# rpp0/gr-lora

Hardware: AMD Instinct MI355X
Metric: IQ Msamples/s demodulated (higher is better)
Workload: dtype f32

## Files before the change

### gr_lora_amd/capi.py

```python
from __future__ import annotations

import ctypes as C
import os
from typing import List, Optional, Sequence, Tuple

import numpy as np

_HERE = os.path.dirname(os.path.abspath(__file__))
LIB_PATH = os.environ.get("LORA_HIP_LIB") or os.path.join(_HERE, "liblora_hip.so")

DEMOD_GRAD, DEMOD_FFT, DEMOD_FFT_COMPAT = 0, 1, 2
FLAG_TRACE = 1
FLAG_PIN_HOST = 2
FLAG_FAST_SYNC = 4
FLAG_NO_DECOUPLED = 8
IQ_CF32, IQ_SC16, IQ_SC8, IQ_CU8 = 0, 1, 2, 3

EXPORTS = [
    "lora_hip_abi_version", "lora_hip_strerror", "lora_hip_last_error", "lora_hip_create", "lora_hip_destroy",
    "lora_hip_get_geometry", "lora_hip_set_sf", "lora_hip_set_samp_rate", "lora_hip_work", "lora_hip_flush",
    "lora_hip_decode_device", "lora_hip_frames_available", "lora_hip_poll_frame", "lora_hip_drain_frames", "lora_hip_drain_slots", "lora_hip_demod_symbols_device", "lora_hip_demod_symbols_ex_device",
    "lora_hip_last_timing", "lora_hip_last_plan", "lora_hip_get_table", "lora_hip_last_payload_pass", "lora_hip_gap_starts_device", "lora_hip_decode_device_begin", "lora_hip_decode_device_end", "lora_hip_decode_device_prepass", "lora_hip_trace", "lora_hip_trace_clear", "lora_hip_check_frame", "lora_hip_estimate_cfo_device", "lora_hip_ref_ifreq_device",
    "lora_hip_set_stream_latency", "lora_hip_stream_info", "lora_hip_walker_kernel_name", "lora_hip_window_stats_device", "lora_hip_detect_preambles_device", "lora_hip_decode_at_headers_device",
    "lora_hip_mux_create", "lora_hip_mux_destroy", "lora_hip_mux_work", "lora_hip_mux_flush", "lora_hip_mux_set_latency", "lora_hip_mux_set_max_ahead", "lora_hip_mux_frames_available",
    "lora_hip_mux_poll_frame", "lora_hip_mux_passes", "lora_hip_mux_last_error",
    "lora_hip_iq_item_bytes", "lora_hip_iq_unpack_device", "lora_hip_work_raw",
]


EXPORTS_CHANNELIZER = [
    "lora_hip_channelizer_create", "lora_hip_channelizer_destroy", "lora_hip_channelizer_last_error", "lora_hip_channelizer_taps",
    "lora_hip_channelizer_output_items", "lora_hip_channelizer_run_device", "lora_hip_channelizer_work", "lora_hip_channelizer_apply_cfo",
    "lora_hip_channelizer_last_kernel_ms", "lora_hip_channelizer_run_device_raw", "lora_hip_channelizer_work_raw",
]


EXPORTS_FILTERBANK = [
    "lora_hip_filterbank_create", "lora_hip_filterbank_destroy", "lora_hip_filterbank_last_error", "lora_hip_filterbank_taps",
    "lora_hip_filterbank_output_items", "lora_hip_filterbank_run_device", "lora_hip_filterbank_run_device_rows", "lora_hip_filterbank_work",
    "lora_hip_filterbank_last_kernel_ms", "lora_hip_filterbank_run_device_raw", "lora_hip_filterbank_run_device_rows_raw", "lora_hip_filterbank_work_raw",
]


EXPORTS_GATEWAY = [
    "lora_hip_gateway_create", "lora_hip_gateway_destroy", "lora_hip_gateway_last_error", "lora_hip_gateway_work", "lora_hip_gateway_work_device",
    "lora_hip_gateway_flush", "lora_hip_gateway_set_latency", "lora_hip_gateway_frames_available", "lora_hip_gateway_poll_frame", "lora_hip_gateway_stats",
    "lora_hip_gateway_work_raw", "lora_hip_gateway_work_device_raw",
]

FILTERBANK_MAX_DST = 8
GATEWAY_MAX_DECODERS = 7
GATEWAY_STEP_OUTPUTS = 65536


class FilterBankConfig(C.Structure):
    _fields_ = [("struct_size", C.c_uint32), ("samp_rate", C.c_double), ("grid_offset_hz", C.c_double), ("n_grid", C.c_uint32),
                ("channels", C.POINTER(C.c_int32)), ("n_channels", C.c_uint32), ("bandwidth", C.c_uint32), ("decimation", C.c_uint32),
                ("device", C.c_int32), ("cutoff_hz", C.c_float), ("transition_hz", C.c_float), ("flags", C.c_uint32)]


class ChannelizerConfig(C.Structure):
    _fields_ = [("struct_size", C.c_uint32), ("samp_rate", C.c_float), ("center_freq", C.c_float), ("channel_list", C.POINTER(C.c_float)),
                ("n_channels", C.c_uint32), ("bandwidth", C.c_uint32), ("decimation", C.c_uint32), ("device", C.c_int32),
                ("cutoff_hz", C.c_float), ("transition_hz", C.c_float), ("flags", C.c_uint32)]


CHANNELIZER_FLAG_UINT32_OFFSET = 1


class Config(C.Structure):
    _fields_ = [("struct_size", C.c_uint32), ("samp_rate", C.c_float), ("bandwidth", C.c_uint32),
                ("sf", C.c_uint8), ("implicit", C.c_uint8), ("cr", C.c_uint8), ("crc", C.c_uint8),
                ("reduced_rate", C.c_uint8), ("disable_drift_correction", C.c_uint8), ("reserved0", C.c_uint8 * 2),
                ("device", C.c_int32), ("demod", C.c_int32), ("flags", C.c_uint32),
                ("segment_symbols", C.c_uint32), ("batch_items", C.c_uint32)]


class FrameInfo(C.Structure):
    _fields_ = [("stream", C.c_uint32), ("length", C.c_uint32), ("header_pos", C.c_int64), ("end_pos", C.c_int64)]


class Step(C.Structure):
    _fields_ = [("state", C.c_int32), ("consumed", C.c_int32), ("pos", C.c_int64), ("bin", C.c_int32),
                ("fine", C.c_int32), ("value", C.c_float), ("stream", C.c_uint32), ("cycles", C.c_uint32), ("reserved", C.c_uint32)]


class Timing(C.Structure):
    _fields_ = [("walker_ms", C.c_float), ("total_device_ms", C.c_float), ("walker_launches", C.c_uint32),
                ("jobs", C.c_uint32), ("probes", C.c_uint32), ("slow_path_relaunches", C.c_uint32),
                ("items", C.c_uint64)]


class FrameCheck(C.Structure):
    _fields_ = [("has_header", C.c_uint8), ("header_checksum_ok", C.c_uint8), ("has_crc", C.c_uint8), ("crc_ok", C.c_uint8),
                ("header_checksum_rx", C.c_uint8), ("header_checksum_calc", C.c_uint8), ("crc_rx", C.c_uint16), ("crc_calc", C.c_uint16),
                ("reserved", C.c_uint16)]


class StreamInfo(C.Structure):
    _fields_ = [("batch_items", C.c_uint64), ("buffered_items", C.c_uint64), ("passes", C.c_uint64), ("passes_by_latency", C.c_uint64),
                ("consumed_base", C.c_int64), ("max_latency_ms", C.c_float), ("pass_in_flight", C.c_uint32)]


class WindowStats(C.Structure):
    _fields_ = [("bin_down", C.c_int32), ("peak_down", C.c_float), ("total_down", C.c_float), ("bin_up", C.c_int32), ("peak_up", C.c_float), ("total_up", C.c_float)]


class Preamble(C.Structure):
    _fields_ = [("header_pos", C.c_int64), ("run_pos", C.c_int64), ("stream", C.c_uint32), ("run_len", C.c_uint32), ("bin", C.c_int32), ("sfd_index", C.c_int32),
                ("pmr", C.c_float), ("cfo_bins", C.c_float), ("cfo_hz", C.c_float), ("delta", C.c_int32)]


class GatewayConfig(C.Structure):
    _fields_ = [("struct_size", C.c_uint32), ("filterbank", FilterBankConfig), ("decoders", C.POINTER(Config)), ("n_decoders", C.c_uint32),
                ("flags", C.c_uint32)]


class GatewayFrameInfo(C.Structure):
    _fields_ = [("row", C.c_uint32), ("grid_index", C.c_int32), ("sf", C.c_uint32), ("decoder", C.c_uint32), ("length", C.c_uint32),
                ("reserved", C.c_uint32), ("header_pos", C.c_int64), ("end_pos", C.c_int64)]


class GatewayStats(C.Structure):
    _fields_ = [("struct_size", C.c_uint32), ("n_decoders", C.c_uint32), ("passes", C.c_uint64 * GATEWAY_MAX_DECODERS),
                ("passes_by_latency", C.c_uint64 * GATEWAY_MAX_DECODERS), ("filterbank_calls", C.c_uint64), ("filterbank_ms", C.c_double),
                ("items_in", C.c_uint64), ("step_outputs", C.c_uint64)]


class LoraHipError(RuntimeError):
    def __init__(self, status: int, msg: str):
        super().__init__("lora_hip status %d: %s" % (status, msg))
        self.status = status


_lib = None


def load():
    global _lib
    if _lib is not None:
        return _lib
    try:
        import torch
    except ImportError:
        pass
    if not os.path.exists(LIB_PATH):
        raise ImportError("liblora_hip.so not built: run `python -c 'import __graft_entry__ as g; g.build()'` "
                          "(hipcc --offload-arch=gfx950).  There is no CPU fallback.")
    L = C.CDLL(LIB_PATH)
    vp = C.c_void_p
    L.lora_hip_abi_version.restype = C.c_uint32
    L.lora_hip_strerror.restype = C.c_char_p
    L.lora_hip_strerror.argtypes = [C.c_int]
    L.lora_hip_last_error.restype = C.c_char_p
    L.lora_hip_last_error.argtypes = [vp]
    L.lora_hip_create.argtypes = [C.POINTER(Config), C.POINTER(vp)]
    L.lora_hip_destroy.argtypes = [vp]
    L.lora_hip_destroy.restype = None
    L.lora_hip_get_geometry.argtypes = [vp, C.POINTER(C.c_uint32), C.POINTER(C.c_uint32), C.POINTER(C.c_uint32)]
    L.lora_hip_set_sf.argtypes = [vp, C.c_uint8]
    L.lora_hip_set_samp_rate.argtypes = [vp, C.c_float]
    L.lora_hip_work.argtypes = [vp, vp, C.c_size_t, C.POINTER(C.c_size_t)]
    L.lora_hip_flush.argtypes = [vp]
    L.lora_hip_decode_device.argtypes = [vp, vp, C.c_size_t, vp, vp, C.c_uint32, vp]
    L.lora_hip_frames_available.restype = C.c_size_t
    L.lora_hip_frames_available.argtypes = [vp]
    L.lora_hip_poll_frame.argtypes = [vp, vp, C.c_size_t, C.POINTER(C.c_size_t), C.POINTER(FrameInfo)]
    L.lora_hip_drain_frames.argtypes = [vp, vp, C.c_size_t, C.POINTER(FrameInfo), C.c_size_t, C.POINTER(C.c_size_t)]
    L.lora_hip_drain_slots.argtypes = [vp, vp, C.c_size_t, C.c_size_t, C.POINTER(C.c_size_t)]
    L.lora_hip_demod_symbols_device.argtypes = [vp, vp, C.c_size_t, vp, C.c_size_t, C.c_int, vp, vp]
    L.lora_hip_demod_symbols_ex_device.argtypes = [vp, vp, C.c_size_t, vp, C.c_size_t, C.c_int, vp, vp, vp]
    L.lora_hip_last_timing.argtypes = [vp, C.POINTER(Timing)]
    L.lora_hip_last_plan.argtypes = [vp, C.POINTER(C.c_uint32), C.POINTER(C.c_uint32)]
    L.lora_hip_last_payload_pass.argtypes = [vp, C.POINTER(C.c_uint32), C.POINTER(C.c_uint32), C.POINTER(C.c_uint32), C.POINTER(C.c_uint32), C.POINTER(C.c_uint32), C.POINTER(C.c_float)]
    L.lora_hip_decode_device_begin.argtypes = [vp, vp, C.c_size_t, vp, vp, C.c_uint32, vp, C.c_uint32]
    L.lora_hip_decode_device_end.argtypes = [vp]
    L.lora_hip_decode_device_prepass.argtypes = [vp, vp, C.c_size_t, vp, vp, C.c_uint32, vp, C.c_uint32]
    L.lora_hip_gap_starts_device.argtypes = [vp, vp, C.c_size_t, vp, vp, C.c_uint32, vp, C.c_size_t, vp, vp]
    L.lora_hip_trace.restype = C.c_size_t
    L.lora_hip_trace.argtypes = [vp, C.POINTER(C.POINTER(Step))]
    L.lora_hip_trace_clear.argtypes = [vp]
    L.lora_hip_trace_clear.restype = None
    L.lora_hip_estimate_cfo_device.argtypes = [vp, vp, C.c_size_t, C.POINTER(C.c_int64), C.c_size_t, C.c_int, C.POINTER(C.c_float), vp]
    L.lora_hip_estimate_cfo_device.restype = C.c_int
    L.lora_hip_ref_ifreq_device.argtypes = [vp, vp, C.c_size_t, C.POINTER(C.c_float), C.POINTER(C.c_float), vp]
    L.lora_hip_ref_ifreq_device.restype = C.c_int
    if hasattr(L, "lora_hip_get_table") or not os.environ.get("LORA_HIP_LIB"):
        L.lora_hip_get_table.argtypes = [vp, C.c_int, C.POINTER(C.c_float), C.c_size_t, C.POINTER(C.c_size_t)]
        L.lora_hip_get_table.restype = C.c_int
    L.lora_hip_window_stats_device.argtypes = [vp, vp, C.c_size_t, vp, C.c_size_t, C.POINTER(WindowStats), vp]
    L.lora_hip_detect_preambles_device.argtypes = [vp, vp, C.c_size_t, vp, vp, C.c_uint32, C.c_float, C.POINTER(Preamble), C.c_size_t, C.POINTER(C.c_size_t), vp]
    L.lora_hip_decode_at_headers_device.argtypes = [vp, vp, C.c_size_t, vp, vp, C.c_uint32, C.POINTER(Preamble), C.c_size_t, vp]
    L.lora_hip_walker_kernel_name.argtypes = [vp]
    L.lora_hip_walker_kernel_name.restype = C.c_char_p
    L.lora_hip_mux_create.argtypes = [C.POINTER(Config), C.c_uint32, C.POINTER(vp)]
    L.lora_hip_mux_destroy.argtypes = [vp]
    L.lora_hip_mux_destroy.restype = None
    L.lora_hip_mux_work.argtypes = [vp, C.c_uint32, vp, C.c_size_t]
    L.lora_hip_mux_flush.argtypes = [vp]
    L.lora_hip_mux_set_latency.argtypes = [vp, C.c_float]
    L.lora_hip_mux_set_max_ahead.argtypes = [vp, C.c_size_t]
    L.lora_hip_mux_frames_available.argtypes = [vp]
    L.lora_hip_mux_frames_available.restype = C.c_size_t
    L.lora_hip_mux_poll_frame.argtypes = [vp, vp, C.c_size_t, C.POINTER(C.c_size_t), C.POINTER(FrameInfo)]
    L.lora_hip_mux_passes.argtypes = [vp, C.POINTER(C.c_uint64), C.POINTER(C.c_uint64)]
    L.lora_hip_mux_last_error.argtypes = [vp]
    L.lora_hip_mux_last_error.restype = C.c_char_p
    L.lora_hip_set_stream_latency.argtypes = [vp, C.c_float]
    L.lora_hip_stream_info.argtypes = [vp, C.POINTER(StreamInfo)]
    L.lora_hip_check_frame.argtypes = [C.c_char_p, C.c_size_t, C.POINTER(FrameCheck)]
    L.lora_hip_check_frame.restype = C.c_int
    L.lora_hip_channelizer_create.argtypes = [C.POINTER(ChannelizerConfig), C.POINTER(vp)]
    L.lora_hip_channelizer_destroy.argtypes = [vp]
    L.lora_hip_channelizer_destroy.restype = None
    L.lora_hip_channelizer_last_error.argtypes = [vp]
    L.lora_hip_channelizer_last_error.restype = C.c_char_p
    L.lora_hip_channelizer_taps.argtypes = [vp, vp, C.c_size_t, C.POINTER(C.c_size_t)]
    L.lora_hip_channelizer_output_items.argtypes = [vp, C.c_size_t]
    L.lora_hip_channelizer_output_items.restype = C.c_size_t
    L.lora_hip_channelizer_run_device.argtypes = [vp, vp, C.c_size_t, vp, C.c_size_t, C.POINTER(C.c_size_t), vp]
    L.lora_hip_channelizer_work.argtypes = [vp, vp, C.c_size_t, vp, C.c_size_t, C.POINTER(C.c_size_t)]
    L.lora_hip_channelizer_apply_cfo.argtypes = [vp, C.c_float]
    L.lora_hip_channelizer_last_kernel_ms.argtypes = [vp]
    L.lora_hip_channelizer_last_kernel_ms.restype = C.c_float
    L.lora_hip_filterbank_create.argtypes = [C.POINTER(FilterBankConfig), C.POINTER(vp)]
    L.lora_hip_filterbank_destroy.argtypes = [vp]
    L.lora_hip_filterbank_destroy.restype = None
    L.lora_hip_filterbank_last_error.argtypes = [vp]
    L.lora_hip_filterbank_last_error.restype = C.c_char_p
    L.lora_hip_filterbank_taps.argtypes = [vp, vp, C.c_size_t, C.POINTER(C.c_size_t)]
    L.lora_hip_filterbank_output_items.argtypes = [vp, C.c_size_t]
    L.lora_hip_filterbank_output_items.restype = C.c_size_t
    L.lora_hip_filterbank_run_device.argtypes = [vp, vp, C.c_size_t, vp, C.c_size_t, C.POINTER(C.c_size_t), vp]
    L.lora_hip_filterbank_work.argtypes = [vp, vp, C.c_size_t, vp, C.c_size_t, C.POINTER(C.c_size_t)]
    L.lora_hip_filterbank_last_kernel_ms.argtypes = [vp]
    L.lora_hip_filterbank_last_kernel_ms.restype = C.c_float
    L.lora_hip_filterbank_run_device_rows.argtypes = [vp, vp, C.c_size_t, C.POINTER(vp), C.c_uint32, C.c_size_t, C.POINTER(C.c_size_t), vp]
    L.lora_hip_gateway_create.argtypes = [C.POINTER(GatewayConfig), C.POINTER(vp)]
    L.lora_hip_gateway_destroy.argtypes = [vp]
    L.lora_hip_gateway_destroy.restype = None
    L.lora_hip_gateway_last_error.argtypes = [vp]
    L.lora_hip_gateway_last_error.restype = C.c_char_p
    L.lora_hip_gateway_work.argtypes = [vp, vp, C.c_size_t]
    L.lora_hip_gateway_work_device.argtypes = [vp, vp, C.c_size_t, vp]
    L.lora_hip_gateway_flush.argtypes = [vp]
    L.lora_hip_gateway_set_latency.argtypes = [vp, C.c_float]
    L.lora_hip_gateway_frames_available.argtypes = [vp]
    L.lora_hip_gateway_frames_available.restype = C.c_size_t
    L.lora_hip_gateway_poll_frame.argtypes = [vp, vp, C.c_size_t, C.POINTER(C.c_size_t), C.POINTER(GatewayFrameInfo)]
    L.lora_hip_gateway_stats.argtypes = [vp, C.POINTER(GatewayStats)]
    if hasattr(L, "lora_hip_work_raw") or not os.environ.get("LORA_HIP_LIB"):
        L.lora_hip_iq_item_bytes.argtypes = [C.c_int]
        L.lora_hip_iq_item_bytes.restype = C.c_size_t
        L.lora_hip_iq_unpack_device.argtypes = [C.c_int, vp, C.c_size_t, C.c_int, C.c_float, vp, vp]
        L.lora_hip_work_raw.argtypes = [vp, vp, C.c_size_t, C.c_int, C.c_float, C.POINTER(C.c_size_t)]
        L.lora_hip_channelizer_run_device_raw.argtypes = [vp, vp, C.c_size_t, C.c_int, C.c_float, vp, C.c_size_t, C.POINTER(C.c_size_t), vp]
        L.lora_hip_channelizer_work_raw.argtypes = [vp, vp, C.c_size_t, C.c_int, C.c_float, vp, C.c_size_t, C.POINTER(C.c_size_t)]
        L.lora_hip_filterbank_run_device_raw.argtypes = [vp, vp, C.c_size_t, C.c_int, C.c_float, vp, C.c_size_t, C.POINTER(C.c_size_t), vp]
        L.lora_hip_filterbank_run_device_rows_raw.argtypes = [vp, vp, C.c_size_t, C.c_int, C.c_float, C.POINTER(vp), C.c_uint32, C.c_size_t, C.POINTER(C.c_size_t), vp]
        L.lora_hip_filterbank_work_raw.argtypes = [vp, vp, C.c_size_t, C.c_int, C.c_float, vp, C.c_size_t, C.POINTER(C.c_size_t)]
        L.lora_hip_gateway_work_raw.argtypes = [vp, vp, C.c_size_t, C.c_int, C.c_float]
        L.lora_hip_gateway_work_device_raw.argtypes = [vp, vp, C.c_size_t, C.c_int, C.c_float, vp]
    _lib = L
    return L


def _raw_items(raw, fmt=None):
    from . import iqformat
    return iqformat.as_components(raw, fmt)


def unpack_device(d_raw: int, n_items: int, fmt: int, d_out: int, scale: float = 0.0, device: int = 0, stream: int = 0):
    L = load()
    st = L.lora_hip_iq_unpack_device(int(device), d_raw, int(n_items), int(fmt), float(scale), d_out, stream)
    if st != 0:
        raise LoraHipError(st, "lora_hip_iq_unpack_device: %s" % L.lora_hip_strerror(st).decode())


def check_frame(blob: bytes) -> FrameCheck:
    out = FrameCheck()
    st = load().lora_hip_check_frame(bytes(blob), len(blob), C.byref(out))
    if st != 0:
        raise LoraHipError(st, "lora_hip_check_frame: blob too short")
    return out


class Handle:

    def __init__(self, samp_rate=1e6, bandwidth=125000, sf=7, implicit=False, cr=4, crc=True, reduced_rate=False,
                 disable_drift_correction=False, device=0, demod=DEMOD_FFT_COMPAT, flags=0, segment_symbols=0,
                 batch_items=0):
        self.L = load()
        cfg = Config(struct_size=C.sizeof(Config), samp_rate=float(samp_rate), bandwidth=int(bandwidth), sf=int(sf),
                     implicit=int(bool(implicit)), cr=int(cr), crc=int(bool(crc)), reduced_rate=int(bool(reduced_rate)),
                     disable_drift_correction=int(bool(disable_drift_correction)), device=int(device), demod=int(demod),
                     flags=int(flags), segment_symbols=int(segment_symbols), batch_items=int(batch_items))
        h = C.c_void_p()
        st = self.L.lora_hip_create(C.byref(cfg), C.byref(h))
        if st != 0:
            raise LoraHipError(st, "%s (%s)" % (self.L.lora_hip_strerror(st).decode(), self.L.lora_hip_last_error(None).decode()))
        self.h = h
        a, b, d = C.c_uint32(), C.c_uint32(), C.c_uint32()
        self.L.lora_hip_get_geometry(self.h, C.byref(a), C.byref(b), C.byref(d))
        self.sps, self.nbins, self.decim = a.value, b.value, d.value
        self.device, self.batch_items = int(device), int(batch_items)

    def close(self):
        if getattr(self, "h", None):
            self.L.lora_hip_destroy(self.h)
            self.h = None

    __del__ = close

    def _check(self, st: int):
        if st != 0:
            raise LoraHipError(st, "%s (%s)" % (self.L.lora_hip_strerror(st).decode(), self.L.lora_hip_last_error(self.h).decode()))

    def work(self, iq: np.ndarray) -> int:
        a = np.ascontiguousarray(iq, dtype=np.complex64)
        n = C.c_size_t(0)
        self._check(self.L.lora_hip_work(self.h, a.ctypes.data, a.size, C.byref(n)))
        return n.value

    def work_raw(self, raw, fmt=None, scale: float = 0.0) -> int:
        a, f, n_items = _raw_items(raw, fmt)
        n = C.c_size_t(0)
# ... 31 lines not shown

    def decode_device_end(self):
        self._check(self.L.lora_hip_decode_device_end(self.h))

    def gap_starts_device(self, dev_ptr: int, total_items: int, offs: Sequence[int], lens: Sequence[int], stream: int = 0):
        o = np.ascontiguousarray(offs, dtype=np.uint64)
        l = np.ascontiguousarray(lens, dtype=np.uint64)
        cap = int(sum(int(x) for x in l) // 64 + 16)
        pos = np.zeros(cap, dtype=np.int64)
        cnt = np.zeros(o.size, dtype=np.uint32)
        self._check(self.L.lora_hip_gap_starts_device(self.h, dev_ptr, total_items, o.ctypes.data, l.ctypes.data, o.size, pos.ctypes.data, cap,
                                                      cnt.ctypes.data, stream))
        out, k = [], 0
        for c in cnt:
            out.append(pos[k:k + int(c)].copy()); k += int(c)
        return out

    def demod_symbols_device(self, dev_ptr: int, total_items: int, offsets: Sequence[int], demod: int, stream: int = 0) -> np.ndarray:
        off = np.ascontiguousarray(offsets, dtype=np.int64)
        out = np.zeros(off.size, dtype=np.uint32)
        self._check(self.L.lora_hip_demod_symbols_device(self.h, dev_ptr, total_items, off.ctypes.data, off.size, demod, out.ctypes.data, stream))
        return out

    def demod_symbols_ex_device(self, dev_ptr: int, total_items: int, offsets: Sequence[int], demod: int, stream: int = 0):
        off = np.ascontiguousarray(offsets, dtype=np.int64)
        out = np.zeros(off.size, dtype=np.uint32)
        fine = np.zeros(off.size, dtype=np.int32)
        self._check(self.L.lora_hip_demod_symbols_ex_device(self.h, dev_ptr, total_items, off.ctypes.data, off.size, demod, out.ctypes.data,
                                                            fine.ctypes.data, stream))
        return out, fine

    def estimate_cfo_device(self, dev_ptr: int, total_items: int, offsets: Sequence[int], mode: int = 1, stream: int = 0) -> np.ndarray:
        off = np.ascontiguousarray(offsets, dtype=np.int64)
        out = np.zeros(off.size, dtype=np.float32)
        self._check(self.L.lora_hip_estimate_cfo_device(self.h, C.c_void_p(dev_ptr), total_items, off.ctypes.data_as(C.POINTER(C.c_int64)), off.size, mode,
                                                        out.ctypes.data_as(C.POINTER(C.c_float)), C.c_void_p(stream)))
        return out

    def ref_ifreq_device(self, dev_ptr: int, n_items: int, stream: int = 0):
        arg = np.zeros(n_items, dtype=np.float32)
        f = np.zeros(n_items - 1, dtype=np.float32)
        self._check(self.L.lora_hip_ref_ifreq_device(self.h, C.c_void_p(dev_ptr), n_items, arg.ctypes.data_as(C.POINTER(C.c_float)),
                                                     f.ctypes.data_as(C.POINTER(C.c_float)), C.c_void_p(stream)))
        return arg, f

    def window_stats_device(self, dev_ptr: int, total_items: int, offsets: Sequence[int], stream: int = 0):
        off = np.ascontiguousarray(offsets, dtype=np.int64)
        out = (WindowStats * max(off.size, 1))()
        self._check(self.L.lora_hip_window_stats_device(self.h, dev_ptr, total_items, off.ctypes.data, off.size, out, stream))
        return [(o.bin_down, o.peak_down, o.total_down, o.bin_up, o.peak_up, o.total_up) for o in out[: off.size]]

    def detect_preambles_device(self, dev_ptr: int, total_items: int, offs: Sequence[int], lens: Sequence[int], threshold: float = 0.0, stream: int = 0, cap: int = 4096):
        o = np.ascontiguousarray(offs, dtype=np.uint64)
        l = np.ascontiguousarray(lens, dtype=np.uint64)
        out = (Preamble * cap)()
        n = C.c_size_t(0)
        self._check(self.L.lora_hip_detect_preambles_device(self.h, dev_ptr, total_items, o.ctypes.data, l.ctypes.data, o.size, float(threshold), out, cap, C.byref(n), stream))
        return [dict(header_pos=p.header_pos, run_pos=p.run_pos, stream=p.stream, run_len=p.run_len, bin=p.bin, sfd_index=p.sfd_index, pmr=p.pmr,
                     cfo_bins=p.cfo_bins, cfo_hz=p.cfo_hz, delta=p.delta) for p in out[: n.value]]

    def decode_at_headers_device(self, dev_ptr: int, total_items: int, offs: Sequence[int], lens: Sequence[int], preambles, stream: int = 0):
        o = np.ascontiguousarray(offs, dtype=np.uint64)
        l = np.ascontiguousarray(lens, dtype=np.uint64)
        arr = (Preamble * max(len(preambles), 1))()
        for i, p in enumerate(preambles):
            st, hp = (p["stream"], p["header_pos"]) if isinstance(p, dict) else p
            arr[i].stream, arr[i].header_pos = int(st), int(hp)
        self._check(self.L.lora_hip_decode_at_headers_device(self.h, dev_ptr, total_items, o.ctypes.data, l.ctypes.data, o.size, arr, len(preambles), stream))

    def frames_available(self) -> int:
        return self.L.lora_hip_frames_available(self.h)

    def poll_frame(self) -> Optional[Tuple[bytes, FrameInfo]]:
        buf = (C.c_uint8 * 320)()
        n = C.c_size_t(0)
        info = FrameInfo()
        self._check(self.L.lora_hip_poll_frame(self.h, buf, 320, C.byref(n), C.byref(info)))
        if n.value == 0:
            return None
        return bytes(buf[: n.value]), info

    def drain(self) -> List[Tuple[bytes, FrameInfo]]:
        out = []
        while True:
            n_avail = self.frames_available()
            if n_avail == 0:
                return out
            k = min(n_avail, 4096)
            buf = (C.c_uint8 * (k * 280))()
            infos = (FrameInfo * k)()
            n = C.c_size_t(0)
            self._check(self.L.lora_hip_drain_frames(self.h, buf, k * 280, infos, k, C.byref(n)))
            raw = bytes(buf)
            off = 0
            for i in range(n.value):
                ln = infos[i].length
                inf = FrameInfo(infos[i].stream, ln, infos[i].header_pos, infos[i].end_pos)
                out.append((raw[off:off + ln], inf))
                off += ln
            if n.value == 0:
                return out

    INFO_DTYPE = np.dtype([("stream", "<u4"), ("length", "<u4"), ("header_pos", "<i8"), ("end_pos", "<i8")])

    def drain_raw(self):
        bufs, infos = [], []
        while True:
            n_avail = self.frames_available()
            if n_avail == 0:
                break
            k = min(n_avail, 8192)
            buf = np.empty(k * 280, dtype=np.uint8)
            inf = np.empty(k, dtype=self.INFO_DTYPE)
            n = C.c_size_t(0)
            self._check(self.L.lora_hip_drain_frames(self.h, buf.ctypes.data, buf.size, C.cast(inf.ctypes.data, C.POINTER(FrameInfo)), k, C.byref(n)))
            if n.value == 0:
                break
            inf = inf[: n.value]
            bufs.append(buf[: int(inf["length"].sum())])
            infos.append(inf)
        if not bufs:
            return np.empty(0, dtype=np.uint8), np.empty(0, dtype=self.INFO_DTYPE)
        return np.concatenate(bufs), np.concatenate(infos)

    def drain_slots(self, slot_bytes: int) -> np.ndarray:
        n_avail = self.frames_available()
        out = np.empty((max(n_avail, 1), slot_bytes), dtype=np.uint8)
        n = C.c_size_t(0)
        self._check(self.L.lora_hip_drain_slots(self.h, out.ctypes.data, slot_bytes, n_avail, C.byref(n)))
        return out[: n.value]

    def timing(self) -> Timing:
        t = Timing()
        self._check(self.L.lora_hip_last_timing(self.h, C.byref(t)))
        return t

    def plan(self):
        b, n = C.c_uint32(0), C.c_uint32(0)
        self._check(self.L.lora_hip_last_plan(self.h, C.byref(b), C.byref(n)))
        return bool(b.value), int(n.value)

    def table(self, which: int) -> np.ndarray:
        n = C.c_size_t()
        self._check(self.L.lora_hip_get_table(self.h, which, None, 0, C.byref(n)))
        out = np.empty(n.value, np.float32)
        self._check(self.L.lora_hip_get_table(self.h, which, out.ctypes.data_as(C.POINTER(C.c_float)), n.value, C.byref(n)))
        return out

    def payload_pass(self):
        a, mv, b, r, c, m = C.c_uint32(0), C.c_uint32(0), C.c_uint32(0), C.c_uint32(0), C.c_uint32(0), C.c_float(0)
        self._check(self.L.lora_hip_last_payload_pass(self.h, C.byref(a), C.byref(mv), C.byref(b), C.byref(r), C.byref(c), C.byref(m)))
        return dict(packets=int(a.value), moved=int(mv.value), rerun=int(b.value), rounds=int(r.value), symbols=int(c.value), ms=float(m.value))

    def trace(self):
        p = C.POINTER(Step)()
        n = self.L.lora_hip_trace(self.h, C.byref(p))
        return [(p[i].state, p[i].pos, p[i].consumed, p[i].bin, p[i].fine, p[i].value, p[i].stream, p[i].cycles) for i in range(n)]

    def trace_clear(self):
        self.L.lora_hip_trace_clear(self.h)


class Mux:

    def __init__(self, n_channels, samp_rate=1e6, bandwidth=125000, sf=7, implicit=False, cr=4, crc=True, reduced_rate=False,
                 disable_drift_correction=False, device=0, demod=DEMOD_FFT_COMPAT, flags=0, segment_symbols=0, batch_items=0):
        self.L = load()
        cfg = Config(struct_size=C.sizeof(Config), samp_rate=float(samp_rate), bandwidth=int(bandwidth), sf=int(sf), implicit=int(bool(implicit)), cr=int(cr),
                     crc=int(bool(crc)), reduced_rate=int(bool(reduced_rate)), disable_drift_correction=int(bool(disable_drift_correction)), device=int(device),
                     demod=int(demod), flags=int(flags), segment_symbols=int(segment_symbols), batch_items=int(batch_items))
        self.h = C.c_void_p()
        st = self.L.lora_hip_mux_create(C.byref(cfg), int(n_channels), C.byref(self.h))
        if st != 0:
            raise LoraHipError(st, "%s (%s)" % (self.L.lora_hip_strerror(st).decode(), self.L.lora_hip_last_error(None).decode()))
        self.n_channels = int(n_channels)

    def _check(self, st):
        if st != 0:
            raise LoraHipError(st, "%s (%s)" % (self.L.lora_hip_strerror(st).decode(), (self.L.lora_hip_mux_last_error(self.h) or b"").decode()))

    def work(self, channel: int, iq: np.ndarray):
        a = np.ascontiguousarray(iq, dtype=np.complex64)
        self._check(self.L.lora_hip_mux_work(self.h, int(channel), a.ctypes.data, a.size))

    def flush(self):
        self._check(self.L.lora_hip_mux_flush(self.h))

    def set_latency(self, ms: float):
        self._check(self.L.lora_hip_mux_set_latency(self.h, float(ms)))

    def set_max_ahead(self, items: int):
        self._check(self.L.lora_hip_mux_set_max_ahead(self.h, int(items)))

    def passes(self):
        a, b = C.c_uint64(0), C.c_uint64(0)
        self._check(self.L.lora_hip_mux_passes(self.h, C.byref(a), C.byref(b)))
        return int(a.value), int(b.value)

    def drain(self) -> List[Tuple[bytes, FrameInfo]]:
        out = []
        buf = (C.c_uint8 * 320)()
        while self.L.lora_hip_mux_frames_available(self.h):
            n = C.c_size_t(0)
            info = FrameInfo()
            self._check(self.L.lora_hip_mux_poll_frame(self.h, buf, 320, C.byref(n), C.byref(info)))
            out.append((bytes(buf[: n.value]), info))
        return out

    def close(self):
        if getattr(self, "h", None):
            self.L.lora_hip_mux_destroy(self.h)
            self.h = None

    __del__ = close


class Channelizer:

    def __init__(self, samp_rate, center_freq, channel_list, bandwidth, decimation=1, device=0, cutoff_hz=0.0, transition_hz=0.0, flags=0):
        self.L = load()
        self.n_channels = len(channel_list)
        self._chan = (C.c_float * self.n_channels)(*[float(c) for c in channel_list])
        cfg = ChannelizerConfig(struct_size=C.sizeof(ChannelizerConfig), samp_rate=float(samp_rate), center_freq=float(center_freq),
                                channel_list=self._chan, n_channels=self.n_channels, bandwidth=int(bandwidth), decimation=int(decimation), device=int(device),
                                cutoff_hz=float(cutoff_hz), transition_hz=float(transition_hz), flags=int(flags))
        self.h = C.c_void_p()
        st = self.L.lora_hip_channelizer_create(C.byref(cfg), C.byref(self.h))
        if st != 0:
            raise LoraHipError(st, self.L.lora_hip_strerror(st).decode())

    def _check(self, st):
        if st != 0:
            raise LoraHipError(st, (self.L.lora_hip_channelizer_last_error(self.h) or b"").decode() or self.L.lora_hip_strerror(st).decode())

    def taps(self) -> np.ndarray:
        n = C.c_size_t(0)
        self._check(self.L.lora_hip_channelizer_taps(self.h, None, 0, C.byref(n)))
        t = np.zeros(n.value, dtype=np.float32)
        self._check(self.L.lora_hip_channelizer_taps(self.h, t.ctypes.data, t.size, C.byref(n)))
        return t

    def output_items(self, n_in: int) -> int:
        return int(self.L.lora_hip_channelizer_output_items(self.h, n_in))

    def work(self, x) -> np.ndarray:
        a = np.ascontiguousarray(x, dtype=np.complex64)
        no = self.output_items(a.size)
        out = np.zeros((self.n_channels, max(no, 1)), dtype=np.complex64)
        n = C.c_size_t(0)
        self._check(self.L.lora_hip_channelizer_work(self.h, a.ctypes.data, a.size, out.ctypes.data, out.shape[1], C.byref(n)))
        return out[:, : n.value]

    def run_device(self, d_in: int, n_in: int, d_out: int, out_stride: int, stream: int = 0) -> int:
        n = C.c_size_t(0)
        self._check(self.L.lora_hip_channelizer_run_device(self.h, d_in, n_in, d_out, out_stride, C.byref(n), stream))
        return int(n.value)

    def work_raw(self, raw, fmt=None, scale: float = 0.0) -> np.ndarray:
        a, f, n_items = _raw_items(raw, fmt)
        no = self.output_items(n_items)
        out = np.zeros((self.n_channels, max(no, 1)), dtype=np.complex64)
        n = C.c_size_t(0)
        self._check(self.L.lora_hip_channelizer_work_raw(self.h, a.ctypes.data, n_items, f, float(scale), out.ctypes.data, out.shape[1], C.byref(n)))
        return out[:, : n.value]

    def run_device_raw(self, d_in: int, n_in: int, fmt: int, d_out: int, out_stride: int, scale: float = 0.0, stream: int = 0) -> int:
        n = C.c_size_t(0)
        self._check(self.L.lora_hip_channelizer_run_device_raw(self.h, d_in, n_in, int(fmt), float(scale), d_out, out_stride, C.byref(n), stream))
        return int(n.value)

    def apply_cfo(self, cfo: float):
        self._check(self.L.lora_hip_channelizer_apply_cfo(self.h, float(cfo)))

    def kernel_ms(self) -> float:
        return float(self.L.lora_hip_channelizer_last_kernel_ms(self.h))

    def close(self):
        if self.h:
            self.L.lora_hip_channelizer_destroy(self.h)
            self.h = C.c_void_p()

    def __del__(self):
        try:
            self.close()
        except Exception:
            pass


class FilterBank:

    def __init__(self, samp_rate, grid_offset, n_grid, channels, bandwidth, decimation=1, device=0, cutoff_hz=0.0, transition_hz=0.0, flags=0):
        self.L = load()
        self.channels = [int(k) for k in channels]
        self.n_channels = len(self.channels)
        self._chan = (C.c_int32 * max(self.n_channels, 1))(*self.channels)
        cfg = FilterBankConfig(struct_size=C.sizeof(FilterBankConfig), samp_rate=float(samp_rate), grid_offset_hz=float(grid_offset), n_grid=int(n_grid),
                               channels=self._chan, n_channels=self.n_channels, bandwidth=int(bandwidth), decimation=int(decimation), device=int(device),
                               cutoff_hz=float(cutoff_hz), transition_hz=float(transition_hz), flags=int(flags))
        self.h = C.c_void_p()
        st = self.L.lora_hip_filterbank_create(C.byref(cfg), C.byref(self.h))
        if st != 0:
            raise LoraHipError(st, self.L.lora_hip_strerror(st).decode())

    def _check(self, st):
        if st != 0:
            raise LoraHipError(st, (self.L.lora_hip_filterbank_last_error(self.h) or b"").decode() or self.L.lora_hip_strerror(st).decode())
# ... 139 lines not shown
```

### gr_lora_amd/csrc/lora_device.h

```cpp
#pragma once
#include <stdint.h>

#if !defined(__HIPCC__) && !defined(HIP_INCLUDE_HIP_HIP_RUNTIME_H)
struct float2 { float x, y; };
#endif

namespace lora_hip {

constexpr int kWG = 256;
constexpr int kMaxBinsPerThread = 16;
constexpr int kMaxFrame = 3 + 255 + 2;
constexpr int kMaxCodewords = 640;

enum DecState : int32_t { kDetect = 0, kSync, kFindSfd, kPause, kDecodeHeader, kDecodePayload, kStop };

enum AttemptStatus : uint32_t {
    kAttemptNone = 0,
    kAttemptFrame = 1,
    kAttemptLostSync = 2,
    kAttemptOutOfData = 3,
    kAttemptAtHeader = 4,
    kAttemptAtSfd = 5,
    kAttemptHeaderOnly = 6
};
struct SkippedPayload {
    uint8_t  phdr[3];
    uint8_t  n_left;
    uint8_t  left[8];
    int32_t  payload_symbols;
};
constexpr float kSfdIllVar = 1.0f / 4096.0f;
constexpr int kMaxSfdRec = 12;

struct DevParams {
    uint32_t sf, nbins, nbins_hdr, sps, decim, log_nbins, delay_after_sync;
    uint32_t implicit, reduced_rate, enable_fine_sync, demod_mode;
    uint32_t ctor_cr, ctor_crc;
    uint32_t use_fast;
    uint32_t fft_groups;
    uint32_t fft_stride;
    uint32_t lds_work_bytes;
    uint32_t ifreq_in_lds_1;
    uint32_t ifreq_in_lds_2;
    float    down_ifreq_avg;
    float    down_ifreq_sd;
    float    down_ifreq_dsum;
    double   sync_a, sync_b;
    uint32_t sync_closed_form;
    uint32_t strict_sync;
    uint32_t samples_per_second;
    uint32_t ffs_on;
    float    ffs_alpha, ffs_jump, ffs_tol;
    const float2 *down;
    const float  *up_ifreq;
    const float  *down_ifreq;
    const float  *up_ifreq_v;
    const float2 *twN;
    const float2 *tws;
    const float  *wave_tabs;
    const float2 *w3_tw;
    const float2 *w3_ctab;
    const float  *team_tabs;
};

struct Job {
    uint64_t stream_off;
    uint64_t stream_len;
    int64_t  start;
    int64_t  scan_limit;
    uint32_t stream_id;
    uint32_t cr_prev;
    uint32_t max_attempts;
    uint32_t stop_at_header;
    int64_t  probe_limit;
    uint32_t start_at_header;
    uint32_t tail_stop_sfd;
};

struct AttemptRec {
    int64_t  start_pos;
    int64_t  trig_pos;
    int64_t  hdr_pos;
    int64_t  end_pos;
    uint32_t status;
    uint32_t npush;
    float    push_tail[4];
    uint32_t cr_prev;
    uint32_t hdr_ambig;
    uint32_t frame_len;
    uint32_t n_symbols;
    int64_t  sfd_pos[kMaxSfdRec];
    uint32_t n_sfd;
    uint8_t  sfd_fails[kMaxSfdRec];
    uint8_t  frame[kMaxFrame + 4];
};

struct JobResult {
    int64_t  final_pos;
    uint32_t n_attempts;
    uint32_t final_cr;
    uint32_t npush;
    float    push_tail[4];
    uint32_t stop_reason;
    uint32_t n_steps;
    uint32_t pad;
    uint32_t cyc[6];
    uint32_t rounds[6];
    int64_t  tail_final_pos;
    uint32_t tail_valid, tail_first_rec, tail_n_attempts, tail_final_cr, tail_npush, tail_stop_reason, tail_pad, tail_rsv;
    float    tail_push_tail[4];
    uint32_t ctl[4];
    uint32_t dbg[6];
};

struct StepRec {
    int32_t  state, consumed;
    int64_t  pos;
    int32_t  bin, fine;
    float    value;
    uint32_t stream;
    uint32_t cycles;
    uint32_t pad;
};

struct LaunchCfg {
    const float2 *iq;
    const Job *jobs;
    JobResult *results;
    AttemptRec *recs;
    uint32_t recs_per_job;
    float *scratch;
    StepRec *trace;
    uint32_t trace_cap;
    uint32_t n_jobs;
    uint32_t *balance;
    uint32_t skip_payload;
};
constexpr uint32_t kBalanceCus = 2048;
constexpr uint32_t kBalanceWords = 3u * kBalanceCus;

struct EnvStream {
    uint64_t off;
    uint32_t first_block;
    uint32_t n_blocks;
};
int launch_envelope(const float2 *iq, const EnvStream *streams , uint32_t n_streams, uint32_t sps,
                    float *d_E, unsigned long long *d_bitmap , void *stream);

int launch_walker(const DevParams &p, const LaunchCfg &c, void *stream);
const char *walker_kernel_name(const DevParams &p);
struct DemodAlt { int32_t *shift; uint32_t *bins; int32_t *fine; int64_t max_start; };
int launch_demod_symbols(const DevParams &p, const float2 *iq, const int64_t *d_offsets, uint32_t n,
                         int demod, uint32_t *d_bins, int32_t *d_fine, float *scratch, void *stream, const DemodAlt *alt = nullptr);
int launch_detect_windows(const DevParams &p, const float2 *iq, const int64_t *d_offsets, uint32_t n, void *d_out , void *stream);
constexpr int kPayloadHyp = 4;
struct PayloadDesc {
    uint32_t n_walk;
    uint32_t n_hyp;
    int32_t  hyp_shift[kPayloadHyp];
    int32_t  hyp_base[kPayloadHyp];
    uint32_t hyp_from[kPayloadHyp];
    uint32_t hyp_to[kPayloadHyp];
    int64_t  room;
    SkippedPayload sk;
};
enum PayloadWalk : uint32_t { kWalkComplete = 0, kWalkOutOfData = 1, kWalkNeedShift = 2 };
struct PayloadOut {
    uint32_t result;
    uint32_t at;
    int32_t  shift;
    uint32_t frame_len;
    uint8_t  frame[kMaxFrame + 4];
};
int launch_payload_chain(const DevParams &p, const uint32_t *d_bins, const int32_t *d_fine, const DemodAlt &alt, const PayloadDesc *descs, PayloadOut *outs, uint32_t n_packets, void *stream);
bool walker_has_skip_variant(const DevParams &p);
int launch_ref_ifreq(const float2 *x, uint32_t n, float *d_arg, float *d_ifreq, void *stream);
int launch_cfo(const DevParams &p, const float2 *iq, const int64_t *d_offsets, uint32_t n, int mode, float *d_out, void *stream);
bool walker3_covers(uint32_t sf);
uint32_t w3_tw_entries(uint32_t sf);
void build_w3_tables(uint32_t sf, float2 *tw, float2 *ctab );
uint32_t wave_tables_floats(uint32_t sf);
void build_wave_tables(uint32_t sf, const float2 *down, float *out);
uint32_t wave_tables_floats_d(uint32_t sf, uint32_t decim);
void build_wave_tables_d(uint32_t sf, uint32_t decim, const float2 *down, float *out);
uint32_t team_tables_entries(uint32_t sf);
void build_team_tables(uint32_t sf, const float2 *down, double dt, double bandwidth, float2 *out);
uint32_t walker_lds_bytes(const DevParams &p);
uint32_t walker_resident_slots(const DevParams &p);
uint32_t walker_resident_slots_full(const DevParams &p);
const char *walker_kernel_name_for(const DevParams &p, uint32_t n_jobs, bool skip = false);

}
```

### gr_lora_amd/csrc/lora_kernels.hip

```cpp

#include <hip/hip_runtime.h>
#include <math.h>
#include <stdio.h>
#include <atomic>
#include <cstdlib>
#include <stdint.h>
#include <type_traits>

#include "lora_device.h"
#include "whitening_data.inc"

namespace lora_hip {

__constant__ unsigned char c_whiten_cr56[LORA_WHITEN_CR56_LEN];
__constant__ unsigned char c_whiten_cr78[LORA_WHITEN_CR78_LEN];
__constant__ unsigned char c_h84_decode[256];
static std::atomic<bool> g_consts_ready[16];

static unsigned char h_hamming_encode(unsigned v)
{
    const unsigned b0 = v & 1u, b1 = (v >> 1) & 1u, b2 = (v >> 2) & 1u, b3 = (v >> 3) & 1u;
    const unsigned p1 = b1 ^ b2 ^ b3, p2 = b0 ^ b1 ^ b2, p3 = b0 ^ b1 ^ b3, p4 = b0 ^ b2 ^ b3;
    return (unsigned char)(p1 | (b0 << 1) | (b1 << 2) | (b2 << 3) | (p2 << 4) | (b3 << 5) | (p3 << 6) | (p4 << 7));
}
// ... 295 lines not shown
    return r;
}
constexpr int ilog2(int v) { return v <= 1 ? 0 : 1 + ilog2(v >> 1); }

#define LORA_DPP(old, v, ctrl, bank) __builtin_amdgcn_update_dpp((old), (v), (ctrl), 0xf, (bank), false)

template <int MASK>
__device__ __forceinline__ float lane_xor(float f)
{
    const int v = __builtin_bit_cast(int, f);
    int r;
    if constexpr (MASK == 1) r = LORA_DPP(0, v, 0xB1, 0xf);
    else if constexpr (MASK == 2) r = LORA_DPP(0, v, 0x4E, 0xf);
    else if constexpr (MASK == 4) {
        r = LORA_DPP(0, v, 0x104, 0x5);
        r = LORA_DPP(r, v, 0x114, 0xA);
    } else if constexpr (MASK == 8) r = LORA_DPP(0, v, 0x128, 0xf);
    else if constexpr (MASK == 16) {
        const auto p = __builtin_amdgcn_permlane16_swap(v, v, false, false);
        r = (threadIdx.x & 16) ? p[0] : p[1];
    } else {
        const auto p = __builtin_amdgcn_permlane32_swap(v, v, false, false);
        r = (threadIdx.x & 32) ? p[0] : p[1];
    }
    return __builtin_bit_cast(float, r);
}

template <int MASK>
__device__ __forceinline__ float2 lane_xor2(float2 v) { return make_float2(lane_xor<MASK>(v.x), lane_xor<MASK>(v.y)); }

__device__ __forceinline__ float wave_sum_rows(float v)
{
    v += lane_xor<1>(v); v += lane_xor<2>(v); v += lane_xor<4>(v); v += lane_xor<8>(v);
    const float r0 = __builtin_bit_cast(float, __builtin_amdgcn_readlane(__builtin_bit_cast(int, v), 0));
    const float r1 = __builtin_bit_cast(float, __builtin_amdgcn_readlane(__builtin_bit_cast(int, v), 16));
    const float r2 = __builtin_bit_cast(float, __builtin_amdgcn_readlane(__builtin_bit_cast(int, v), 32));
    const float r3 = __builtin_bit_cast(float, __builtin_amdgcn_readlane(__builtin_bit_cast(int, v), 48));
    return (r0 + r1) + (r2 + r3);
}

__device__ __forceinline__ uint32_t uni32(uint32_t v) { return (uint32_t)__builtin_amdgcn_readfirstlane((int)v); }
__device__ __forceinline__ uint64_t uni64(uint64_t v) { return ((uint64_t)uni32((uint32_t)(v >> 32)) << 32) | uni32((uint32_t)v); }
__device__ __forceinline__ Job uniform_job(const Job &j)
{
    Job u;
    u.stream_off = uni64(j.stream_off); u.stream_len = uni64(j.stream_len);
    u.start = (int64_t)uni64((uint64_t)j.start); u.scan_limit = (int64_t)uni64((uint64_t)j.scan_limit);
    u.stream_id = uni32(j.stream_id); u.cr_prev = uni32(j.cr_prev); u.max_attempts = uni32(j.max_attempts); u.stop_at_header = uni32(j.stop_at_header);
    u.probe_limit = (int64_t)uni64((uint64_t)j.probe_limit);
    u.start_at_header = uni32(j.start_at_header); u.tail_stop_sfd = uni32(j.tail_stop_sfd);
    return u;
}

__device__ __forceinline__ uint32_t rotl_bits(uint32_t bits, uint32_t count, uint32_t size)
{
    const uint32_t mask = (1u << size) - 1u;
    count %= size;
    bits &= mask;
    return ((bits << count) & mask) | (bits >> (size - count));
}

__device__ __forceinline__ uint8_t deshuffle_byte(uint8_t v)
{
    return (uint8_t)(((v >> 5) & 1u) | (((v >> 0) & 1u) << 1) | (((v >> 1) & 1u) << 2) | (((v >> 2) & 1u) << 3) |
                     (((v >> 4) & 1u) << 4) | (((v >> 3) & 1u) << 5) | (((v >> 6) & 1u) << 6) | (((v >> 7) & 1u) << 7));
}

__device__ __forceinline__ uint8_t data_bits(uint8_t cw)
{
    return (uint8_t)(((cw >> 1) & 1u) | (((cw >> 2) & 1u) << 1) | (((cw >> 3) & 1u) << 2) | (((cw >> 5) & 1u) << 3));
}

__device__ void deinterleave_block(Shared &sh, uint32_t n_words, uint32_t ppm, uint32_t &n_cw)
{
    if (n_words <= 8u) {
        uint32_t r[8];
#pragma unroll
        for (uint32_t i = 0; i < 8u; i++) r[i] = (i < n_words) ? rotl_bits(sh.words[i], i, ppm) : 0u;
        for (uint32_t x = 0; x < ppm; x++) {
            uint32_t c = 0;
#pragma unroll
            for (uint32_t i = 0; i < 8u; i++) c |= ((r[i] >> x) & 1u) << i;
            if (n_cw < kMaxCodewords) sh.cw[n_cw++] = (uint8_t)c;
        }
        return;
    }
    for (uint32_t x = 0; x < ppm; x++) {
        uint8_t c = 0;
        for (uint32_t i = 0; i < n_words; i++) c |= (uint8_t)(((rotl_bits(sh.words[i], i, ppm) >> x) & 1u) << i);
        if (n_cw < kMaxCodewords) sh.cw[n_cw++] = c;
    }
}
__device__ __forceinline__ void deinterleave_block_wave(Shared &sh, uint64_t words_pk, uint32_t n_words, uint32_t ppm, uint32_t &n_cw)
{
    const uint32_t lane = threadIdx.x & 63u, x = lane >> 3, i = lane & 7u;
    const uint32_t w = (uint32_t)(words_pk >> (8u * i)) & 0xffu;
    int sh_amt = (int)x - (int)(i % ppm);
    if (sh_amt < 0) sh_amt += (int)ppm;
    const bool bit = x < ppm && i < n_words && ((w >> sh_amt) & 1u);
    const unsigned long long m = __ballot(bit);
    if (i == 0u && x < ppm && n_cw + x < (uint32_t)kMaxCodewords) sh.cw[n_cw + x] = (uint8_t)((m >> (8u * x)) & 0xffu);
    n_cw = (n_cw + ppm <= (uint32_t)kMaxCodewords) ? n_cw + ppm : (uint32_t)kMaxCodewords;
}

__device__ __forceinline__ void deinterleave_block_wave16(Shared &sh, const uint32_t (&wpk)[4], uint32_t n_words, uint32_t ppm, uint32_t &n_cw)
{
    const uint32_t lane = threadIdx.x & 63u, x = lane >> 3, i = lane & 7u;
    const uint32_t pair = i < 2u ? wpk[0] : i < 4u ? wpk[1] : i < 6u ? wpk[2] : wpk[3];
    const uint32_t w = (pair >> (16u * (i & 1u))) & 0xffffu;
    const int rot = (int)(i % ppm);
    int sh_amt = (int)x - rot;
    if (sh_amt < 0) sh_amt += (int)ppm;
    const bool bit = x < ppm && i < n_words && ((w >> sh_amt) & 1u);
    const unsigned long long m = __ballot(bit);
    if (i == 0u && x < ppm && n_cw + x < (uint32_t)kMaxCodewords) sh.cw[n_cw + x] = (uint8_t)((m >> (8u * x)) & 0xffu);
    int sh8 = 8 - rot;
    if (sh8 < 0) sh8 += (int)ppm;
    const unsigned long long m8 = __ballot(lane < 8u && ppm > 8u && i < n_words && ((w >> sh8) & 1u));
    if (lane == 0u && ppm > 8u && n_cw + 8u < (uint32_t)kMaxCodewords) sh.cw[n_cw + 8u] = (uint8_t)(m8 & 0xffu);
    n_cw = (n_cw + ppm <= (uint32_t)kMaxCodewords) ? n_cw + ppm : (uint32_t)kMaxCodewords;
}

__device__ void decode_header_bytes(const Shared &sh, uint32_t n_cw, int cr_class, uint8_t out[3])
{
    uint8_t w[6];
    for (int i = 0; i < 5; i++) w[i] = ((uint32_t)i < n_cw) ? deshuffle_byte(sh.cw[i]) : 0;
    w[5] = 0;
    for (int k = 0; k < 3; k++) {
        if (cr_class == 2) out[k] = (uint8_t)((c_h84_decode[w[2 * k]] << 4) | c_h84_decode[w[2 * k + 1]]);
        else if (cr_class == 1) out[k] = (uint8_t)((data_bits(w[2 * k]) << 4) | data_bits(w[2 * k + 1]));
        else out[k] = 0;
    }
}

__device__ void decode_payload_bytes(Shared &sh, uint32_t n_cw, uint32_t cr, uint32_t n_bytes)
{
    __syncthreads();
    for (uint32_t i = threadIdx.x; i < n_cw; i += blockDim.x) {
        uint8_t w = deshuffle_byte(sh.cw[i]);
        if (cr <= 2u) w ^= (i < LORA_WHITEN_CR56_LEN) ? c_whiten_cr56[i] : 0;
        else w ^= (i < LORA_WHITEN_CR78_LEN) ? c_whiten_cr78[i] : 0;
        sh.cw[i] = w;
    }
    __syncthreads();
    for (uint32_t k = threadIdx.x; k < n_bytes; k += blockDim.x) {
        const uint8_t c0 = (2u * k < n_cw) ? sh.cw[2u * k] : 0, c1 = (2u * k + 1u < n_cw) ? sh.cw[2u * k + 1u] : 0;
        uint8_t lo, hi;
        if (cr >= 3u) { lo = c_h84_decode[c0]; hi = c_h84_decode[c1]; }
        else if (cr >= 1u) { lo = data_bits(c0); hi = data_bits(c1); }
        else { lo = 0; hi = 0; }
        sh.dec[k] = (uint8_t)((hi << 4) | lo);
    }
    __syncthreads();
}

template <int FLDS>
__device__ __forceinline__ void walker_body(const DevParams &P, const LaunchCfg &C)
{
    extern __shared__ __attribute__((aligned(16))) unsigned char smem[];
    float2 *work = reinterpret_cast<float2 *>(smem);
    float *fl = reinterpret_cast<float *>(smem);
    Shared &sh = *reinterpret_cast<Shared *>(smem + P.lds_work_bytes);
    float *red = sh.red;
    __shared__ strict::Cands g_sc;
    __shared__ __attribute__((aligned(16))) float g_strict_buf[strict::kK * 256];

    const uint32_t jid = blockIdx.x;
    if (jid >= C.n_jobs) return;
    const Job job = C.jobs[jid];
    const float2 *__restrict__ X = C.iq + job.stream_off;
    const int64_t n_items = (int64_t)job.stream_len;
    const uint32_t sps = P.sps;
    float *gscratch = C.scratch ? C.scratch + (size_t)jid * 2u * sps : nullptr;
    float *f1, *f2;
    if constexpr (FLDS >= 1) f1 = fl; else f1 = gscratch;
    if constexpr (FLDS >= 2) f2 = fl; else f2 = gscratch;
    AttemptRec *recs = C.recs + (size_t)jid * C.recs_per_job;
    StepRec *trace = C.trace ? C.trace + (size_t)jid * C.trace_cap : nullptr;
    const bool t0 = threadIdx.x == 0;
    const float *vtab = P.up_ifreq_v, *utab = P.up_ifreq;

    int32_t state = kDetect;
    int64_t pos = job.start;
    uint32_t corr_fails = 0, cr = job.cr_prev, has_crc = P.ctor_crc;
    int32_t payload_symbols = 0;
    uint32_t payload_length = 0, n_words = 0, n_cw = 0, n_sym = 0;
    float energy_threshold = 0.0f;
    uint8_t phdr0 = 0, phdr1 = (uint8_t)((P.ctor_cr << 5) | (P.ctor_crc << 4)), phdr2 = 0;
    uint32_t n_att = 0, npush = 0, n_steps = 0, stop_reason = 0;
    float push_tail[4] = {0.f, 0.f, 0.f, 0.f};
    int64_t att_start = pos, att_trig = -1, att_hdr = -1;
    uint32_t att_cr_prev = cr, att_ambig = 0;
    bool in_attempt = false, frame_ok = false;
    if (job.start_at_header) { state = kDecodeHeader; in_attempt = true; att_trig = pos; att_hdr = pos; }

    auto end_step = [&](int32_t st_in, int32_t consumed, int32_t step_bin, int32_t fine, float step_val, long long t_start) -> bool {
        if (trace && t0 && n_steps < C.trace_cap) {
            StepRec &s = trace[n_steps];
            s.state = st_in; s.consumed = consumed; s.pos = pos; s.bin = step_bin; s.fine = fine; s.value = step_val;
            s.stream = job.stream_id; s.cycles = (uint32_t)(clock64() - t_start); s.pad = 0;
        }
        n_steps++;
        pos += consumed;
        if (in_attempt && state == kDetect) {
            if (t0) {
                AttemptRec &r = recs[n_att];
                r.status = frame_ok ? kAttemptFrame : kAttemptLostSync;
                if (!frame_ok) r.frame_len = 0;
                r.start_pos = att_start; r.trig_pos = att_trig; r.hdr_pos = att_hdr; r.end_pos = pos;
                r.npush = npush;
                for (int i = 0; i < 4; i++) r.push_tail[i] = push_tail[i];
                r.cr_prev = att_cr_prev; r.hdr_ambig = att_ambig; r.n_symbols = n_sym; r.n_sfd = 0;
            }
            n_att++;
            in_attempt = false;
            frame_ok = false;
            npush = 0;
            att_start = pos;
        } else if (in_attempt && job.stop_at_header && state == kDecodeHeader) {
            stop_reason = 3;
            return true;
        }
        return false;
    };

    auto post_symbol = [&](bool do_demod, uint32_t bin_idx, bool is_first) {
        bool block_done = false;
        if (do_demod) {
            const bool reduced = is_first || P.reduced_rate;
            if (reduced) bin_idx = (uint32_t)(lroundf((float)bin_idx / 4.0f) % (long)P.nbins_hdr);
            const uint32_t word = bin_idx ^ (bin_idx >> 1u);
            const uint32_t need = 4u + (is_first ? 4u : cr);
            if (t0 && n_words < 16u) sh.words[n_words] = word;
            n_words++;
            n_sym++;
            if (n_words == need) {
                const uint32_t ppm = reduced ? P.sf - 2u : P.sf;
                if (t0) { uint32_t tmp = n_cw; deinterleave_block(sh, need, ppm, tmp); }
                n_cw = (n_cw + ppm <= (uint32_t)kMaxCodewords) ? n_cw + ppm : (uint32_t)kMaxCodewords;
                n_words = 0;
                block_done = true;
            }
        }
        if (is_first) {
            if (block_done) {
                if (P.implicit) {
                    payload_symbols = 1;
                } else {
                    __syncthreads();
                    if (t0) {
                        uint8_t hA[3], hB[3], h0[3] = {0, 0, 0};
                        decode_header_bytes(sh, n_cw, 2, hA);
                        decode_header_bytes(sh, n_cw, 1, hB);
                        const uint8_t *use = (cr >= 3u) ? hA : (cr >= 1u ? hB : h0);
                        sh.hdr[0] = use[0]; sh.hdr[1] = use[1]; sh.hdr[2] = use[2];
                        sh.hdr[3] = (uint8_t)((hA[0] != hB[0]) || (hA[1] != hB[1]) || (hA[2] != hB[2]));
                        const uint32_t rem = n_cw > 5u ? n_cw - 5u : 0u;
                        for (uint32_t i = 0; i < rem; i++) sh.cw[i] = sh.cw[i + 5u];
                    }
                    __syncthreads();
                    n_cw = n_cw > 5u ? n_cw - 5u : 0u;
                    phdr0 = sh.hdr[0]; phdr1 = sh.hdr[1]; phdr2 = sh.hdr[2];
                    att_ambig = sh.hdr[3];
                    if ((phdr1 >> 5) > 4) phdr1 = (uint8_t)((phdr1 & 0x1f) | (4u << 5));
                    cr = phdr1 >> 5;
                    has_crc = (phdr1 >> 4) & 1u;
                    payload_length = (uint32_t)phdr0 + 2u * has_crc;
                    const uint32_t redundancy = P.reduced_rate ? 2u : 0u;
                    const int symbols_per_block = (int)cr + 4;
                    const float bits_needed = (float)payload_length * 8.0f;
                    const float symbols_needed = bits_needed * ((float)symbols_per_block / 4.0f) / (float)(P.sf - redundancy);
                    const int blocks_needed = (int)ceilf(symbols_needed / (float)symbols_per_block);
                    payload_symbols = blocks_needed * symbols_per_block;
                }
                state = kDecodePayload;
            }
        } else {
            if (block_done && !P.implicit) payload_symbols -= (int32_t)(4u + cr);
            if (payload_symbols <= 0) {
                uint32_t n_bytes;
                if (cr >= 3u) n_bytes = (uint32_t)ceilf((float)n_cw * 4.0f / (4.0f + (float)cr));
                else n_bytes = (n_cw + 1u) / 2u;
                if (n_bytes > (uint32_t)(kMaxCodewords / 2 + 8)) n_bytes = kMaxCodewords / 2 + 8;
                decode_payload_bytes(sh, n_cw, cr, n_bytes);
                const uint32_t plen = payload_length > 257u ? 257u : payload_length;
                AttemptRec &r = recs[n_att];
                for (uint32_t i = threadIdx.x; i < plen; i += kWG) r.frame[3u + i] = (i < n_bytes) ? sh.dec[i] : 0;
                if (t0) {
                    r.frame[0] = phdr0; r.frame[1] = phdr1; r.frame[2] = phdr2;
                    r.frame_len = 3u + plen;
                }
                frame_ok = true;
                state = kDetect;
                n_words = 0; n_cw = 0;
            }
        }
    };

    while (true) {
        if (state == kDetect && !in_attempt) {
            if (pos >= job.scan_limit) { stop_reason = 0; break; }
            if (n_att >= C.recs_per_job) { stop_reason = 2; break; }
            if (job.max_attempts && n_att >= job.max_attempts) { stop_reason = 3; break; }
        }
        if (pos + 2 * (int64_t)sps > n_items) { stop_reason = 1; break; }
        const float2 *__restrict__ x = X + pos;
// ... 737 lines not shown
```

### gr_lora_amd/csrc/lora_runtime.cpp

```cpp

#include <hip/hip_runtime.h>

#include <algorithm>
#include <cmath>
#include <cstddef>
#include <cstdarg>
#include <cstdio>
#include <cstdlib>
#include <cstring>
#include <chrono>
#include <deque>
#include <new>
#include <string>
#include <vector>

#include "../../include/lora_hip.h"
#include "lora_device.h"
#include "lora_stitch.hpp"
#include "lora_mux_dev.h"
#include "lora_iq.h"

using namespace lora_hip;

namespace {

constexpr int kLoratapLen = 15;
constexpr uint32_t kWorkBudget = 64u * 1024u + 64u;

struct FrameQueue {
    struct Ref { size_t off; lora_hip_frame_info_t info; };
    std::vector<uint8_t> bytes;
    std::vector<Ref> refs;
    size_t head = 0;
    size_t size() const { return refs.size() - head; }
    bool empty() const { return head == refs.size(); }
    uint8_t *push(uint32_t len, const lora_hip_frame_info_t &info)
    {
        const size_t off = bytes.size();
        bytes.resize(off + len, 0);
        refs.push_back(Ref{off, info});
        return bytes.data() + off;
    }
    const Ref &front() const { return refs[head]; }
    const uint8_t *front_bytes() const { return bytes.data() + refs[head].off; }
    void pop()
    {
        if (++head == refs.size()) { refs.clear(); bytes.clear(); head = 0; }
    }
};

template <typename T>
struct PinnedBuf {
    T *p = nullptr;
    size_t cap = 0;
    hipError_t reserve(size_t n)
    {
        if (n <= cap) return hipSuccess;
        if (p) (void)hipHostFree(p);
        p = nullptr; cap = 0;
        const size_t want = n + n / 4 + 16;
        hipError_t e = hipHostMalloc((void **)&p, want * sizeof(T), hipHostMallocDefault);
        if (e == hipSuccess) cap = want;
        return e;
    }
    void release() { if (p) (void)hipHostFree(p); p = nullptr; cap = 0; }
};

uint8_t snr_byte(float snr)
{
    const double v = (double)(10.0f * log10f(snr)) + 0.5;
    if (!(v > -2147483649.0 && v < 2147483648.0)) return 0;
    return (uint8_t)(int32_t)v;
}

template <typename T>
struct DevBuf {
    T *p = nullptr;
    size_t cap = 0;
    hipError_t reserve(size_t n)
    {
        if (n <= cap) return hipSuccess;
        if (p) (void)hipFree(p);
        p = nullptr; cap = 0;
        const size_t want = n + n / 4 + 16;
        hipError_t e = hipMalloc((void **)&p, want * sizeof(T));
        if (e == hipSuccess) cap = want;
        return e;
    }
    void release() { if (p) (void)hipFree(p); p = nullptr; cap = 0; }
};

struct ChunkPipe {
    struct Chan {
        size_t fill = 0, tail_len = 0;
        uint32_t cr = 0;
        PwrState pwr;
        int64_t host_base = 0;
    };
    std::vector<Chan> ch;
    DevBuf<float2> dbuf[2];
    int cur = 0;
    size_t batch = 0, tailcap = 0, region = 0;
    hipStream_t copy_st = nullptr, comp_st = nullptr;
    hipEvent_t up_ev = nullptr, tail_ev = nullptr;
    bool inflight = false;
    float max_latency_ms = 50.0f;
    std::chrono::steady_clock::time_point t_first;
    bool have_first = false;
    uint64_t passes = 0, passes_by_latency = 0;
    float2 *row(size_t c) const { return dbuf[cur].p + c * region + tailcap + ch[c].fill; }
};

}

struct lora_hip_decoder {
    lora_hip_config_t cfg{};
    DevParams P{};
    int device = 0;
    float2 *d_down = nullptr, *d_twN = nullptr, *d_tws = nullptr;
    float *d_wave_tabs = nullptr;
    float2 *d_w3_tw = nullptr, *d_w3_ctab = nullptr;
    float2 *d_team_tabs = nullptr;
    float *d_up_ifreq = nullptr, *d_down_ifreq = nullptr, *d_up_ifreq_v = nullptr;
    std::vector<float2> h_up;
    size_t n_up_ifreq_v = 0;
    DevBuf<Job> d_jobs;
    DevBuf<JobResult> d_results;
    DevBuf<AttemptRec> d_recs;
    DevBuf<float> d_scratch;
    DevBuf<StepRec> d_trace;
    DevBuf<float2> d_staging;
    DevBuf<int64_t> d_offsets;
    DevBuf<uint32_t> d_bins;
    RunOut run_out[2];
    std::vector<JobResult> h_results;
    std::vector<AttemptRec> h_recs;
    std::vector<StepRec> h_trace;
    hipEvent_t ev0 = nullptr, ev1 = nullptr, ev_done = nullptr;
    hipEvent_t ev_pre0 = nullptr, ev_pre1 = nullptr, ev_dep = nullptr;
    hipStream_t pre_stream = nullptr;
    struct Pending { uint32_t nj = 0, recs_per_job = 0, eager = 0, trace_cap = 0; bool direct = true, open = false; hipStream_t st = nullptr;
                     std::chrono::steady_clock::time_point hp0, hp1; } pending;
    PassCtx pass;
    std::vector<StreamDesc> pass_streams;
    const float2 *pass_iq = nullptr;
    hipStream_t pass_st = nullptr;
    bool pass_open = false, iq_ready = false;
    bool pre_issued = false;
    const float2 *pre_iq = nullptr;
    uint64_t pre_sig = 0;
    uint32_t pre_ns = 0;
    std::chrono::steady_clock::time_point pre_hq0;
    FrameQueue frames;
    PinnedBuf<Job> p_jobs;
    PinnedBuf<JobResult> p_res;
    PinnedBuf<AttemptRec> p_recs;
    DevBuf<uint32_t> d_balance;
    DevBuf<float> d_env_E;
    DevBuf<unsigned long long> d_env_buf;
    PinnedBuf<EnvStream> p_env_streams;
    PinnedBuf<unsigned long long> p_env_buf;
    float envelope_ms = 0.0f;
    std::vector<lora_hip_step_t> trace;
    lora_hip_timing_t timing{};
    std::string err;
    ChunkPipe pipe;
    struct HostFeed {
        PinnedBuf<float2> stage[2];
        hipEvent_t stage_ev[2] = {nullptr, nullptr};
        bool stage_busy[2] = {false, false};
        int stage_i = 0;
        DevBuf<uint32_t> d_raw;
        std::vector<std::pair<uintptr_t, uintptr_t>> pinned;
        std::vector<std::pair<uintptr_t, uintptr_t>> refused;
    } feed;
    const char *last_kernel = nullptr;
    uint32_t last_kernel_jobs = 0;
    uint32_t resident_slots = 0;
    uint32_t resident_slots_alt = ~0u;
    uint32_t eager_recs = 4;
    uint32_t last_plan_burst = 0, last_plan_segments = 0;
    int decoupled_policy = -1;
    bool launch_skip = false;
    uint32_t dec_backoff = 0;
    uint32_t last_payload_packets = 0, last_payload_rerun = 0, last_payload_symbols = 0, last_payload_moved = 0, last_payload_rounds = 0;
    float last_payload_ms = 0.0f;
    PinnedBuf<int64_t> p_pay_off;
    PinnedBuf<PayloadDesc> p_pay_desc;
    PinnedBuf<PayloadOut> p_pay_out;
    DevBuf<int32_t> d_fine, d_alt_shift, d_alt_fine;
    DevBuf<uint32_t> d_alt_bins;
    hipStream_t pay_stream = nullptr;
    hipEvent_t ev_pay0 = nullptr, ev_pay1 = nullptr, ev_pay_done = nullptr;
    struct PayState { std::vector<uint32_t> active; size_t used = 0, cap_sym = 0, n_sym = 0; int round = 0; float ms = 0.0f; bool open = false; } pay;
};

namespace {

thread_local std::string g_create_err;

lora_hip_status fail(lora_hip_decoder *h, lora_hip_status s, const char *fmt, ...)
{
    char buf[512];
    va_list ap;
    va_start(ap, fmt);
    vsnprintf(buf, sizeof buf, fmt, ap);
    va_end(ap);
    if (h) h->err = buf;
    g_create_err = buf;
    return s;
}

#define HIP_TRY(h, expr)                                                                                   \
    do {                                                                                                   \
        hipError_t e__ = (expr);                                                                           \
        if (e__ != hipSuccess) return fail(h, LORA_HIP_ERR_HIP, "%s: %s", #expr, hipGetErrorString(e__)); \
    } while (0)

void host_ifreq(const float2 *x, float *out, uint32_t window)
{
    for (uint32_t i = 1; i < window; i++) {
        const float p1 = std::atan2(x[i - 1].y, x[i - 1].x);
        float p2 = std::atan2(x[i].y, x[i].x);
        while ((double)(p2 - p1) > M_PI) p2 = (float)((double)p2 - 2.0 * M_PI);
        while ((double)(p2 - p1) < -M_PI) p2 = (float)((double)p2 + 2.0 * M_PI);
        out[i - 1] = p2 - p1;
    }
    out[window - 1] = out[window - 2];
}

template <typename T>
lora_hip_status upload(lora_hip_decoder *h, T **dst, const std::vector<T> &src)
{
    HIP_TRY(h, hipMalloc((void **)dst, src.size() * sizeof(T)));
    HIP_TRY(h, hipMemcpy(*dst, src.data(), src.size() * sizeof(T), hipMemcpyHostToDevice));
    return LORA_HIP_OK;
}

lora_hip_status build_tables(lora_hip_decoder *h)
{
    const lora_hip_config_t &c = h->cfg;
    DevParams &P = h->P;
    const uint32_t samples_per_second = (uint32_t)c.samp_rate;
    const double dt = (double)(1.0f / (float)samples_per_second);
    const double symbols_per_second = (double)c.bandwidth / (double)(1u << c.sf);
    const uint32_t sps = (uint32_t)((double)samples_per_second / symbols_per_second);
    const uint32_t N = 1u << c.sf;
    if (sps < N || (sps & (sps - 1u)) != 0u)
        return fail(h, LORA_HIP_ERR_BAD_CONFIG, "samples per symbol (%u) must be a power-of-two multiple of 2^sf (%u)", sps, N);
    const uint32_t D = sps / N;
    if (D > 16u) return fail(h, LORA_HIP_ERR_BAD_CONFIG, "decimation %u > 16 is not supported", D);
    P.sf = c.sf; P.nbins = N; P.nbins_hdr = 1u << (c.sf - 2); P.sps = sps; P.decim = D; P.samples_per_second = samples_per_second;
    P.log_nbins = c.sf; P.delay_after_sync = sps / 4u;
    P.implicit = c.implicit ? 1u : 0u; P.reduced_rate = c.reduced_rate ? 1u : 0u;
    P.enable_fine_sync = c.disable_drift_correction ? 0u : 1u;
    P.demod_mode = (uint32_t)c.demod;
    P.ctor_cr = c.cr & 7u; P.ctor_crc = c.crc ? 1u : 0u;
    P.use_fast = getenv("LORA_HIP_NO_FAST") ? 0u : 1u;
    uint32_t G = 1;
    while ((size_t)(D / G) * (N + 1u) * sizeof(float2) > kWorkBudget && G < D) G <<= 1;
    P.fft_groups = G;
    P.fft_stride = (D / G > 1u) ? N + 1u : N;
    uint32_t work = (uint32_t)((size_t)(D / G) * P.fft_stride * sizeof(float2));
    if (work < 2u * sps * sizeof(float) && 2u * sps * sizeof(float) <= kWorkBudget) work = 2u * sps * (uint32_t)sizeof(float);
    if (work < sps * sizeof(float) && sps * sizeof(float) <= kWorkBudget) work = sps * (uint32_t)sizeof(float);
    work = (work + 15u) & ~15u;
    P.lds_work_bytes = work;
    P.ifreq_in_lds_1 = (sps * sizeof(float) <= work) ? 1u : 0u;
    P.ifreq_in_lds_2 = (2u * sps * sizeof(float) <= work) ? 1u : 0u;

    std::vector<float2> down(sps), up(sps), twN(N / 2u > 0 ? N / 2u : 1u), tws(sps);
    const double T = -0.5 * c.bandwidth * symbols_per_second, f0 = c.bandwidth / 2.0, pre_dir = 2.0 * M_PI;
    for (uint32_t i = 0; i < sps; i++) {
        const double t = dt * i;
        const float pd = (float)(pre_dir * t * (f0 + T * t));
        const float pu = (float)(pre_dir * t * (f0 + T * t) * -1.0f);
        const float cd = std::cos(pd), sd = std::sin(pd), cu = std::cos(pu), su = std::sin(pu);
        down[i] = make_float2(cd - sd, sd + cd);
        up[i] = make_float2(cu - su, su + cu);
    }
    std::vector<float> down_ifreq(sps), up_ifreq(sps), up3(3u * (size_t)sps + 4u * D + 8u);
    host_ifreq(down.data(), down_ifreq.data(), sps);
    host_ifreq(up.data(), up_ifreq.data(), sps);
    {
        std::vector<float2> tmp(3u * (size_t)sps);
        for (int r = 0; r < 3; r++) std::copy(up.begin(), up.end(), tmp.begin() + (size_t)r * sps);
        host_ifreq(tmp.data(), up3.data(), 3u * sps);
        for (size_t i = 3u * (size_t)sps; i < up3.size(); i++) up3[i] = up3[3u * (size_t)sps - 1u];
    }
    {
        P.ffs_on = 0u; P.ffs_alpha = 0.0f; P.ffs_jump = 0.0f; P.ffs_tol = 0.0f;
        if (D == 8u && c.sf >= 7u && c.sf <= 12u && !getenv("LORA_HIP_NO_FFS")) {
            const size_t S = sps, lo = S + 7u, hi = 3u * S - 8u;
            auto dV = [&](size_t m) { return (double)up3[m + 1u] - (double)up3[m]; };
            double sum = 0.0;
            bool ok = std::fabs(dV(2u * S - 1u)) > 0.5;
            for (size_t m = lo; m < hi; m++) if (m != 2u * S - 1u) { sum += dV(m); ok = ok && std::fabs(dV(m)) < 0.01; }
            const double alpha = sum / (double)(hi - lo - 1u);
            std::vector<double> cs(hi - lo + 1u, 0.0);
            for (size_t m = lo; m < hi; m++) { const double e = (m == 2u * S - 1u) ? 0.0 : dV(m) - alpha; cs[m - lo + 1u] = cs[m - lo] + e * e; }
            double worst = 0.0;
            for (size_t o = lo; o + S <= hi; o++) worst = std::max(worst, cs[o + S - lo] - cs[o - lo]);
            const double enorm = std::sqrt(worst), fmax = c.sf >= 11u ? std::atan(0.5) : c.sf >= 9u ? M_PI / 2.0 : M_PI;
            const double fnorm = c.sf >= 9u ? std::sqrt((double)S * fmax * fmax + 8.0 * M_PI * M_PI) : fmax * std::sqrt((double)S);
            double tol = 1.05 * fnorm * enorm + 1.0e-4;
            if (c.sf >= 9u && tol > 0.15) tol = 12.0 * fmax * enorm + 1.0e-4;
            if (ok && tol < 0.2) { P.ffs_on = 1u; P.ffs_alpha = (float)alpha; P.ffs_jump = (float)(dV(2u * S - 1u) - alpha); P.ffs_tol = (float)tol; }
            if (getenv("LORA_HIP_DEBUG")) fprintf(stderr, "[lora_hip] closed-form fine_sync: SF%u alpha %.6g jump %.6g |e| %.4g tol %.4g -> %s\n", (unsigned)c.sf, alpha, dV(2u * S - 1u) - alpha, enorm, tol, P.ffs_on ? "on" : "off");
        }
    }
    {
        const uint32_t n = sps - 1u;
        float s = 0.0f;
        for (uint32_t i = 0; i < n; i++) s += down_ifreq[i];
        const float avg = s / (float)n;
        float var = 0.0f;
        for (uint32_t i = 0; i < n; i++) { const float t = down_ifreq[i] - avg; var += t * t; }
        var /= (float)n;
        P.down_ifreq_avg = avg;
        P.down_ifreq_sd = std::sqrt(var);
        float ds = 0.0f;
        for (uint32_t i = 0; i < n; i++) ds += down_ifreq[i] - avg;
        P.down_ifreq_dsum = ds;
        double sk = 0, su = 0, skk = 0, sku = 0;
        for (uint32_t k = 0; k < n; k++) { sk += k; su += up_ifreq[k]; skk += (double)k * k; sku += (double)k * up_ifreq[k]; }
        P.sync_b = (n * sku - sk * su) / (n * skk - sk * sk);
        P.sync_a = (su - P.sync_b * sk) / n;
        P.sync_closed_form = sps >= 4096u ? 1u : 0u;
        P.strict_sync = (c.flags & LORA_HIP_FLAG_FAST_SYNC) ? 0u : 1u;
        if (const char *e = getenv("LORA_HIP_STRICT_SYNC")) P.strict_sync = (e[0] != '0') ? 1u : 0u;
        h->decoupled_policy = (c.flags & LORA_HIP_FLAG_NO_DECOUPLED) ? 0 : -1;
        if (const char *e = getenv("LORA_HIP_DECOUPLED")) h->decoupled_policy = e[0] == '0' ? 0 : e[0] == '1' ? 1 : -1;
    }
    for (uint32_t t = 0; t < N / 2u; t++) {
        const double a = -2.0 * M_PI * (double)t / (double)N;
        twN[t] = make_float2((float)std::cos(a), (float)std::sin(a));
    }
    for (uint32_t m = 0; m < sps; m++) {
        const double a = -2.0 * M_PI * (double)m / (double)sps;
        tws[m] = make_float2((float)std::cos(a), (float)std::sin(a));
    }
    lora_hip_status s;
    if ((s = upload(h, &h->d_down, down)) != LORA_HIP_OK) return s;
    if ((s = upload(h, &h->d_twN, twN)) != LORA_HIP_OK) return s;
    if ((s = upload(h, &h->d_tws, tws)) != LORA_HIP_OK) return s;
    if ((s = upload(h, &h->d_up_ifreq, up_ifreq)) != LORA_HIP_OK) return s;
    if ((s = upload(h, &h->d_down_ifreq, down_ifreq)) != LORA_HIP_OK) return s;
    if ((s = upload(h, &h->d_up_ifreq_v, up3)) != LORA_HIP_OK) return s;
    h->h_up = up; h->n_up_ifreq_v = up3.size();
    P.down = h->d_down; P.twN = h->d_twN; P.tws = h->d_tws;
    P.wave_tabs = nullptr;
    if (D == 8u && wave_tables_floats(c.sf) != 0u) {
        std::vector<float> wt(wave_tables_floats(c.sf));
        build_wave_tables(c.sf, down.data(), wt.data());
        if ((s = upload(h, &h->d_wave_tabs, wt)) != LORA_HIP_OK) return s;
        P.wave_tabs = h->d_wave_tabs;
    }
    if (wave_tables_floats_d(c.sf, D) != 0u) {
        std::vector<float> wt(wave_tables_floats_d(c.sf, D));
        build_wave_tables_d(c.sf, D, down.data(), wt.data());
        if ((s = upload(h, &h->d_wave_tabs, wt)) != LORA_HIP_OK) return s;
        P.wave_tabs = h->d_wave_tabs;
    }
    P.w3_tw = nullptr; P.w3_ctab = nullptr;
    if (D == 8u && walker3_covers(c.sf)) {
        std::vector<float2> tw(w3_tw_entries(c.sf)), ct(sps);
        build_w3_tables(c.sf, tw.data(), ct.data());
        if ((s = upload(h, &h->d_w3_tw, tw)) != LORA_HIP_OK) return s;
        if ((s = upload(h, &h->d_w3_ctab, ct)) != LORA_HIP_OK) return s;
        P.w3_tw = h->d_w3_tw; P.w3_ctab = h->d_w3_ctab;
    }
    P.team_tabs = nullptr;
    if (D == 8u && team_tables_entries(c.sf) != 0u) {
        std::vector<float2> tt(team_tables_entries(c.sf));
        build_team_tables(c.sf, down.data(), dt, (double)c.bandwidth, tt.data());
        if ((s = upload(h, &h->d_team_tabs, tt)) != LORA_HIP_OK) return s;
        P.team_tabs = reinterpret_cast<const float *>(h->d_team_tabs);
    }
    P.up_ifreq = h->d_up_ifreq; P.down_ifreq = h->d_down_ifreq; P.up_ifreq_v = h->d_up_ifreq_v;
    return LORA_HIP_OK;
}

void publish(lora_hip_decoder *h, const AttemptRec &r, StreamDesc &sd)
{
    lora_hip_frame_info_t info;
    info.stream = sd.id;
    info.length = (uint32_t)kLoratapLen + r.frame_len;
    info.header_pos = sd.abs_base + r.hdr_pos;
    info.end_pos = sd.abs_base + r.end_pos;
    uint8_t *blob = h->frames.push(info.length, info);
    blob[13] = snr_byte(sd.pwr.snr);
    std::memcpy(blob + kLoratapLen, r.frame, r.frame_len);
}

lora_hip_status run_jobs_begin(lora_hip_decoder *h, const float2 *d_iq, const std::vector<Job> &jobs, uint32_t recs_per_job,
                               uint32_t trace_cap, hipStream_t st, RunOut &out)
{
    const uint32_t nj = (uint32_t)jobs.size();
    const auto hp0 = std::chrono::steady_clock::now();
    if (h->pending.open) return fail(h, LORA_HIP_ERR_INTERNAL, "a launch is already in flight on this handle");
    h->pending = lora_hip_decoder::Pending{};
    h->pending.nj = nj; h->pending.recs_per_job = recs_per_job; h->pending.trace_cap = trace_cap; h->pending.st = st; h->pending.hp0 = hp0;
    out.rpj = recs_per_job; out.cap = recs_per_job;
    out.res.resize(nj);
    out.recs.clear();
    if (nj == 0) return LORA_HIP_OK;
    static const bool staged_bufs = getenv("LORA_HIP_STAGED") != nullptr;
    if (staged_bufs) {
        HIP_TRY(h, h->d_jobs.reserve(nj));
        HIP_TRY(h, h->d_results.reserve(nj));
        HIP_TRY(h, h->d_recs.reserve((size_t)nj * recs_per_job));
    }
    const bool need_scratch = !h->P.ifreq_in_lds_2;
    if (need_scratch) HIP_TRY(h, h->d_scratch.reserve((size_t)nj * 2u * h->P.sps));
    if (trace_cap) HIP_TRY(h, h->d_trace.reserve((size_t)nj * trace_cap));
    static const bool direct = getenv("LORA_HIP_STAGED") == nullptr;
    const uint32_t eager = direct ? recs_per_job : std::min(std::max(h->eager_recs, 2u), recs_per_job);
    HIP_TRY(h, h->p_jobs.reserve(nj));
    HIP_TRY(h, h->p_res.reserve(nj));
    HIP_TRY(h, h->p_recs.reserve((size_t)nj * eager));
    std::memcpy(h->p_jobs.p, jobs.data(), nj * sizeof(Job));
    if (!direct) HIP_TRY(h, hipMemcpyAsync(h->d_jobs.p, h->p_jobs.p, nj * sizeof(Job), hipMemcpyHostToDevice, st));
    LaunchCfg c{};
    c.iq = d_iq; c.recs_per_job = recs_per_job;
    c.jobs = direct ? h->p_jobs.p : h->d_jobs.p; c.results = direct ? h->p_res.p : h->d_results.p; c.recs = direct ? h->p_recs.p : h->d_recs.p;
    c.scratch = need_scratch ? h->d_scratch.p : nullptr;
    c.trace = trace_cap ? h->d_trace.p : nullptr; c.trace_cap = trace_cap; c.n_jobs = nj;
    static const bool no_balance = getenv("LORA_HIP_NO_BALANCE") != nullptr;
    if (!h->d_balance.p && !no_balance) {
        HIP_TRY(h, h->d_balance.reserve(kBalanceWords));
        HIP_TRY(h, hipMemsetAsync(h->d_balance.p, 0, kBalanceWords * sizeof(uint32_t), st));
    }
    c.balance = no_balance ? nullptr : h->d_balance.p;
    c.skip_payload = h->launch_skip ? 1u : 0u;
    HIP_TRY(h, hipEventRecord(h->ev0, st));
    if (nj >= h->last_kernel_jobs) { h->last_kernel = walker_kernel_name_for(h->P, nj, h->launch_skip); h->last_kernel_jobs = nj; }
    if (launch_walker(h->P, c, st) != 0) return fail(h, LORA_HIP_ERR_HIP, "walker launch failed: %s", hipGetErrorString(hipGetLastError()));
    HIP_TRY(h, hipEventRecord(h->ev1, st));
    if (!direct) {
        HIP_TRY(h, hipMemcpyAsync(h->p_res.p, h->d_results.p, nj * sizeof(JobResult), hipMemcpyDeviceToHost, st));
        HIP_TRY(h, hipMemcpy2DAsync(h->p_recs.p, eager * sizeof(AttemptRec), h->d_recs.p, recs_per_job * sizeof(AttemptRec), eager * sizeof(AttemptRec), nj,
                                    hipMemcpyDeviceToHost, st));
    }
    HIP_TRY(h, hipEventRecord(h->ev_done, st));
    h->pending.eager = eager; h->pending.direct = direct; h->pending.open = true;
    h->pending.hp1 = std::chrono::steady_clock::now();
    return LORA_HIP_OK;
}

lora_hip_status run_jobs_end(lora_hip_decoder *h, RunOut &out)
{
    if (!h->pending.open) return LORA_HIP_OK;
    h->pending.open = false;
    const uint32_t nj = h->pending.nj, recs_per_job = h->pending.recs_per_job, eager = h->pending.eager, trace_cap = h->pending.trace_cap;
    const hipStream_t st = h->pending.st;
    const auto hp0 = h->pending.hp0, hp1 = h->pending.hp1;
    const Job *jobs = h->p_jobs.p;
    HIP_TRY(h, hipEventSynchronize(h->ev_done));
    const auto hp2 = std::chrono::steady_clock::now();
    std::memcpy(out.res.data(), h->p_res.p, nj * sizeof(JobResult));
    static const bool dbg_stats = getenv("LORA_HIP_DEBUG") != nullptr;
    if (dbg_stats && h->P.use_fast) {
        double cyc[6] = {0}, rnd[6] = {0};
        for (uint32_t j = 0; j < nj; j++) for (int i = 0; i < 6; i++) { cyc[i] += 64.0 * out.res[j].cyc[i]; rnd[i] += out.res[j].rounds[i]; }
        fprintf(stderr, "[lora_hip] per-job avg kcycles (rounds): DETECT %.0f (%.1f) SYNC %.0f (%.1f) SFD %.0f (%.1f) PAUSE %.0f (%.1f) HDR %.0f (%.1f) PAYLOAD %.0f (%.1f)\n",
                cyc[0] / nj / 1e3, rnd[0] / nj, cyc[1] / nj / 1e3, rnd[1] / nj, cyc[2] / nj / 1e3, rnd[2] / nj, cyc[3] / nj / 1e3, rnd[3] / nj, cyc[4] / nj / 1e3, rnd[4] / nj, cyc[5] / nj / 1e3, rnd[5] / nj);
        {
            double na = 0, nt = 0, ntv = 0; uint32_t sr[4] = {0, 0, 0, 0}, tsr[4] = {0, 0, 0, 0}, tpad = 0;
            for (uint32_t j = 0; j < nj; j++) {
                const JobResult &r = out.res[j];
                na += r.n_attempts; sr[r.stop_reason & 3u]++;
                if (r.tail_valid) { ntv++; nt += r.tail_n_attempts; tsr[r.tail_stop_reason & 3u]++; tpad += r.tail_pad; }
            }
            fprintf(stderr, "[lora_hip] attempts/job %.2f, stop reasons %u/%u/%u/%u; tails %.0f (attempts/tail %.2f, stop reasons %u/%u/%u/%u, pending %u)\n", na / nj, sr[0], sr[1],
                    sr[2], sr[3], ntv, ntv ? nt / ntv : 0.0, tsr[0], tsr[1], tsr[2], tsr[3], tpad);
        }
        double ctl[4] = {0};
        for (uint32_t j = 0; j < nj; j++) for (int i = 0; i < 4; i++) ctl[i] += 64.0 * out.res[j].ctl[i];
        fprintf(stderr, "[lora_hip] control per job, kcycles: copy-in %.0f loop %.0f plan %.0f copy-out %.0f (walker3: demodulation %.0f, replay %.0f of the decode rounds; with LORA_W3_REPLAY_STATS=2 copy-in and symbol loop in the 3rd / 4th figure)\n", ctl[0] / nj / 1e3, ctl[1] / nj / 1e3, ctl[2] / nj / 1e3, ctl[3] / nj / 1e3, ctl[0] / nj / 1e3, ctl[1] / nj / 1e3);
        std::vector<double> tot(nj);
        for (uint32_t j = 0; j < nj; j++) { double t = 0; for (int i = 0; i < 6; i++) t += 64.0 * out.res[j].cyc[i]; tot[j] = t; }
        std::sort(tot.begin(), tot.end());
        double mean = 0; for (double t : tot) mean += t; mean /= nj;
        fprintf(stderr, "[lora_hip] job kcycles over %u jobs: min %.0f p50 %.0f p90 %.0f max %.0f mean %.0f\n", nj, tot[0] / 1e3, tot[nj / 2] / 1e3,
                tot[(size_t)(nj * 0.9)] / 1e3, tot[nj - 1] / 1e3, mean / 1e3);
    }
    if (const char *tl = getenv("LORA_HIP_JOB_TIMELINE")) {
        if (FILE *f = fopen(tl, "a")) {
            fprintf(f, "# launch of %u jobs: job hw_id xcc_id t_start t_end(100MHz) cyc[6] x64 start scan_limit n_att\n", nj);
            for (uint32_t j = 0; j < nj; j++) {
                const JobResult &r = out.res[j];
                fprintf(f, "%u %u %u %u %u %u %u %u %u %u %u %lld %lld %u %u %u %u %u\n", j, r.dbg[0], r.dbg[1], r.dbg[2], r.dbg[3], r.cyc[0], r.cyc[1], r.cyc[2], r.cyc[3], r.cyc[4], r.cyc[5],
                        (long long)jobs[j].start, (long long)jobs[j].scan_limit, r.n_attempts, r.dbg[5] - r.dbg[4], r.rounds[5], r.rounds[0], r.rounds[2]);
            }
            fclose(f);
        }
    }
    uint32_t max_att = 0;
    for (uint32_t j = 0; j < nj; j++) max_att = std::max(max_att, out.res[j].n_attempts + (out.res[j].tail_valid ? out.res[j].tail_n_attempts : 0u));
    if (max_att > recs_per_job) max_att = recs_per_job;
    const uint32_t stride = std::max(max_att, 1u);
    out.rpj = stride;
    out.recs.resize_uninit((size_t)nj * stride);
    for (uint32_t j = 0; j < nj; j++) {
        const uint32_t used = std::min(std::min(eager, max_att), out.res[j].n_attempts + (out.res[j].tail_valid ? out.res[j].tail_n_attempts : 0u));
        for (uint32_t a = 0; a < used; a++) {
            const AttemptRec *src = h->p_recs.p + (size_t)j * eager + a;
            const size_t n = offsetof(AttemptRec, frame) + std::min<size_t>(src->frame_len, sizeof src->frame);
            std::memcpy(&out.recs[(size_t)j * stride + a], src, n);
        }
    }
    if (dbg_stats && h->P.use_fast) {
        double sync_rounds = 0; uint32_t frames = 0, tails = 0, early = 0;
        for (uint32_t j = 0; j < nj; j++) {
            const JobResult &r = out.res[j];
            sync_rounds += r.rounds[1];
            const uint32_t used = std::min(std::min(eager, max_att), r.n_attempts + (r.tail_valid ? r.tail_n_attempts : 0u));
            for (uint32_t a = 0; a < used; a++) {
                const AttemptRec &t = out.recs[(size_t)j * stride + a];
                frames += (a < r.n_attempts && t.status == kAttemptFrame) ? 1u : 0u;
                if (r.tail_valid && a + 1u == r.n_attempts + r.tail_n_attempts && r.tail_pad) { tails++; early += t.status == kAttemptAtSfd ? 1u : 0u; }
            }
        }
        fprintf(stderr, "[lora_hip] acquisitions: %.0f SYNC rounds for %u frames of this launch (%.2f per frame); %u tail probes reached a packet, %u of them stopped behind their first FIND_SFD step\n",
                sync_rounds, frames, frames ? sync_rounds / frames : 0.0, tails, early);
    }
    h->eager_recs = std::min(std::max(max_att, 2u), 8u);
    bool more = false;
    if (max_att > eager) {
        HIP_TRY(h, hipMemcpy2DAsync(out.recs.data() + eager, stride * sizeof(AttemptRec), h->d_recs.p + eager,
                                    recs_per_job * sizeof(AttemptRec), (max_att - eager) * sizeof(AttemptRec), nj, hipMemcpyDeviceToHost, st));
        more = true;
    }
    if (trace_cap) {
        h->h_trace.resize((size_t)nj * trace_cap);
        HIP_TRY(h, hipMemcpyAsync(h->h_trace.data(), h->d_trace.p, (size_t)nj * trace_cap * sizeof(StepRec), hipMemcpyDeviceToHost, st));
        more = true;
    }
    if (more) HIP_TRY(h, hipStreamSynchronize(st));
    float ms = 0.0f;
    HIP_TRY(h, hipEventElapsedTime(&ms, h->ev0, h->ev1));
    if (dbg_stats) {
        const auto hp3 = std::chrono::steady_clock::now();
        auto us = [](auto a, auto b) { return std::chrono::duration<double, std::micro>(b - a).count(); };
        fprintf(stderr, "[lora_hip] run_jobs host: enqueue %.0f us, wait %.0f us (kernel %.0f us), unpack %.0f us; results %zu B + records %zu B\n", us(hp0, hp1), us(hp1, hp2),
                ms * 1e3, us(hp2, hp3), nj * sizeof(JobResult), (size_t)nj * eager * sizeof(AttemptRec));
    }
    h->timing.walker_ms += ms;
    h->timing.total_device_ms += ms;
    h->timing.walker_launches++;
    return LORA_HIP_OK;
}

lora_hip_status run_jobs(lora_hip_decoder *h, const float2 *d_iq, const std::vector<Job> &jobs, uint32_t recs_per_job, uint32_t trace_cap,
                         hipStream_t st, RunOut &out)
{
    const lora_hip_status s = run_jobs_begin(h, d_iq, jobs, recs_per_job, trace_cap, st, out);
    return s == LORA_HIP_OK ? run_jobs_end(h, out) : s;
}

void append_trace(lora_hip_decoder *h, const RunOut &out, uint32_t job_index, uint32_t trace_cap, int64_t abs_base)
{
    const JobResult &jr = out.res[job_index];
    for (uint32_t i = 0; i < jr.n_steps; i++) {
        const StepRec &s = h->h_trace[(size_t)job_index * trace_cap + i];
        lora_hip_step_t o;
        o.state = s.state; o.consumed = s.consumed; o.pos = abs_base + s.pos; o.bin = s.bin; o.fine = s.fine;
        o.value = s.value; o.stream = s.stream; o.cycles = s.cycles; o.reserved = 0;
        h->trace.push_back(o);
    }
}

uint64_t streams_signature(const std::vector<StreamDesc> &streams)
{
    uint64_t x = 1469598103934665603ull;
    for (const StreamDesc &sd : streams)
        for (uint64_t v : {sd.off, sd.len}) { x ^= v; x *= 1099511628211ull; }
    return x ^ streams.size();
}

lora_hip_status quiet_edges_enqueue(lora_hip_decoder *h, const float2 *d_iq, const std::vector<StreamDesc> &streams, hipStream_t st)
{
    const uint32_t sps = h->P.sps, ns = (uint32_t)streams.size();
    h->pre_issued = false;
    h->pre_hq0 = std::chrono::steady_clock::now();
    HIP_TRY(h, h->p_env_streams.reserve(ns));
    uint64_t nb = 0;
    for (uint32_t i = 0; i < ns; i++) {
        const uint64_t n = streams[i].len / sps;
        nb = (nb + 63u) & ~63ull;
        if (n == 0 || nb + n > 0xffffffffull) return LORA_HIP_ERR_ARG;
        h->p_env_streams.p[i] = EnvStream{streams[i].off, (uint32_t)nb, (uint32_t)n};
        nb += n;
    }
    const size_t words = (size_t)((nb + 63u) / 64u);
    HIP_TRY(h, h->d_env_E.reserve(nb));
    HIP_TRY(h, h->d_env_buf.reserve(words));
    HIP_TRY(h, h->p_env_buf.reserve(words));
    const hipStream_t ps = h->pre_stream;
    if (!h->iq_ready) {
        HIP_TRY(h, hipEventRecord(h->ev_dep, st));
        HIP_TRY(h, hipStreamWaitEvent(ps, h->ev_dep, 0));
    }
    static const bool dbg = getenv("LORA_HIP_DEBUG") != nullptr;
    if (dbg) HIP_TRY(h, hipEventRecord(h->ev_pre0, ps));
    static const bool direct = getenv("LORA_HIP_STAGED") == nullptr;
    if (launch_envelope(d_iq, h->p_env_streams.p, ns, sps, h->d_env_E.p, direct ? h->p_env_buf.p : h->d_env_buf.p, ps) != 0)
        return fail(h, LORA_HIP_ERR_HIP, "envelope launch failed: %s", hipGetErrorString(hipGetLastError()));
    if (dbg) HIP_TRY(h, hipEventRecord(h->ev_pre1, ps));
    if (!direct) HIP_TRY(h, hipMemcpyAsync(h->p_env_buf.p, h->d_env_buf.p, words * 8u, hipMemcpyDeviceToHost, ps));
    h->pre_issued = true; h->pre_iq = d_iq; h->pre_sig = streams_signature(streams); h->pre_ns = ns;
    return LORA_HIP_OK;
}

lora_hip_status quiet_edges_collect(lora_hip_decoder *h, std::vector<std::vector<int64_t>> &edges)
{
    if (!h->pre_issued) return LORA_HIP_ERR_ARG;
    h->pre_issued = false;
    const uint32_t sps = h->P.sps, ns = h->pre_ns;
    static const bool dbg = getenv("LORA_HIP_DEBUG") != nullptr;
    const auto hq0 = h->pre_hq0, hq1 = std::chrono::steady_clock::now();
    HIP_TRY(h, hipStreamSynchronize(h->pre_stream));
    const auto hq2 = std::chrono::steady_clock::now();
    if (dbg) { float ms = 0; if (hipEventElapsedTime(&ms, h->ev_pre0, h->ev_pre1) == hipSuccess) h->envelope_ms = ms; }
    edges.resize(ns);
    uint32_t n_found = 0;
    const unsigned long long *bm = h->p_env_buf.p;
    for (uint32_t i = 0; i < ns; i++) {
        std::vector<int64_t> &e = edges[i];
        e.clear();
        const uint64_t b0 = h->p_env_streams.p[i].first_block, b1 = b0 + h->p_env_streams.p[i].n_blocks;
        for (uint64_t w = b0 / 64u; w * 64u < b1; w++) {
            unsigned long long bits = bm[w];
            while (bits) {
// ... 64 lines not shown
        if (launch_demod_symbols(h->P, d_iq, h->d_offsets.p, (uint32_t)n_sym, (int)h->P.demod_mode, h->d_bins.p + ps.used, h->d_fine.p + ps.used, nullptr, st, has_alt ? &ar : nullptr) != 0)
            return fail(h, LORA_HIP_ERR_HIP, "payload pass: symbol launch failed: %s", hipGetErrorString(hipGetLastError()));
    }
    if (launch_payload_chain(h->P, h->d_bins.p, h->d_fine.p, alt, launch, h->p_pay_out.p, (uint32_t)ps.active.size(), st) != 0)
        return fail(h, LORA_HIP_ERR_HIP, "payload pass: chain launch failed: %s", hipGetErrorString(hipGetLastError()));
    HIP_TRY(h, hipEventRecord(h->ev_pay1, st));
    HIP_TRY(h, hipEventRecord(h->ev_pay_done, st));
    ps.n_sym = n_sym;
    return LORA_HIP_OK;
}

lora_hip_status payload_pass_begin(lora_hip_decoder *h, const float2 *d_iq, std::vector<PayloadReq> &reqs)
{
    lora_hip_decoder::PayState &ps = h->pay;
    ps = lora_hip_decoder::PayState{};
    const size_t np = reqs.size();
    if (np == 0) return LORA_HIP_OK;
    size_t total = 0;
    for (const PayloadReq &q : reqs) total += q.n_walk;
    ps.cap_sym = total * (size_t)kPayloadHyp;
    HIP_TRY(h, h->p_pay_off.reserve(total));
    HIP_TRY(h, h->p_pay_desc.reserve(2 * np));
    HIP_TRY(h, h->p_pay_out.reserve(np));
    HIP_TRY(h, h->d_offsets.reserve(total));
    HIP_TRY(h, h->d_bins.reserve(ps.cap_sym));
    HIP_TRY(h, h->d_fine.reserve(ps.cap_sym));
    HIP_TRY(h, h->d_alt_shift.reserve(ps.cap_sym));
    HIP_TRY(h, h->d_alt_bins.reserve(ps.cap_sym));
    HIP_TRY(h, h->d_alt_fine.reserve(ps.cap_sym));
    const int64_t sps = (int64_t)h->P.sps;
    ps.active.resize(np);
    for (size_t i = 0; i < np; i++) {
        PayloadReq &q = reqs[i];
        q.status = kPayloadUnresolved; q.end_shift = 0; q.frame_len = 0;
        PayloadDesc &d = h->p_pay_desc.p[i];
        d = PayloadDesc{};
        d.n_walk = q.n_walk; d.sk = q.sk;
        d.room = (int64_t)q.stream_len - 2 * sps - q.start;
        ps.active[i] = (uint32_t)i;
    }
    ps.open = true;
    return payload_launch_round(h, d_iq, reqs);
}

void payload_pass_abort(lora_hip_decoder *h)
{
    if (h->pay_stream) (void)hipStreamSynchronize(h->pay_stream);
    h->pay = lora_hip_decoder::PayState{};
}

lora_hip_status payload_pass_end(lora_hip_decoder *h, const float2 *d_iq, std::vector<PayloadReq> &reqs)
{
    lora_hip_decoder::PayState &ps = h->pay;
    if (!ps.open) return LORA_HIP_OK;
    ps.open = false;
    for (;;) {
        HIP_TRY(h, hipEventSynchronize(h->ev_pay_done));
        ps.used += ps.n_sym;
        h->last_payload_symbols += (uint32_t)ps.n_sym;
        h->last_payload_rounds++;
        float ms = 0.0f;
        HIP_TRY(h, hipEventElapsedTime(&ms, h->ev_pay0, h->ev_pay1));
        ps.ms += ms;
        for (size_t a = ps.active.size(); a-- > 0;) if (ps.active[a] != a) h->p_pay_out.p[ps.active[a]] = h->p_pay_out.p[a];
        std::vector<uint32_t> next;
        for (uint32_t i : ps.active) {
            PayloadReq &q = reqs[i];
            const PayloadOut &o = h->p_pay_out.p[i];
            if (o.result == kWalkComplete && o.frame_len >= 3u && o.frame_len <= (uint32_t)sizeof q.frame) {
                q.status = kPayloadDecoded; q.end_shift = o.shift; q.frame_len = o.frame_len;
                std::memcpy(q.frame, o.frame, o.frame_len);
            } else if (o.result == kWalkOutOfData) {
                q.status = kPayloadOutOfData;
            } else if (o.result == kWalkNeedShift && h->p_pay_desc.p[i].n_hyp < (uint32_t)kPayloadHyp) {
                next.push_back(i);
            }
        }
        ps.active.swap(next);
        ps.round++;
        if (ps.active.empty() || ps.round >= kPayloadHyp) break;
        const lora_hip_status s = payload_launch_round(h, d_iq, reqs);
        if (s != LORA_HIP_OK) return s;
    }
    h->last_payload_ms += ps.ms;
    h->timing.walker_ms += ps.ms;
    h->timing.total_device_ms += ps.ms;
    h->timing.walker_launches += 2;
    return LORA_HIP_OK;
}

struct DeviceEnv {
    lora_hip_decoder *h;
    const float2 *d_iq;
    hipStream_t st;
    uint32_t sps() const { return h->P.sps; }
    uint32_t ctor_cr() const { return h->P.ctor_cr; }
    uint32_t segment_symbols() const { return h->cfg.segment_symbols; }
    uint32_t resident_slots() const
    {
        if (h->resident_slots == 0) h->resident_slots = std::max<uint32_t>(walker_resident_slots(h->P), 64u);
        return h->resident_slots;
    }
    uint32_t resident_slots_alt() const
    {
        if (h->resident_slots_alt == ~0u) h->resident_slots_alt = walker_resident_slots_full(h->P);
        return h->resident_slots_alt;
    }
    bool tracing() const { return (h->cfg.flags & LORA_HIP_FLAG_TRACE) != 0; }
    bool implicit() const { return h->P.implicit != 0; }
    bool early_probe() const
    {
        static const bool off = getenv("LORA_HIP_NO_EARLY_PROBE") != nullptr;
        return !off && h->P.use_fast && h->P.decim == 8u && walker3_covers(h->P.sf);
    }
    bool decoupled(size_t n_jobs)
    {
        h->last_payload_packets = 0; h->last_payload_rerun = 0; h->last_payload_symbols = 0; h->last_payload_ms = 0.0f; h->last_payload_moved = 0; h->last_payload_rounds = 0;
        if (h->decoupled_policy == 0 || !walker_has_skip_variant(h->P) || tracing()) return false;
        if (h->decoupled_policy == 1) return true;
        if (h->dec_backoff) return false;
        const uint32_t full = resident_slots_alt() ? resident_slots_alt() : resident_slots();
        constexpr uint32_t fill = 100u;
        return 100u * (uint32_t)n_jobs <= fill * full;
    }
    void set_skip_payload(bool on) { h->launch_skip = on; }
    void abort_payload() { ::payload_pass_abort(h); }
    int run_payload_begin(std::vector<PayloadReq> &reqs) { return ::payload_pass_begin(h, d_iq, reqs) == LORA_HIP_OK ? 0 : -1; }
    int run_payload_end(std::vector<PayloadReq> &reqs) { return ::payload_pass_end(h, d_iq, reqs) == LORA_HIP_OK ? 0 : -1; }
    void count_payload(uint32_t packets, uint32_t moved, uint32_t rerun)
    {
        h->last_payload_packets += packets; h->last_payload_rerun += rerun; h->last_payload_moved += moved;
        if (rerun) h->timing.slow_path_relaunches++;
        if (h->decoupled_policy < 0 && packets >= 4u && 4u * (rerun + moved) > packets) h->dec_backoff = 32;
        static const bool dbg = getenv("LORA_HIP_DEBUG") != nullptr;
        if (dbg) fprintf(stderr, "[lora_hip] payload pass: %u packets, %u symbol reads in %u round(s), %.3f ms; %u packet(s) ended off the zero-drift grid (their jobs split there), %u handed to the complete kernels\n",
                         packets, h->last_payload_symbols, h->last_payload_rounds, h->last_payload_ms, moved, rerun);
    }
    RunOut &run_out(int which) { return h->run_out[which & 1]; }
    bool quiet_edges(const std::vector<StreamDesc> &streams, std::vector<std::vector<int64_t>> &edges)
    {
        return ::quiet_edges(h, d_iq, streams, st, edges) == LORA_HIP_OK;
    }
    int run_jobs(const std::vector<Job> &jobs, uint32_t rpj, uint32_t trace_cap, RunOut &out)
    {
        return ::run_jobs(h, d_iq, jobs, rpj, trace_cap, st, out) == LORA_HIP_OK ? 0 : -1;
    }
    int run_jobs_begin(const std::vector<Job> &jobs, uint32_t rpj, uint32_t trace_cap, RunOut &out)
    {
        return ::run_jobs_begin(h, d_iq, jobs, rpj, trace_cap, st, out) == LORA_HIP_OK ? 0 : -1;
    }
    int run_jobs_end(RunOut &out) { return ::run_jobs_end(h, out) == LORA_HIP_OK ? 0 : -1; }
    void publish(const AttemptRec &r, StreamDesc &sd) { ::publish(h, r, sd); }
    void append_trace(const RunOut &out, uint32_t job, uint32_t cap, int64_t base) { ::append_trace(h, out, job, cap, base); }
    void count_jobs(uint32_t n) { h->timing.jobs += n; h->last_kernel_jobs = 0; if (h->dec_backoff) h->dec_backoff--; }
    void count_probes(uint32_t n) { h->timing.probes += n; }
    void count_slow_path() { h->timing.slow_path_relaunches++; }
    void count_repair()
    {
        static const bool dbg = getenv("LORA_HIP_DEBUG") != nullptr;
        if (dbg) fprintf(stderr, "[lora_hip] cut repaired from the true header (no serial walk)\n");
    }
    void note_plan(bool burst_aware, size_t n_segs)
    {
        h->last_plan_burst = burst_aware ? 1u : 0u; h->last_plan_segments = (uint32_t)n_segs;
        static const bool dbg = getenv("LORA_HIP_DEBUG") != nullptr;
        if (dbg) fprintf(stderr, "[lora_hip] segment plan: %s, %zu segments (envelope kernels %.3f ms)\n", burst_aware ? "burst-aware" : "fixed grid", n_segs, burst_aware ? h->envelope_ms : 0.0f);
    }
    double walker_ms() const { return h->timing.walker_ms; }
};

lora_hip_status scheduler_failed(lora_hip_decoder *h)
{
    h->pending.open = false;
    return h->err.empty() ? fail(h, LORA_HIP_ERR_INTERNAL, "scheduler failed") : LORA_HIP_ERR_HIP;
}

lora_hip_status pass_begin(lora_hip_decoder *h, const float2 *d_iq, hipStream_t st, bool iq_ready)
{
    h->pass_iq = d_iq; h->pass_st = st;
    h->iq_ready = iq_ready;
    h->err.clear();
    DeviceEnv env{h, d_iq, st};
    const int rc = lora_hip::decode_begin(env, h->pass_streams, h->pass);
    h->iq_ready = false;
    if (rc != 0) return scheduler_failed(h);
    h->pass_open = true;
    return LORA_HIP_OK;
}

lora_hip_status pass_end(lora_hip_decoder *h)
{
    h->pass_open = false;
    h->err.clear();
    DeviceEnv env{h, h->pass_iq, h->pass_st};
    return lora_hip::decode_end(env, h->pass_streams, h->pass) == 0 ? LORA_HIP_OK : scheduler_failed(h);
}


void pipe_init(lora_hip_decoder *h, uint32_t n_channels, size_t batch)
{
    ChunkPipe &p = h->pipe;
    p.ch.assign(n_channels, ChunkPipe::Chan{});
    for (ChunkPipe::Chan &c : p.ch) c.cr = h->P.ctor_cr;
    p.batch = batch;
    p.tailcap = std::max<size_t>(batch, 4u * (size_t)h->P.sps);
    p.region = p.tailcap + batch;
}

lora_hip_status pipe_open(lora_hip_decoder *h)
{
    ChunkPipe &p = h->pipe;
    if (p.copy_st) return LORA_HIP_OK;
    HIP_TRY(h, hipStreamCreateWithFlags(&p.copy_st, hipStreamNonBlocking));
    HIP_TRY(h, hipStreamCreateWithFlags(&p.comp_st, hipStreamNonBlocking));
    HIP_TRY(h, hipEventCreateWithFlags(&p.up_ev, hipEventDisableTiming));
    HIP_TRY(h, hipEventCreateWithFlags(&p.tail_ev, hipEventDisableTiming));
    for (int i = 0; i < 2; i++) HIP_TRY(h, p.dbuf[i].reserve(p.ch.size() * p.region));
    return LORA_HIP_OK;
}

bool pipe_launchable(const lora_hip_decoder *h)
{
    for (const ChunkPipe::Chan &c : h->pipe.ch)
        if (c.fill != 0 && c.tail_len + c.fill >= 2u * (size_t)h->P.sps) return true;
    return false;
}

bool pipe_latency_due(const lora_hip_decoder *h)
{
    const ChunkPipe &p = h->pipe;
    return p.max_latency_ms > 0.0f && p.have_first && pipe_launchable(h) &&
           std::chrono::duration<float, std::milli>(std::chrono::steady_clock::now() - p.t_first).count() >= p.max_latency_ms;
}

lora_hip_status pipe_collect(lora_hip_decoder *h)
{
    ChunkPipe &p = h->pipe;
    if (!p.inflight) return LORA_HIP_OK;
    p.inflight = false;
    const lora_hip_status s = pass_end(h);
    if (s != LORA_HIP_OK) return s;
    bool any_tail = false;
    for (const StreamDesc &sd : h->pass_streams) {
        ChunkPipe::Chan &c = p.ch[sd.id];
        c.cr = sd.cr_out; c.pwr = sd.pwr;
        const size_t keep_from = (size_t)std::min<int64_t>(std::max<int64_t>(sd.final_pos, 0), (int64_t)sd.len);
        const size_t tail = sd.len - keep_from;
        c.host_base += (int64_t)keep_from;
        if (tail > p.tailcap) {
            const size_t ncap = std::max(2u * p.tailcap, tail + (size_t)h->P.sps), nregion = ncap + p.batch;
            HIP_TRY(h, hipStreamSynchronize(p.copy_st));
            HIP_TRY(h, hipStreamSynchronize(p.comp_st));
            for (int i = 0; i < 2; i++) {
                DevBuf<float2> nb;
                HIP_TRY(h, nb.reserve(p.ch.size() * nregion));
                for (size_t q = 0; q < p.ch.size(); q++)
                    HIP_TRY(h, hipMemcpyAsync(nb.p + q * nregion + (ncap - p.tailcap), p.dbuf[i].p + q * p.region, p.region * sizeof(float2), hipMemcpyDeviceToDevice, p.comp_st));
                HIP_TRY(h, hipStreamSynchronize(p.comp_st));
                std::swap(p.dbuf[i], nb);
                nb.release();
            }
            for (StreamDesc &x : h->pass_streams) x.off = (x.off / p.region) * nregion + (x.off % p.region) + (ncap - p.tailcap);
            p.tailcap = ncap; p.region = nregion;
        }
        if (tail) {
            HIP_TRY(h, hipMemcpyAsync(p.dbuf[p.cur].p + (size_t)sd.id * p.region + p.tailcap - tail, p.dbuf[p.cur ^ 1].p + sd.off + keep_from, tail * sizeof(float2),
                                      hipMemcpyDeviceToDevice, p.comp_st));
            any_tail = true;
        }
        c.tail_len = tail;
    }
    if (any_tail) {
        HIP_TRY(h, hipEventRecord(p.tail_ev, p.comp_st));
        HIP_TRY(h, hipStreamWaitEvent(p.copy_st, p.tail_ev, 0));
    }
    return LORA_HIP_OK;
}

lora_hip_status pipe_collect_if_done(lora_hip_decoder *h)
{
    lora_hip_status s = LORA_HIP_OK;
    if (h->pipe.inflight && h->pending.open && hipEventQuery(h->ev_done) == hipSuccess) s = pipe_collect(h);
    (void)hipGetLastError();
    return s;
}

lora_hip_status pipe_rotate(lora_hip_decoder *h, bool by_latency)
{
    ChunkPipe &p = h->pipe;
    HIP_TRY(h, hipEventRecord(p.up_ev, p.copy_st));
    lora_hip_status s = pipe_collect(h);
    if (s != LORA_HIP_OK) return s;
    std::vector<StreamDesc> &sds = h->pass_streams;
    sds.clear();
    for (uint32_t c = 0; c < p.ch.size(); c++) {
        ChunkPipe::Chan &C = p.ch[c];
        const size_t len = C.tail_len + C.fill;
        if (len < 2u * (size_t)h->P.sps) continue;
        StreamDesc sd{};
        sd.off = (uint64_t)c * p.region + p.tailcap - C.tail_len; sd.len = len; sd.id = c;
        sd.cr_in = C.cr; sd.pwr = C.pwr; sd.abs_base = C.host_base;
        sds.push_back(sd);
    }
    if (sds.empty()) return LORA_HIP_OK;
    HIP_TRY(h, hipStreamWaitEvent(p.comp_st, p.up_ev, 0));
    h->timing = lora_hip_timing_t{};
    for (const StreamDesc &sd : sds) h->timing.items += sd.len;
// ... 770 lines not shown
    struct Cand { uint32_t stream; int64_t k, e, a0; int32_t bin; float pmr; size_t b_first, b_n; };
    std::vector<Cand> cands;
    std::vector<int64_t> boffs;
    for (uint32_t s = 0; s < n_streams; s++) {
        const lora_hip_window_stats_t *W = A.data() + first[s];
        const int64_t K = (int64_t)(first[s + 1] - first[s]), len = (int64_t)stream_len[s];
        int64_t k = 0;
        while (k < K) {
            if (!(pmr(W[k].peak_down, W[k].total_down) >= thr)) { k++; continue; }
            int64_t e = k + 1;
            while (e < K && pmr(W[e].peak_down, W[e].total_down) >= thr && circ(W[e].bin_down, W[e - 1].bin_down) <= 1) e++;
            if (e - k >= kMinRun) {
                int32_t best = W[k].bin_down; int64_t best_n = 0;
                for (int64_t i = k; i < e; i++) {
                    int64_t c = 0;
                    for (int64_t j = k; j < e; j++) c += W[j].bin_down == W[i].bin_down;
                    if (c > best_n || (c == best_n && W[i].bin_down < best)) { best_n = c; best = W[i].bin_down; }
                }
                float pm = 0.0f;
                for (int64_t i = k; i < e; i++) pm += pmr(W[i].peak_down, W[i].total_down);
                int64_t a0 = k * sps - (int64_t)best * D;
                if (a0 < 0) a0 += sps;
                Cand c{s, k, e, a0, best, pm / (float)(e - k), boffs.size(), 0};
                for (int64_t j = 0; j <= (e - k) + kSfdReach; j++) {
                    const int64_t p = a0 + j * sps;
                    if (p + sps > len) break;
                    boffs.push_back((int64_t)stream_off[s] + p);
                    c.b_n++;
                }
                cands.push_back(c);
            }
            k = e;
        }
    }
    std::vector<lora_hip_window_stats_t> B;
    rc = window_stats_abs(h, (const float2 *)d_iq, boffs, B, st);
    if (rc != LORA_HIP_OK) return rc;
    struct Hit { size_t cand; int64_t found; size_t c_first, c_n; int64_t j0, j1; };
    std::vector<Hit> hits;
    std::vector<int64_t> coffs;
    constexpr int64_t kRefineWindows = 6;
    int64_t skip_until = -1; uint32_t skip_stream = 0xffffffffu;
    for (size_t ci = 0; ci < cands.size(); ci++) {
        const Cand &c = cands[ci];
        if (c.stream == skip_stream && c.k < skip_until) continue;
        const lora_hip_window_stats_t *W = B.data() + c.b_first;
        int64_t found = -1;
        for (size_t j = 0; j + 1 < c.b_n; j++) {
            if (pmr(W[j].peak_up, W[j].total_up) >= thr && W[j].peak_up > W[j].peak_down && pmr(W[j + 1].peak_up, W[j + 1].total_up) >= thr &&
                W[j + 1].peak_up > W[j + 1].peak_down) { found = (int64_t)j; break; }
        }
        if (found < 0) continue;
        Hit hit{ci, found, coffs.size(), 0, std::max<int64_t>(0, found - 2 - kRefineWindows), found - 2};
        while (hit.j0 < hit.j1 && c.a0 + hit.j0 * sps - D / 2 < 0) hit.j0++;
        for (int64_t dl = -(D / 2); dl <= D / 2 && hit.j0 < hit.j1; dl++)
            for (int64_t j = hit.j0; j < hit.j1; j++) { coffs.push_back((int64_t)stream_off[c.stream] + c.a0 + j * sps + dl); hit.c_n++; }
        hits.push_back(hit);
        skip_stream = c.stream; skip_until = (c.a0 + (found + 2) * sps) / sps;
    }
    std::vector<lora_hip_window_stats_t> Cst;
    rc = window_stats_abs(h, (const float2 *)d_iq, coffs, Cst, st);
    if (rc != LORA_HIP_OK) return rc;
    size_t n_out = 0;
    bool overflow = false;
    for (const Hit &hit : hits) {
        const Cand &c = cands[hit.cand];
        const lora_hip_window_stats_t *W = B.data() + c.b_first;
        int64_t delta = 0;
        if (hit.c_n) {
            const int64_t nj = hit.j1 - hit.j0, nd = D + 1;
            std::vector<double> P((size_t)nd, 0.0);
            for (int64_t i = 0; i < nd; i++)
                for (int64_t j = 0; j < nj; j++) {
                    const lora_hip_window_stats_t &w = Cst[hit.c_first + (size_t)(i * nj + j)];
                    if (w.bin_down == 0) P[(size_t)i] += (double)w.peak_down;
                }
            double best = -1.0;
            for (int64_t i = 0; i < nd; i++) {
                const double v = P[(size_t)i] + (i >= 1 ? P[(size_t)i - 1] : 0.0) + (i + 1 < nd ? P[(size_t)i + 1] : 0.0);
                const int64_t d = i - D / 2;
                const bool closer = std::llabs(d) < std::llabs(delta) || (std::llabs(d) == std::llabs(delta) && d < delta);
                if (v > best || (v == best && closer)) { best = v; delta = d; }
            }
            if (!(best > 0.0)) delta = 0;
        }
        const int64_t found = hit.found;
        const int32_t bu = W[found].bin_up, sb = bu < N / 2 ? bu : bu - (int32_t)N;
        if (n_out < cap) {
            lora_hip_preamble_t &o = out[n_out];
            o.header_pos = c.a0 + delta + found * sps + 2 * sps + sps / 4; o.run_pos = c.k * sps; o.stream = c.stream; o.run_len = (uint32_t)(c.e - c.k);
            o.bin = c.bin; o.sfd_index = (int32_t)found; o.pmr = c.pmr; o.cfo_bins = -0.5f * (float)sb;
            o.cfo_hz = o.cfo_bins * (float)h->cfg.bandwidth / (float)N; o.delta = (int32_t)delta;
        } else overflow = true;
        n_out++;
    }
    *n_found = n_out;
    return overflow ? LORA_HIP_ERR_OVERFLOW : LORA_HIP_OK;
}

lora_hip_status lora_hip_decode_at_headers_device(lora_hip_decoder_t *h, const void *d_iq, size_t total_items, const uint64_t *stream_off,
                                                  const uint64_t *stream_len, uint32_t n_streams, const lora_hip_preamble_t *pre, size_t n, void *hip_stream)
{
    if (!h || !d_iq || !n_streams || !stream_off || !stream_len || (n && !pre)) return LORA_HIP_ERR_ARG;
    if (h->pass_open) return fail(h, LORA_HIP_ERR_ARG, "lora_hip_decode_at_headers_device: a pass is open on this handle");
    if (h->P.implicit) return fail(h, LORA_HIP_ERR_BAD_CONFIG, "decode at given headers needs an explicit header (the implicit mode's energy threshold comes from DETECT)");
    if (n == 0) return LORA_HIP_OK;
    HIP_TRY(h, hipSetDevice(h->device));
    std::vector<Job> jobs(n, Job{});
    for (size_t i = 0; i < n; i++) {
        const uint32_t s = pre[i].stream;
        if (s >= n_streams || stream_off[s] > total_items || stream_len[s] > total_items - stream_off[s]) return fail(h, LORA_HIP_ERR_ARG, "entry %zu: bad stream", i);
        if (pre[i].header_pos < 0 || (uint64_t)pre[i].header_pos + 2u * h->P.sps > stream_len[s]) return fail(h, LORA_HIP_ERR_ARG, "entry %zu: header position outside its stream", i);
        Job &j = jobs[i];
        j.stream_off = stream_off[s]; j.stream_len = stream_len[s]; j.stream_id = s;
        j.start = pre[i].header_pos; j.scan_limit = pre[i].header_pos;
        j.cr_prev = h->P.ctor_cr; j.max_attempts = 1; j.start_at_header = 1;
    }
    h->err.clear();
    h->timing = lora_hip_timing_t{};
    RunOut &out = h->run_out[0];
    const lora_hip_status rc = run_jobs(h, (const float2 *)d_iq, jobs, 2, 0, (hipStream_t)hip_stream, out);
    if (rc != LORA_HIP_OK) return rc;
    for (size_t i = 0; i < n; i++) {
        if (out.res[i].n_attempts == 0 || out.rpj == 0) continue;
        const AttemptRec &r = out.rec(i, 0);
        if (r.status != kAttemptFrame) continue;
        StreamDesc sd{};
        sd.id = jobs[i].stream_id; sd.abs_base = 0;
        publish(h, r, sd);
    }
    return LORA_HIP_OK;
}

lora_hip_status lora_hip_last_plan(const lora_hip_decoder_t *h, uint32_t *burst_aware, uint32_t *segments)
{
    if (!h) return LORA_HIP_ERR_ARG;
    if (burst_aware) *burst_aware = h->last_plan_burst;
    if (segments) *segments = h->last_plan_segments;
    return LORA_HIP_OK;
}

lora_hip_status lora_hip_last_payload_pass(const lora_hip_decoder_t *h, uint32_t *packets, uint32_t *moved, uint32_t *rerun, uint32_t *rounds, uint32_t *symbols, float *ms)
{
    if (!h) return LORA_HIP_ERR_ARG;
    if (packets) *packets = h->last_payload_packets;
    if (moved) *moved = h->last_payload_moved;
    if (rounds) *rounds = h->last_payload_rounds;
    if (rerun) *rerun = h->last_payload_rerun;
    if (symbols) *symbols = h->last_payload_symbols;
    if (ms) *ms = h->last_payload_ms;
    return LORA_HIP_OK;
}

const char *lora_hip_walker_kernel_name(const lora_hip_decoder_t *h) { return h ? (h->last_kernel ? h->last_kernel : walker_kernel_name(h->P)) : ""; }

lora_hip_status lora_hip_last_timing(const lora_hip_decoder_t *h, lora_hip_timing_t *t)
{
    if (!h || !t) return LORA_HIP_ERR_ARG;
    *t = h->timing;
    return LORA_HIP_OK;
}

size_t lora_hip_trace(const lora_hip_decoder_t *h, const lora_hip_step_t **steps)
{
    if (!h || !steps) return 0;
    *steps = h->trace.data();
    return h->trace.size();
}

void lora_hip_trace_clear(lora_hip_decoder_t *h)
{
    if (h) h->trace.clear();
}

}
```

### gr_lora_amd/csrc/lora_walker2.inc.hip

```cpp

constexpr int kW2DetectK = 4;
#ifndef LORA_W2_WAVES_SF7
#define LORA_W2_WAVES_SF7 8
#endif
#ifndef LORA_W2_WAVES_SF8
#define LORA_W2_WAVES_SF8 8
#endif
#ifndef LORA_W2_SFD_K
#define LORA_W2_SFD_K 2
#endif
#ifndef LORA_W2_EU_SF8
#define LORA_W2_EU_SF8 4
#endif
constexpr int kW2MaxWaves = LORA_W2_WAVES_SF7 > LORA_W2_WAVES_SF8 ? LORA_W2_WAVES_SF7 : LORA_W2_WAVES_SF8;

constexpr int kW2SfdK = LORA_W2_SFD_K;

enum W2Mode : int32_t { kPlanExit = 0, kPlanDetect, kPlanSync, kPlanSfd, kPlanPause, kPlanDecode, kPlanFinalize };

struct alignas(16) W2Plan {
    int64_t pos;
    int32_t mode;
    int32_t buf;
    int32_t resolve_prev;
    int32_t n_win;
    int32_t prev_n;
    int32_t zmode;
};

struct alignas(16) W2State {
    int64_t  pos, att_start, att_trig, att_hdr;
    int32_t  state, done, stop_reason, in_attempt;
    uint32_t corr_fails, cr, has_crc, payload_length;
    int32_t  payload_symbols;
    uint32_t n_words, n_cw, n_sym;
    uint32_t n_att, npush, n_steps, frame_ok;
    uint32_t att_cr_prev, att_ambig;
    float    energy_threshold;
    float    push_tail[4];
    uint8_t  phdr[4];
    uint32_t fin_pending, fin_n_bytes, fin_plen;
    int32_t  fin_st, fin_consumed, fin_bin, fin_fine;
};

struct alignas(16) W2Stats {
    long long prev_t;
    int32_t   prev_state;
    uint32_t  cyc[6], rounds[6], ctl[4];
};

struct alignas(16) W2Shared {
    float    red[kW2MaxWaves * 72 + 8];
    float    specf[kW2MaxWaves][4];
    float    detf[kW2MaxWaves * kW2DetectK][4];
    int32_t  detn[kW2MaxWaves];
    int32_t  speci[2][kW2MaxWaves][4];
    W2Plan   plan[2];
    Shared   sh;
    W2State  st;
    W2Stats  stats;
    int64_t  ph_start;
    uint32_t ph_go, ph_cr, ph_natt, ph_pad;
    uint32_t det_streak;
    uint32_t prio;
    uint32_t words_pk[2];
    strict::Cands sc;
    uint32_t words_pk16[4];
};

struct W2Tabs {
    const float  *v;
    const float  *dd;
    float        *scratch;
};

template <int WAVES>
__device__ __forceinline__ void w2_block_argmax_first(float &v, int &idx, float *red)
{
    const int lane = threadIdx.x & 63, wave = threadIdx.x >> 6;
#pragma unroll
    for (int o = 32; o > 0; o >>= 1) {
        const float ov = __shfl_xor(v, o, 64);
        const int oi = __shfl_xor(idx, o, 64);
        if (ov > v || (ov == v && oi < idx)) { v = ov; idx = oi; }
    }
    __syncthreads();
    if (lane == 0) { red[wave] = v; ((int *)red)[16 + wave] = idx; }
    __syncthreads();
    v = red[0]; idx = ((int *)red)[16];
#pragma unroll
    for (int w = 1; w < WAVES; w++) {
        const float ov = red[w];
        const int oi = ((int *)red)[16 + w];
        if (ov > v || (ov == v && oi < idx)) { v = ov; idx = oi; }
    }
}

__device__ __forceinline__ bool w2_pre_step(W2State &S, const Job &job, uint32_t rec_cap, uint32_t sps)
{
    if (S.state == kDetect && !S.in_attempt) {
        if (S.pos >= job.scan_limit) { S.stop_reason = 0; S.done = 1; return false; }
        if (S.n_att >= rec_cap) { S.stop_reason = 2; S.done = 1; return false; }
        if (job.max_attempts && S.n_att >= job.max_attempts) { S.stop_reason = 3; S.done = 1; return false; }
    }
    if (S.pos + 2 * (int64_t)sps > (int64_t)job.stream_len) { S.stop_reason = 1; S.done = 1; return false; }
    return true;
}

template <bool KEEP_SFD = false>
__device__ __forceinline__ void w2_end_step(W2State &S, const Job &job, const LaunchCfg &C, AttemptRec *recs, StepRec *trace, int32_t st_in,
                            int32_t consumed, int32_t step_bin, int32_t fine, float step_val, long long t_start, bool lead = true)
{
    if (trace && lead && S.n_steps < C.trace_cap) {
        StepRec &s = trace[S.n_steps];
        s.state = st_in; s.consumed = consumed; s.pos = S.pos; s.bin = step_bin; s.fine = fine; s.value = step_val;
        s.stream = job.stream_id; s.cycles = (uint32_t)(clock64() - t_start); s.pad = 0;
    }
    S.n_steps++;
    S.pos += consumed;
    if (S.in_attempt && S.state == kDetect) {
        if (lead) {
            AttemptRec &r = recs[S.n_att];
            r.status = S.frame_ok ? kAttemptFrame : kAttemptLostSync;
            if (!S.frame_ok) r.frame_len = 0;
            r.start_pos = S.att_start; r.trig_pos = S.att_trig; r.hdr_pos = S.att_hdr; r.end_pos = S.pos;
            r.npush = S.npush;
            for (int i = 0; i < 4; i++) r.push_tail[i] = S.push_tail[i];
            r.cr_prev = S.att_cr_prev; r.hdr_ambig = S.att_ambig; r.n_symbols = S.n_sym;
            if constexpr (!KEEP_SFD) r.n_sfd = 0;
        }
        S.n_att++;
        S.in_attempt = 0;
        S.frame_ok = 0;
        S.npush = 0;
        S.att_start = S.pos;
    } else if (S.in_attempt && job.stop_at_header && S.state == kDecodeHeader) {
        S.stop_reason = 3;
        S.done = 1;
    }
}

template <bool WAVE = false, bool W16 = false>
__device__ __forceinline__ bool w2_post_symbol(const DevParams &P, W2State &S, Shared &sh, uint32_t bin_idx, bool is_first, uint32_t *wpk = nullptr, bool do_demod = true)
{
    const bool reduced = is_first || P.reduced_rate;
    bool block_done = false;
    if (do_demod) {
    if (reduced) bin_idx = (uint32_t)lroundf((float)bin_idx / 4.0f) & (P.nbins_hdr - 1u);
    const uint32_t word = bin_idx ^ (bin_idx >> 1u);
    const uint32_t need = 4u + (is_first ? 4u : S.cr);
    if constexpr (WAVE && W16) {
        const uint32_t sh16 = 16u * (S.n_words & 1u), ins = (word & 0xffffu) << sh16, keep = ~(0xffffu << sh16), q = S.n_words >> 1;
        if (q == 0u) wpk[0] = (wpk[0] & keep) | ins;
        else if (q == 1u) wpk[1] = (wpk[1] & keep) | ins;
        else if (q == 2u) wpk[2] = (wpk[2] & keep) | ins;
        else if (q == 3u) wpk[3] = (wpk[3] & keep) | ins;
    } else
    if constexpr (WAVE) {
        const uint32_t sh8 = 8u * (S.n_words & 3u), ins = (word & 0xffu) << sh8, keep = ~(0xffu << sh8);
        if (S.n_words < 4u) wpk[0] = (wpk[0] & keep) | ins;
        else if (S.n_words < 8u) wpk[1] = (wpk[1] & keep) | ins;
    } else {
        if (S.n_words < 16u) sh.words[S.n_words] = word;
    }
    S.n_words++;
    S.n_sym++;
    if (S.n_words == need) {
        const uint32_t ppm = reduced ? P.sf - 2u : P.sf;
        uint32_t tmp = S.n_cw;
        if constexpr (WAVE && W16) { const uint32_t w4[4] = {wpk[0], wpk[1], wpk[2], wpk[3]}; deinterleave_block_wave16(sh, w4, need, ppm, tmp); }
        else if constexpr (WAVE) deinterleave_block_wave(sh, ((uint64_t)wpk[1] << 32) | wpk[0], need, ppm, tmp);
        else deinterleave_block(sh, need, ppm, tmp);
        S.n_cw = (S.n_cw + ppm <= (uint32_t)kMaxCodewords) ? S.n_cw + ppm : (uint32_t)kMaxCodewords;
        S.n_words = 0;
        block_done = true;
    }
    }
    if (is_first) {
        if (block_done && P.implicit) {
            S.payload_symbols = 1;
            S.state = kDecodePayload;
        } else
        if (block_done) {
            uint8_t hA[3], hB[3], h0[3] = {0, 0, 0};
            decode_header_bytes(sh, S.n_cw, 2, hA);
            decode_header_bytes(sh, S.n_cw, 1, hB);
            const uint8_t *use = (S.cr >= 3u) ? hA : (S.cr >= 1u ? hB : h0);
            S.att_ambig = (uint32_t)((hA[0] != hB[0]) || (hA[1] != hB[1]) || (hA[2] != hB[2]));
            S.phdr[0] = use[0]; S.phdr[1] = use[1]; S.phdr[2] = use[2];
            const uint32_t rem = S.n_cw > 5u ? S.n_cw - 5u : 0u;
            for (uint32_t i = 0; i < rem; i++) sh.cw[i] = sh.cw[i + 5u];
            S.n_cw = rem;
            if ((S.phdr[1] >> 5) > 4) S.phdr[1] = (uint8_t)((S.phdr[1] & 0x1f) | (4u << 5));
            S.cr = S.phdr[1] >> 5;
            S.has_crc = (S.phdr[1] >> 4) & 1u;
            S.payload_length = (uint32_t)S.phdr[0] + 2u * S.has_crc;
            const uint32_t redundancy = P.reduced_rate ? 2u : 0u;
            const int symbols_per_block = (int)S.cr + 4;
            const float bits_needed = (float)S.payload_length * 8.0f;
            const float symbols_needed = bits_needed * ((float)symbols_per_block / 4.0f) / (float)(P.sf - redundancy);
            const int blocks_needed = (int)ceilf(symbols_needed / (float)symbols_per_block);
            S.payload_symbols = blocks_needed * symbols_per_block;
            S.state = kDecodePayload;
        }
        return false;
    }
    if (block_done && !P.implicit) S.payload_symbols -= (int32_t)(4u + S.cr);
    if (S.payload_symbols <= 0) {
        uint32_t n_bytes;
        if (S.cr >= 3u) n_bytes = (uint32_t)ceilf((float)S.n_cw * 4.0f / (4.0f + (float)S.cr));
        else n_bytes = (S.n_cw + 1u) / 2u;
        if (n_bytes > (uint32_t)(kMaxCodewords / 2 + 8)) n_bytes = kMaxCodewords / 2 + 8;
        S.fin_n_bytes = n_bytes;
        S.fin_plen = S.payload_length > 257u ? 257u : S.payload_length;
        return true;
    }
    return false;
}

template <int SF>
// ... 107 lines not shown
    if (lane == 63) { g0 += (double)f[J - 1]; g1 += (double)(SPS - 1) * (double)f[J - 1]; }
    {
#pragma unroll
        for (int o = 32; o > 0; o >>= 1) { g0 += __shfl_xor(g0, o, 64); g1 += __shfl_xor(g1, o, 64); }
    }
    if (lane >= 1 && lane <= 32) scr[lane - 1] = f[0];
    if (lane >= 31) scr[32 + 1 + (63 - lane)] = f[J - 1];
    if (lane == 63) scr[32] = f[J - 1];
    __builtin_amdgcn_wave_barrier();
    asm volatile("s_waitcnt lgkmcnt(0)" ::: "memory");
    const int i = lane - 31;
    float ps = scr[lane];
#pragma unroll
    for (int o = 1; o < 32; o <<= 1) {
        const float up = __shfl_up(ps, o, 32);
        if ((lane & 31) >= o) ps += up;
    }
    const float hsum = __shfl(ps, lane < 31 ? 30 - lane : 0, 64);
    float c_i = -3.0e38f;
    bool in_range = lane <= 62;
    if constexpr (SEARCH < 32) in_range = in_range && i > -SEARCH && i < SEARCH;
    if (in_range) {
        const double a = sync_a, b = sync_b;
        const double wd = (double)Tv[2 * SPS - 1] - (a + b * (double)(SPS - 1));
        double edge;
        float wrap_f;
        if (i >= 0) {
            edge = i > 0 ? -(double)ps : 0.0;
            wrap_f = scr[32 + i];
        } else {
            edge = (double)hsum;
            wrap_f = scr[-i - 1];
        }
        c_i = (float)(a * g0 + b * ((double)i * g0 + g1) + b * (double)SPS * edge + wd * (double)wrap_f);
    }
    int li = lane;
#pragma unroll
    for (int o = 32; o > 0; o >>= 1) {
        const float ov = __shfl_xor(c_i, o, 64);
        const int oi = __shfl_xor(li, o, 64);
        if (ov > c_i || (ov == c_i && oi < li)) { c_i = ov; li = oi; }
    }
    const int32_t lag = (c_i > 0.0f) ? li - 31 : 0;
    return W2SfdOut{c, -lag, 0};
}

template <int SF, int WAVES>
__device__ __attribute__((noinline)) void w2_sync_closed_form(const float *f2, double *pre, double sync_a, double sync_b, float &bv, int &bi, float &b2, int &i2)
{
    constexpr uint32_t sps = 8u << SF, kW2 = 64u * WAVES;
    const int wave = threadIdx.x >> 6, lane = threadIdx.x & 63;
                constexpr uint32_t NCH = 2u * sps / 4u < 256u ? 2u * sps / 4u : 256u, CH = 2u * sps / NCH, n = sps - 1u;
                double sF = 0.0, sG = 0.0;
                if (threadIdx.x < NCH) {
    #pragma unroll
                    for (uint32_t q = 0; q < CH; q += 4u) {
                        const uint32_t t = threadIdx.x * CH + q;
                        const float4 fv = *reinterpret_cast<const float4 *>(f2 + t);
                        const double tc = (double)((int)t - (int)sps);
                        sF += ((double)fv.x + (double)fv.y) + ((double)fv.z + (double)fv.w);
                        sG += tc * (double)fv.x + (tc + 1.0) * (double)fv.y + (tc + 2.0) * (double)fv.z + (tc + 3.0) * (double)fv.w;
                    }
                }
                double iF = sF, iG = sG;
    #pragma unroll
                for (int o = 1; o < 64; o <<= 1) {
                    const double uF = __shfl_up(iF, o, 64), uG = __shfl_up(iG, o, 64);
                    if (lane >= o) { iF += uF; iG += uG; }
                }
                if (threadIdx.x < NCH && lane == 63) { pre[2u * NCH + wave] = iF; pre[2u * NCH + 4u + wave] = iG; }
                __syncthreads();
                if (threadIdx.x < NCH) {
                    double oF = iF - sF, oG = iG - sG;
                    for (int w = 0; w < wave; w++) { oF += pre[2u * NCH + w]; oG += pre[2u * NCH + 4u + w]; }
                    pre[threadIdx.x] = oF; pre[NCH + threadIdx.x] = oG;
                }
                __syncthreads();
                constexpr uint32_t R = (sps + kW2 - 1u) / kW2;
                const uint32_t i0 = threadIdx.x * R;
                bv = 0.0f;
                bi = 0x7fffffff;
                b2 = 0.0f;
                i2 = 0x7fffffff;
                if (sps % kW2 != 0u && i0 >= sps) return;
                auto prefix_at = [&](uint32_t j, double &F, double &G) {
                    const uint32_t c = j / CH;
                    F = pre[c]; G = pre[NCH + c];
                    for (uint32_t t = c * CH; t < j; t++) { const double fv = (double)f2[t]; F += fv; G += (double)((int)t - (int)sps) * fv; }
                };
                double F0, G0, F1, G1;
                prefix_at(i0, F0, G0);
                prefix_at(i0 + n, F1, G1);
                double s0 = F1 - F0, s1 = (G1 - G0) + (double)((int)sps - (int)i0) * s0;
    #pragma unroll
                for (uint32_t r = 0; r < R; r++) {
                    const uint32_t i = i0 + r;
                    if (sps % kW2 != 0u && i >= sps) break;
                    const float c = (float)(sync_a * s0 + sync_b * s1);
                    if (c > bv) { b2 = bv; i2 = bi; bv = c; bi = (int)i; }
                    else if (c > b2) { b2 = c; i2 = (int)i; }
                    const double fin = (double)f2[i + n], fout = (double)f2[i];
                    s0 += fin - fout;
                    s1 += (double)n * fin - s0;
                }
}

template <int SF, int WAVES>
__device__ __attribute__((noinline)) void w2_sync_exact_ifreq(const float2 *__restrict__ x, float *f2)
{
    constexpr int SPS = 8 << SF, kW2 = 64 * WAVES, NI = 2 * SPS / kW2;
    static_assert(NI * kW2 == 2 * SPS, "whole samples per thread");
    typedef __attribute__((address_space(3))) float lds_f;
    lds_f *fl = (lds_f *)f2;
    float2 xv[NI];
    float am[NI], an[NI];
#pragma unroll
    for (int k = 0; k < NI; k++) xv[k] = x[threadIdx.x + (uint32_t)k * kW2];
#pragma unroll
    for (int k = 0; k < NI; k++) { am[k] = strict::fd_atan2f(xv[k].y, xv[k].x); fl[threadIdx.x + (uint32_t)k * kW2] = am[k]; }
    __syncthreads();
#pragma unroll
    for (int k = 0; k < NI; k++) { const uint32_t i = threadIdx.x + (uint32_t)k * kW2; an[k] = fl[i + 1u < 2u * SPS ? i + 1u : i]; }
    __syncthreads();
#pragma unroll
    for (int k = 0; k < NI; k++) fl[threadIdx.x + (uint32_t)k * kW2] = strict::ref_ifreq(am[k], an[k]);
}

#ifndef LORA_W2_ZM_ATTR
#define LORA_W2_ZM_ATTR __forceinline__
#endif
template <int SF, int SEARCH = 32>
__device__ LORA_W2_ZM_ATTR W2SfdOut w2_sfd_window_zm(const float2 *p, const float *Tv, const float *Tdd, float *scr, float down_ifreq_sd, float down_ifreq_dsum, double sync_a, double sync_b)
{
    return w2_sfd_window<SF, true, SEARCH>(p, Tv, Tdd, scr, down_ifreq_sd, down_ifreq_dsum, sync_a, sync_b);
}
template <int SF> constexpr bool kW2Alias = SF == 8;
struct W2DemodZ { uint32_t s; int32_t fine; float en; };
template <int SF, bool GRAD, int LD = 3>
__device__ LORA_W2_ZM_ATTR W2DemodZ w2_demod_zm(uint32_t enable_fine_sync, uint32_t demod_mode, bool want_energy, WaveTabs T, const float2 *x)
{
    DevParams Q{};
    Q.enable_fine_sync = enable_fine_sync; Q.demod_mode = demod_mode;
    W2DemodZ r{0u, 0, 0.0f};
    if constexpr (LD != 3 || SF < 7) {
        if constexpr (GRAD) wave_demod_symbol_grad_d<SF, LD, true>(Q, T.v, x, want_energy, r.s, r.fine, r.en);
        else wave_demod_symbol_d<SF, LD, true>(Q, T, x, r.s, r.fine, want_energy ? &r.en : nullptr);
    } else
    if constexpr (GRAD) wave_demod_symbol_grad<SF, true>(Q, T.v, x, want_energy, r.s, r.fine, r.en);
    else wave_demod_symbol<SF, 0, true>(Q, T, x, r.s, r.fine, want_energy ? &r.en : nullptr);
    return r;
}
template <int SF, int LD> constexpr uint32_t w2_table_entries() { if constexpr (LD == 3 && SF >= 7) return WaveGeom<SF>::n_ent; else return WaveGeomD<SF, LD>::n_ent; }

template <int SF, int WAVES, bool GRAD, bool SKIP = false, int LD = 3>
__device__ __forceinline__ void walker2_body(const DevParams &P, const LaunchCfg &C)
{
    constexpr int N = 1 << SF, SPS = N << LD;
    constexpr int GSF = SF + LD - 3;
    constexpr uint32_t NENT = w2_table_entries<SF, LD>();
    constexpr int kW2 = 64 * WAVES, kW2Workers = WAVES - 1;
    constexpr int kW2Win = kW2Workers;
    static_assert(kW2Win <= kW2MaxWaves, "speci is sized for kW2MaxWaves windows");
    static_assert(WAVES <= kW2MaxWaves, "W2Shared is sized for kW2MaxWaves wavefronts");
    constexpr uint32_t sps = SPS;
    extern __shared__ __attribute__((aligned(16))) unsigned char smem[];
    W2Shared &W = *reinterpret_cast<W2Shared *>(smem);
    W2State &S = W.st;
    Shared &sh = W.sh;
    constexpr bool ALIAS = kW2Alias<SF> && !GRAD && LD == 3;
    constexpr uint32_t NV = (3u * SPS + 40u + 3u) & ~3u;
    float *lds0 = reinterpret_cast<float *>(smem + ((sizeof(W2Shared) + 15) & ~(size_t)15));
    float *vl = ALIAS ? lds0 : lds0 + 2 * SPS;
    float *ddl = vl + NV;
    v2f *tab2 = reinterpret_cast<v2f *>(ddl + SPS);
    float *f2 = ALIAS ? reinterpret_cast<float *>(tab2) : lds0;
    double *pre = ALIAS ? reinterpret_cast<double *>(f2 + 2 * SPS)
                        : reinterpret_cast<double *>(tab2 + (GRAD ? 0u : NENT));
    static_assert(!ALIAS || (2u * SPS * 4u + (2u * 256u + 8u) * 8u <= NENT * 8u), "SYNC's work areas fit the table block");

    const uint32_t jid = blockIdx.x;
    if (jid >= C.n_jobs) return;
    Job job = C.jobs[jid];
    if constexpr (SF == 7) job = uniform_job(job);
    uint32_t rec_cap = C.recs_per_job;
    const float2 *__restrict__ X = C.iq + job.stream_off;
    const int64_t n_items = (int64_t)job.stream_len;
    AttemptRec *recs = C.recs + (size_t)jid * C.recs_per_job;
    StepRec *trace = C.trace ? C.trace + (size_t)jid * C.trace_cap : nullptr;
    const int wave = threadIdx.x >> 6, lane = threadIdx.x & 63;
    const bool is_ctl = wave == kW2Workers;
    const bool t0 = threadIdx.x == kW2Workers * 64;
    if (is_ctl) __builtin_amdgcn_s_setprio(2);

    const uint32_t dbg_t0 = (uint32_t)__builtin_amdgcn_s_memrealtime(), dbg_c0 = (uint32_t)(clock64() >> 6);
    WaveTabs FT{};
    if constexpr (GRAD) {
        for (uint32_t i = threadIdx.x; i < 3u * sps + 40u; i += kW2) vl[i] = P.up_ifreq_v[i];
        FT.v = vl;
    } else {
        if constexpr (LD == 3 && SF >= 7) FT = wave_tabs_to_lds<SF>(P, tab2, vl, kW2);
        else FT = wave_tabs_to_lds_d<SF, LD>(P, tab2, vl, kW2);
    }
    for (uint32_t i = threadIdx.x; i < sps; i += kW2) ddl[i] = P.down_ifreq[i] - P.down_ifreq_avg;

    auto plan_from = [&](W2State &S, W2Plan &pl, bool zreq = false ) {
        pl.buf = 0; pl.resolve_prev = 0; pl.n_win = kW2Workers; pl.pos = S.pos; pl.prev_n = 0; pl.zmode = zreq ? 1 : 0;
        if (!S.done) (void)w2_pre_step(S, job, rec_cap, sps);
        if (S.done) { pl.mode = kPlanExit; return; }
        if (S.fin_pending) { pl.mode = kPlanFinalize; return; }
        if (S.state != kDetect) W.det_streak = 0u;
        switch (S.state) {
        case kDetect:
            pl.mode = kPlanDetect; pl.n_win = W.det_streak++ == 0u ? 1 : kW2DetectK;
            return;
        case kSync: pl.mode = kPlanSync; break;
        case kFindSfd: pl.mode = kPlanSfd; break;
        case kPause: pl.mode = kPlanPause; break;
        default:
            pl.mode = kPlanDecode; pl.n_win = kW2Win;
            if (S.state == kDecodePayload && !P.implicit) {
                const int32_t rem = S.payload_symbols - (int32_t)S.n_words;
                pl.n_win = rem < kW2Win ? (rem > 0 ? rem : 1) : kW2Win;
            }
            break;
        }
    };
    auto plan_from_state = [&](W2Plan &pl) { plan_from(S, pl); };

    W2Tabs T{vl, ddl, W.red};
    uint32_t *bal_mine = nullptr, *bal_other = nullptr;
    uint32_t bal_rem = 0xffffffffu, bal_seen = 0u, bal_slot = 0u;
    if (t0) W.prio = 0u;
    if (t0 && C.balance) {
        const uint32_t hw = __builtin_amdgcn_s_getreg((31 << 11) | 4), xcc = __builtin_amdgcn_s_getreg((31 << 11) | 20);
        const uint32_t cu = ((xcc & 7u) << 8) | ((hw >> 8) & 0xffu);
        bal_slot = atomicAdd(&C.balance[2u * kBalanceCus + cu], 1u) & 1u;
        bal_mine = C.balance + 2u * cu + bal_slot;
        bal_other = C.balance + 2u * cu + (bal_slot ^ 1u);
    }
    for (int phase = 0; phase < 2; phase++) {
    if (t0) {
        S = W2State{};
        S.state = kDetect; S.pos = job.start; S.cr = job.cr_prev; S.has_crc = P.ctor_crc;
        S.phdr[1] = (uint8_t)((P.ctor_cr << 5) | (P.ctor_crc << 4));
        S.att_start = job.start; S.att_trig = -1; S.att_hdr = -1; S.att_cr_prev = job.cr_prev;
        if (job.start_at_header && phase == 0) { S.state = kDecodeHeader; S.in_attempt = 1; S.att_trig = job.start; S.att_hdr = job.start; }
        if (phase == 0) W.stats = W2Stats{};
        W.stats.prev_state = -1;
        W.det_streak = 0u;
        plan_from_state(W.plan[0]);
    }

    for (uint32_t it = 0;; it++) {
        __syncthreads();
        const W2Plan &pl_in = W.plan[it & 1u];
        const uint64_t pl_pp = (uint64_t)pl_in.pos;
        const int64_t plan_pos = (int64_t)(((uint64_t)__builtin_amdgcn_readfirstlane((uint32_t)(pl_pp >> 32)) << 32) | __builtin_amdgcn_readfirstlane((uint32_t)pl_pp));
        const int32_t plan_mode = __builtin_amdgcn_readfirstlane(pl_in.mode), plan_buf = __builtin_amdgcn_readfirstlane(pl_in.buf);
        const int32_t plan_resolve_prev = __builtin_amdgcn_readfirstlane(pl_in.resolve_prev), plan_n_win = __builtin_amdgcn_readfirstlane(pl_in.n_win);
        const int32_t plan_prev_n = __builtin_amdgcn_readfirstlane(pl_in.prev_n), plan_z = __builtin_amdgcn_readfirstlane(pl_in.zmode);
        W2Plan &next = W.plan[(it + 1u) & 1u];
        if (plan_mode == kPlanExit) break;
        const int64_t pos = plan_pos;
        const long long t_start = clock64();
        if (t0) {
            W2Stats &Q = W.stats;
            const int sidx = plan_mode == kPlanDetect ? 0 : plan_mode == kPlanSync ? 1 : plan_mode == kPlanSfd ? 2 : plan_mode == kPlanPause ? 3 : 5;
            if (Q.prev_state >= 0) { Q.cyc[Q.prev_state] += (uint32_t)((t_start - Q.prev_t) >> 6); Q.rounds[Q.prev_state]++; }
            Q.prev_state = sidx; Q.prev_t = t_start;
        }
        if (t0 && bal_mine) {
            W.prio = (bal_rem > bal_seen || (bal_rem == bal_seen && bal_slot != 0u)) ? 1u : 0u;
            const int64_t target = phase == 0 ? job.scan_limit + (job.probe_limit > job.scan_limit ? 12 * (int64_t)sps : 0) : pos + 6 * (int64_t)sps;
            const int64_t left = (target - pos) / (int64_t)sps;
            bal_rem = left < 1 ? 1u : (left > 0x3fffffff ? 0x3fffffffu : (uint32_t)left);
            __hip_atomic_store(bal_mine, bal_rem, __ATOMIC_RELAXED, __HIP_MEMORY_SCOPE_AGENT);
            bal_seen = __hip_atomic_load(bal_other, __ATOMIC_RELAXED, __HIP_MEMORY_SCOPE_AGENT);
        }
        if (!is_ctl) {
            if (W.prio) __builtin_amdgcn_s_setprio(1); else __builtin_amdgcn_s_setprio(0);
        }
        const int64_t wpos = pos + (int64_t)wave * sps;

        if (plan_mode == kPlanDetect) {
            const int kd = plan_n_win;
            if (!is_ctl) {
                const int64_t dpos = pos + (int64_t)wave * kd * sps;
                int nvalid = 0;
                if (dpos + 2 * (int64_t)sps <= n_items) {
                    const int64_t fit = (n_items - dpos) / (int64_t)sps - 1;
                    nvalid = fit < kd ? (int)fit : kd;
                }
                float a[kW2DetectK][4];
                if (nvalid > 0) {
                    if (kd == 1) { const float4 r = w2_detect_window<GSF>(X + dpos); a[0][0] = r.x; a[0][1] = r.y; a[0][2] = r.z; a[0][3] = r.w; }
                    else w2_detect_windows<GSF, kW2DetectK>(X + dpos, nvalid, a);
                }
                if (lane == 0) {
                    W.detn[wave] = nvalid;
                    for (int i = 0; i < kW2DetectK; i++)
                        if (i < nvalid) { float *o = W.detf[wave * kW2DetectK + i]; o[0] = a[i][0]; o[1] = a[i][1]; o[2] = a[i][2]; o[3] = a[i][3]; }
                }
            }
            __syncthreads();
            if (is_ctl) {
                constexpr int NWmax = kW2Workers * kW2DetectK;
                static_assert(NWmax <= 64, "one lane per DETECT window");
                const int NW = kW2Workers * kd;
                const int q = lane;
                const int qw = q / kd, qi = q - qw * kd;
                const bool valid = q < NW && qi < W.detn[qw];
                float autocorr = 0.0f, pushed = 0.0f, e2 = 0.0f;
                if (valid) {
                    const float *o = W.detf[qw * kW2DetectK + qi];
                    const float d0 = o[0], d1 = o[1], e1 = o[2];
                    e2 = o[3];
                    pushed = e1 / (float)sps;
                    const float sq = sqrtf(e1 * e2);
                    autocorr = hypotf(d0 / sq, d1 / sq);
                }
                const unsigned long long vmask = __ballot(valid), tmask = __ballot(valid && autocorr >= 0.90f);
                W.red[q] = pushed; W.red[64 + q] = e2; W.red[128 + q] = autocorr;
                __builtin_amdgcn_wave_barrier();
                if (t0) {
                    W2State L = S;
                    int64_t n_lim = (job.scan_limit - L.pos + (int64_t)sps - 1) / (int64_t)sps;
                    if (n_lim < 1) n_lim = 1;
                    const int n_valid = (~vmask == 0ull) ? 64 : __builtin_ctzll(~vmask);
                    int n_max = n_valid < NW ? n_valid : NW;
                    if ((int64_t)n_max > n_lim) n_max = (int)n_lim;
                    const int qt = tmask ? __builtin_ctzll(tmask) : 64;
                    const bool trig = qt < n_max;
                    const int nd = trig ? qt + 1 : n_max;
                    if (nd > 0) {
                        if (trace) {
                            for (int i = 0; i < nd; i++) {
                                if (L.n_steps + (uint32_t)i < C.trace_cap) {
                                    StepRec &r = trace[L.n_steps + (uint32_t)i];
                                    r.state = kDetect; r.consumed = (trig && i == nd - 1) ? 0 : (int32_t)sps; r.pos = L.pos + (int64_t)i * sps; r.bin = -1; r.fine = 0;
                                    r.value = W.red[128 + i]; r.stream = job.stream_id; r.cycles = (uint32_t)(clock64() - t_start); r.pad = 0;
                                }
                            }
                        }
                        for (int i = (nd > 4 ? nd - 4 : 0); i < nd; i++) {
                            const float pv = W.red[i];
                            if (L.npush >= 4u) { L.push_tail[0] = L.push_tail[1]; L.push_tail[1] = L.push_tail[2]; L.push_tail[2] = L.push_tail[3]; L.push_tail[3] = pv; }
                            else {
                                const uint32_t k = L.npush;
                                if (k == 0u) L.push_tail[0] = pv; else if (k == 1u) L.push_tail[1] = pv; else if (k == 2u) L.push_tail[2] = pv; else L.push_tail[3] = pv;
                            }
                            L.npush++;
                        }
                        if (nd > 4) L.npush += (uint32_t)(nd - 4);
                        L.energy_threshold = W.red[64 + nd - 1] / 2.0f;
                        L.n_steps += (uint32_t)nd;
                        L.pos += (int64_t)(trig ? nd - 1 : nd) * sps;
                        if (trig) {
                            L.corr_fails = 0u;
                            L.state = kSync;
                            L.in_attempt = 1;
                            L.att_trig = L.pos; L.att_hdr = -1; L.att_cr_prev = L.cr; L.att_ambig = 0; L.n_sym = 0;
                        }
                    }
                    W2Plan np;
                    plan_from(L, np);
                    next = np; S = L;
                }
            }
            continue;
        }

        if (plan_mode == kPlanSync) {
            const float2 *__restrict__ x = X + pos;
            if (P.strict_sync) {
                w2_sync_exact_ifreq<GSF, WAVES>(x, f2);
            } else {
                constexpr int NI = (2 * SPS + kW2 - 1) / kW2;
                float2 xb[NI], xa[NI];
#pragma unroll
                for (int k = 0; k < NI; k++) {
                    const uint32_t i = 1u + threadIdx.x + (uint32_t)k * kW2;
                    if (i < 2u * sps) { xb[k] = x[i - 1]; xa[k] = x[i]; }
                }
                __builtin_amdgcn_sched_group_barrier(0x020, 2 * NI, 0);
                __builtin_amdgcn_sched_group_barrier(0x002, 64 * NI, 0);
#pragma unroll
                for (int k = 0; k < NI; k++) {
                    const uint32_t i = 1u + threadIdx.x + (uint32_t)k * kW2;
                    if (i < 2u * sps) f2[i - 1] = ifreq_prod_z(xb[k], xa[k]);
                }
            }
            __syncthreads();
            if (t0) { f2[2u * sps - 1u] = f2[2u * sps - 2u]; strict::cands_reset(W.sc); }
            __syncthreads();
            float bv, b2;
            int bi, i2;
            w2_sync_closed_form<GSF, WAVES>(f2, pre, P.sync_a, P.sync_b, bv, bi, b2, i2);
            const float my_bv = bv;
            const int my_bi = bi;
            w2_block_argmax_first<WAVES>(bv, bi, W.red);
            if (P.strict_sync) {
                strict::cands_push(W.sc, bv, my_bv, my_bi, b2, i2);
                __syncthreads();
                const int nc = W.sc.n;
                if (nc >= 2 && nc <= strict::kK) {
                    float ev;
                    if constexpr (SF == 7 && LD == 3) bi = strict::resolve_lds_inl<kW2>(f2, SPS, vl, &W.sc, reinterpret_cast<float *>(pre), 1024, &ev);
                    else bi = strict::resolve_lds<kW2>(f2, SPS, vl, &W.sc, reinterpret_cast<float *>(pre), 1024, &ev);
                    bv = ev;
                }
            }
            if (t0) {
                const int32_t consumed = (bi == 0x7fffffff) ? 0 : bi;
                W2State L = S;
                L.state = kFindSfd;
                w2_end_step(L, job, C, recs, trace, kSync, consumed, -1, 0, bv, t_start);
                W2Plan np;
                plan_from(L, np);
                next = np; S = L;
            }
            if constexpr (ALIAS) {
                __syncthreads();
                const v2f *__restrict__ src = reinterpret_cast<const v2f *>(P.wave_tabs);
                for (uint32_t i = threadIdx.x; i < NENT; i += kW2) tab2[i] = src[i];
            }
            continue;
        }

        if (plan_mode == kPlanSfd) {
            constexpr int kSfdWin = kW2SfdK * kW2Workers;
            static_assert(kW2SfdK <= 2 && kSfdWin <= 64, "results go to specf[w][k] / speci[k][w]");
#pragma unroll
            for (int k = 0; k < kW2SfdK; k++) {
                const int64_t kpos = wpos + (int64_t)k * kW2Workers * sps;
                const bool kvalid = !is_ctl && wave < plan_n_win && kpos + 2 * (int64_t)sps <= n_items;
                float c = 0.0f;
                int32_t fine = 0;
                int32_t pz = 0;
                if (kvalid) {
                    const W2SfdOut r = plan_z ? w2_sfd_window_zm<GSF, (4 << LD)>(X + kpos, T.v, T.dd, T.scratch + wave * 72, P.down_ifreq_sd, P.down_ifreq_dsum, P.sync_a, P.sync_b)
                                              : w2_sfd_window<GSF, false, (4 << LD)>(X + kpos, T.v, T.dd, T.scratch + wave * 72, P.down_ifreq_sd, P.down_ifreq_dsum, P.sync_a, P.sync_b);
                    c = r.c; fine = r.fine; pz = r.pz;
                }
                if (lane == 0 && !is_ctl) { W.specf[wave][k] = c; W.speci[k][wave][0] = kvalid ? 1 : 0; W.speci[k][wave][1] = fine; W.speci[k][wave][2] = pz; }
            }
            __syncthreads();
            if (is_ctl) {
                W2State L = S;
                const int qw = lane % kW2Workers, qk = lane / kW2Workers;
                const float my_c = lane < kSfdWin ? W.specf[qw][qk] : 0.0f;
                const int32_t my_v = lane < kSfdWin ? W.speci[qk][qw][0] : 0, my_f = lane < kSfdWin ? W.speci[qk][qw][1] : 0;
                const int32_t my_p = lane < kSfdWin ? W.speci[qk][qw][2] : 0;
                asm volatile("s_waitcnt lgkmcnt(0)" ::: "memory");
                bool zreq = false;
                for (int w = 0; w < kSfdWin; w++) {
                    if (w > 0 && !w2_pre_step(L, job, rec_cap, sps)) break;
                    if (!__builtin_amdgcn_readlane(my_v, w)) break;
                    if (__builtin_amdgcn_readlane(my_p, w)) { zreq = true; break; }
                    const float cw = __builtin_bit_cast(float, __builtin_amdgcn_readlane(__builtin_bit_cast(int32_t, my_c), w));
                    int32_t fw = 0;
                    if (cw > 0.96f) {
                        L.state = kPause;
                    } else {
                        if (cw < -0.97f) fw = __builtin_amdgcn_readlane(my_f, w);
                        else L.corr_fails++;
                        if (L.corr_fails > 4u) L.state = kDetect;
                    }
                    w2_end_step(L, job, C, recs, trace, kFindSfd, (int32_t)sps + fw, -1, fw, cw, t_start, t0);
                    if (L.state != kFindSfd || L.done || fw != 0) break;
                }
                if (L.state == kPause && !L.done && w2_pre_step(L, job, rec_cap, sps)) {
                    L.state = kDecodeHeader;
                    const int32_t consumed = (int32_t)(sps + sps / 4u);
                    L.att_hdr = L.pos + consumed;
                    w2_end_step(L, job, C, recs, trace, kPause, consumed, -1, 0, 0.0f, t_start, t0);
                }
                W2Plan np;
                plan_from(L, np, zreq);
                if (t0) { next = np; S = L; }
            }
            continue;
        }

        if (plan_mode == kPlanPause) {
            if (t0) {
                S.state = kDecodeHeader;
                const int32_t consumed = (int32_t)(sps + sps / 4u);
                S.att_hdr = S.pos + consumed;
                w2_end_step(S, job, C, recs, trace, kPause, consumed, -1, 0, 0.0f, t_start);
                plan_from_state(next);
            }
            continue;
        }

        if (plan_mode == kPlanFinalize) {
            const uint32_t n_cw = S.n_cw, cr = S.cr, n_bytes = S.fin_n_bytes, plen = S.fin_plen;
            decode_payload_bytes(sh, n_cw, cr, n_bytes);
            AttemptRec &r = recs[S.n_att];
            for (uint32_t i = threadIdx.x; i < plen; i += kW2) r.frame[3u + i] = (i < n_bytes) ? sh.dec[i] : 0;
            __syncthreads();
            if (t0) {
                r.frame[0] = S.phdr[0]; r.frame[1] = S.phdr[1]; r.frame[2] = S.phdr[2];
                r.frame_len = 3u + plen;
                S.frame_ok = 1;
                S.state = kDetect;
                S.n_words = 0; S.n_cw = 0;
                S.fin_pending = 0;
                w2_end_step(S, job, C, recs, trace, S.fin_st, S.fin_consumed, S.fin_bin, S.fin_fine, 0.0f, t_start);
                plan_from_state(next);
            }
            continue;
        }

        int64_t dpos = pos;
        int32_t dn = plan_n_win;
        if (plan_resolve_prev && plan_prev_n > 0) {
            const int rb = plan_buf ^ 1;
            const int32_t s_l = lane < plan_prev_n ? W.speci[rb][lane][0] : -1, f_l = lane < plan_prev_n ? W.speci[rb][lane][1] : 0;
            const unsigned long long moved = __ballot(s_l >= 0 && f_l != 0);
            if (moved) {
                const int wq = __builtin_ctzll(moved);
                const int32_t redo = plan_prev_n - (wq + 1);
                dpos = pos - (int64_t)redo * sps + (int64_t)__builtin_amdgcn_readlane(f_l, wq);
                dn = plan_n_win + redo < kW2Win ? plan_n_win + redo : kW2Win;
            }
        }
        if (!is_ctl) {
            {
                const int widx = wave;
                const int64_t dwpos = dpos + (int64_t)widx * sps;
                const bool dvalid = widx < dn && dwpos + 2 * (int64_t)sps <= n_items;
                uint32_t ws = 0;
                int32_t wfine = 0;
                float wen = 0.0f;
                if (dvalid) {
                    if (plan_z) {
                        const W2DemodZ z = w2_demod_zm<SF, GRAD, LD>(P.enable_fine_sync, P.demod_mode, P.implicit != 0u, FT, X + dwpos);
                        ws = z.s; wfine = z.fine; wen = z.en;
                    } else
                    if constexpr (LD != 3 || SF < 7) {
                        if constexpr (GRAD) wave_demod_symbol_grad_d<SF, LD>(P, FT.v, X + dwpos, P.implicit != 0u, ws, wfine, wen);
                        else wave_demod_symbol_d<SF, LD>(P, FT, X + dwpos, ws, wfine, P.implicit != 0u ? &wen : nullptr);
                    } else
                    if constexpr (GRAD) wave_demod_symbol_grad<SF>(P, FT.v, X + dwpos, P.implicit != 0u, ws, wfine, wen);
                    else wave_demod_symbol<SF, kWaveFmode<SF>>(P, FT, X + dwpos, ws, wfine, P.implicit != 0u ? &wen : nullptr);
                }
                if (lane == 0) { W.speci[plan_buf][widx][0] = dvalid ? (int32_t)ws : -1; W.speci[plan_buf][widx][1] = wfine; W.speci[plan_buf][widx][2] = __builtin_bit_cast(int32_t, wen); }
            }
        } else {
            bool predicted = true, zreq = false;
            const long long tr0 = clock64();
            constexpr bool W16 = SF > 8;
            uint32_t wpk[W16 ? 4 : 2];
            if constexpr (W16) { wpk[0] = W.words_pk16[0]; wpk[1] = W.words_pk16[1]; wpk[2] = W.words_pk16[2]; wpk[3] = W.words_pk16[3]; }
            else { wpk[0] = W.words_pk[0]; wpk[1] = W.words_pk[1]; }
            W2State L = S;
            asm volatile("s_waitcnt lgkmcnt(0)" ::: "memory");
            const long long tr1 = clock64();
            if (plan_resolve_prev) {
                const int rb = plan_buf ^ 1;
                const int32_t my_s = lane < kW2Win ? W.speci[rb][lane][0] : -1, my_f = lane < kW2Win ? W.speci[rb][lane][1] : 0;
                const int32_t my_e = (P.implicit != 0u && lane < kW2Win) ? W.speci[rb][lane][2] : 0;
                for (int w = 0; w < kW2Win; w++) {
                    if (w > 0 && !w2_pre_step(L, job, rec_cap, sps)) break;
                    const int32_t sw = __builtin_amdgcn_readlane(my_s, w);
                    int32_t fw = __builtin_amdgcn_readlane(my_f, w);
                    if (!(L.state == kDecodeHeader || L.state == kDecodePayload)) break;
                    if (sw == (int32_t)kPoisonBin) { zreq = true; break; }
                    if (sw < 0) break;
                    const bool is_first = L.state == kDecodeHeader;
                    const int32_t st_w = L.state;
                    const uint32_t sres = (uint32_t)sw;
                    uint32_t bin_idx = GRAD ? sres : ((sres == 0u && P.demod_mode == 2u) ? 0u : (sres + (uint32_t)N - 1u) % (uint32_t)N);
                    int32_t step_bin = (int32_t)bin_idx;
                    bool do_demod = true;
                    if (P.implicit != 0u && !is_first) {
                        const float ew = __builtin_bit_cast(float, __builtin_amdgcn_readlane(my_e, w));
                        if (ew < L.energy_threshold) { L.payload_symbols = 0; L.payload_length = L.n_cw / 2u; do_demod = false; bin_idx = 0u; step_bin = -1; fw = 0; }
                    }
                    if (w2_post_symbol<true, W16>(P, L, sh, bin_idx, is_first, wpk, do_demod)) {
                        L.fin_pending = 1; L.fin_st = st_w; L.fin_consumed = (int32_t)sps + fw; L.fin_bin = step_bin; L.fin_fine = fw;
                        break;
                    }
                    w2_end_step(L, job, C, recs, trace, st_w, (int32_t)sps + fw, step_bin, fw, 0.0f, t_start, t0);
                    if constexpr (SKIP) {
                        if (is_first && L.state == kDecodePayload && !L.done) {
                            AttemptRec &r = recs[L.n_att];
                            if (t0) {
                                SkippedPayload sk;
                                sk.phdr[0] = L.phdr[0]; sk.phdr[1] = L.phdr[1]; sk.phdr[2] = L.phdr[2];
                                sk.n_left = (uint8_t)(L.n_cw < 8u ? L.n_cw : 8u);
                                for (uint32_t i = 0; i < 8u; i++) sk.left[i] = i < L.n_cw ? sh.cw[i] : (uint8_t)0;
                                sk.payload_symbols = L.payload_symbols;
                                *reinterpret_cast<SkippedPayload *>(r.frame) = sk;
                            }
                            const int32_t n_walk = L.payload_symbols > 0 ? L.payload_symbols : 1;
                            L.state = kDetect; L.frame_ok = 0; L.n_words = 0; L.n_cw = 0;
                            w2_end_step(L, job, C, recs, nullptr, kDecodePayload, n_walk * (int32_t)sps, -1, 0, 0.0f, t_start, t0);
                            if (t0) { r.status = kAttemptHeaderOnly; r.frame_len = (uint32_t)sizeof(SkippedPayload); }
                            break;
                        }
                    }
                    if (L.done || fw != 0) break;
                }
                predicted = !zreq && !L.done && !L.fin_pending && (L.state == kDecodeHeader || L.state == kDecodePayload) && L.pos == dpos &&
                            w2_pre_step(L, job, rec_cap, sps);
            }
            const long long tr2 = clock64();
            W2Plan np;
            if (predicted) {
                int32_t n_next = kW2Win;
                if (L.state == kDecodePayload && !P.implicit) {
                    const int32_t rem = L.payload_symbols - (int32_t)L.n_words - dn;
                    n_next = rem < kW2Win ? (rem > 0 ? rem : 0) : kW2Win;
                }
                np.mode = kPlanDecode; np.pos = dpos + (int64_t)dn * sps; np.buf = plan_buf ^ 1; np.resolve_prev = 1; np.n_win = n_next;
                np.prev_n = dn; np.zmode = 0;
            } else {
                plan_from(L, np, zreq);
            }
            const long long tr3 = clock64();
            if (t0) {
                next = np;
                S = L;
                if constexpr (W16) { W.words_pk16[0] = wpk[0]; W.words_pk16[1] = wpk[1]; W.words_pk16[2] = wpk[2]; W.words_pk16[3] = wpk[3]; }
                else { W.words_pk[0] = wpk[0]; W.words_pk[1] = wpk[1]; }
                asm volatile("s_waitcnt lgkmcnt(0)" ::: "memory");
                W.stats.ctl[0] += (uint32_t)((tr1 - tr0) >> 6); W.stats.ctl[1] += (uint32_t)((tr2 - tr1) >> 6); W.stats.ctl[2] += (uint32_t)((tr3 - tr2) >> 6);
                W.stats.ctl[3] += (uint32_t)((clock64() - tr3) >> 6);
                W.stats.cyc[4] += (uint32_t)((clock64() - tr0) >> 6); W.stats.rounds[4]++;
            }
        }
    }

    __syncthreads();
    if (t0) {
        const bool in_attempt = S.in_attempt != 0;
        if (in_attempt && S.n_att < rec_cap) {
            AttemptRec &r = recs[S.n_att];
            r.status = (S.stop_reason == 3) ? kAttemptAtHeader : kAttemptOutOfData;
            r.start_pos = S.att_start; r.trig_pos = S.att_trig; r.hdr_pos = S.att_hdr; r.end_pos = S.pos;
            r.npush = S.npush;
            for (int i = 0; i < 4; i++) r.push_tail[i] = S.push_tail[i];
            r.cr_prev = S.att_cr_prev; r.hdr_ambig = S.att_ambig; r.n_symbols = S.n_sym; r.frame_len = 0; r.n_sfd = 0;
        }
        JobResult &jr = C.results[jid];
        const int64_t e_pos = in_attempt ? S.att_start : S.pos;
        const uint32_t e_natt = S.n_att + (in_attempt ? 1u : 0u), e_npush = in_attempt ? 0u : S.npush, e_pad = in_attempt ? 1u : 0u;
        bool go = false;
        if (phase == 0) {
            jr.final_pos = e_pos;
            jr.n_attempts = e_natt;
            jr.final_cr = S.cr;
            jr.npush = e_npush;
            for (int i = 0; i < 4; i++) jr.push_tail[i] = S.push_tail[i];
            jr.stop_reason = (uint32_t)S.stop_reason;
            jr.n_steps = S.n_steps < C.trace_cap ? S.n_steps : C.trace_cap;
            jr.pad = e_pad;
            jr.tail_valid = 0;
            go = job.probe_limit > job.scan_limit && S.stop_reason == 0 && !in_attempt && !trace && e_natt < C.recs_per_job;
            W.ph_go = go ? 1u : 0u; W.ph_start = e_pos; W.ph_cr = S.cr; W.ph_natt = e_natt; W.ph_pad = 0;
        } else {
            jr.tail_valid = 1; jr.tail_first_rec = W.ph_natt;
            jr.tail_final_pos = e_pos; jr.tail_n_attempts = e_natt; jr.tail_final_cr = S.cr; jr.tail_npush = e_npush;
            for (int i = 0; i < 4; i++) jr.tail_push_tail[i] = S.push_tail[i];
            jr.tail_stop_reason = (uint32_t)S.stop_reason; jr.tail_pad = e_pad; jr.tail_rsv = 0;
        }
        if (!go) {
            W2Stats &Q = W.stats;
            if (Q.prev_state >= 0) { Q.cyc[Q.prev_state] += (uint32_t)((clock64() - Q.prev_t) >> 6); Q.rounds[Q.prev_state]++; }
            for (int i = 0; i < 6; i++) { jr.cyc[i] = Q.cyc[i]; jr.rounds[i] = Q.rounds[i]; }
            for (int i = 0; i < 4; i++) jr.ctl[i] = Q.ctl[i];
            jr.dbg[0] = __builtin_amdgcn_s_getreg((31 << 11) | 4); jr.dbg[1] = __builtin_amdgcn_s_getreg((31 << 11) | 20);
            jr.dbg[2] = dbg_t0; jr.dbg[3] = (uint32_t)__builtin_amdgcn_s_memrealtime();
            jr.dbg[4] = dbg_c0; jr.dbg[5] = (uint32_t)(clock64() >> 6);
        }
    }
    if (phase == 1) break;
    __syncthreads();
    if (!W.ph_go) break;
    bal_rem = 0xffffffffu;
    {
        const int64_t st = W.ph_start;
        const uint32_t lo = __builtin_amdgcn_readfirstlane((uint32_t)st), hi = __builtin_amdgcn_readfirstlane((uint32_t)((uint64_t)st >> 32));
        const uint32_t natt = __builtin_amdgcn_readfirstlane(W.ph_natt);
        job.start = (int64_t)(((uint64_t)hi << 32) | lo);
        job.cr_prev = __builtin_amdgcn_readfirstlane(W.ph_cr);
        job.scan_limit = job.probe_limit; job.stop_at_header = 1; job.max_attempts = 0;
        recs += natt;
        rec_cap = C.recs_per_job - natt;
    }
    __syncthreads();
    }
    if (t0 && bal_mine) __hip_atomic_store(bal_mine, 0u, __ATOMIC_RELAXED, __HIP_MEMORY_SCOPE_AGENT);
}

constexpr int kW2WavesSf7 = LORA_W2_WAVES_SF7, kW2WavesSf8 = LORA_W2_WAVES_SF8;
__global__ __launch_bounds__(64 * kW2WavesSf7, 4) void walker2_kernel_sf7(DevParams P, LaunchCfg C) { walker2_body<7, kW2WavesSf7, false>(P, C); }
__global__ __launch_bounds__(64 * kW2WavesSf8, LORA_W2_EU_SF8) void walker2_kernel_sf8(DevParams P, LaunchCfg C) { walker2_body<8, kW2WavesSf8, false>(P, C); }
__global__ __launch_bounds__(64 * kW2WavesSf8, 2) void walker2_kernel_sf8_wide(DevParams P, LaunchCfg C) { walker2_body<8, kW2WavesSf8, false>(P, C); }
__global__ __launch_bounds__(64 * kW2WavesSf7, 2) void walker2_kernel_sf7_wide(DevParams P, LaunchCfg C) { walker2_body<7, kW2WavesSf7, false>(P, C); }
__global__ __launch_bounds__(64 * kW2WavesSf7, 2) void walker2_kernel_sf7_grad_wide(DevParams P, LaunchCfg C) { walker2_body<7, kW2WavesSf7, true>(P, C); }
__global__ __launch_bounds__(64 * kW2WavesSf8, 2) void walker2_kernel_sf8_grad_wide(DevParams P, LaunchCfg C) { walker2_body<8, kW2WavesSf8, true>(P, C); }
#ifndef LORA_W2_EU_GRAD_SF7
#define LORA_W2_EU_GRAD_SF7 4
#endif
#ifndef LORA_W2_EU_GRAD_SF8
#define LORA_W2_EU_GRAD_SF8 4
#endif
__global__ __launch_bounds__(64 * kW2WavesSf7, LORA_W2_EU_GRAD_SF7) void walker2_kernel_sf7_grad(DevParams P, LaunchCfg C) { walker2_body<7, kW2WavesSf7, true>(P, C); }
__global__ __launch_bounds__(64 * kW2WavesSf8, LORA_W2_EU_GRAD_SF8) void walker2_kernel_sf8_grad(DevParams P, LaunchCfg C) { walker2_body<8, kW2WavesSf8, true>(P, C); }
__global__ __launch_bounds__(64 * kW2WavesSf7, 4) void walker2_kernel_sf7_skip(DevParams P, LaunchCfg C) { walker2_body<7, kW2WavesSf7, false, true>(P, C); }
__global__ __launch_bounds__(64 * kW2WavesSf8, 2) void walker2_kernel_sf8_skip(DevParams P, LaunchCfg C) { walker2_body<8, kW2WavesSf8, false, true>(P, C); }
__global__ __launch_bounds__(64 * kW2WavesSf7, LORA_W2_EU_GRAD_SF7) void walker2_kernel_sf7_grad_skip(DevParams P, LaunchCfg C) { walker2_body<7, kW2WavesSf7, true, true>(P, C); }
__global__ __launch_bounds__(64 * kW2WavesSf8, LORA_W2_EU_GRAD_SF8) void walker2_kernel_sf8_grad_skip(DevParams P, LaunchCfg C) { walker2_body<8, kW2WavesSf8, true, true>(P, C); }

#define LORA_W2_DECIM_KERNEL(SFV, DV, LDV, EU) \
    __global__ __launch_bounds__(512, EU) void walker2_kernel_sf##SFV##_d##DV(DevParams P, LaunchCfg C) { walker2_body<SFV, 8, false, false, LDV>(P, C); } \
    __global__ __launch_bounds__(512, EU) void walker2_kernel_sf##SFV##_d##DV##_grad(DevParams P, LaunchCfg C) { walker2_body<SFV, 8, true, false, LDV>(P, C); }
LORA_W2_DECIM_KERNEL(7, 2, 1, 4)
LORA_W2_DECIM_KERNEL(7, 4, 2, 4)
LORA_W2_DECIM_KERNEL(8, 2, 1, 4)
LORA_W2_DECIM_KERNEL(8, 4, 2, 4)
LORA_W2_DECIM_KERNEL(9, 2, 1, 4)
LORA_W2_DECIM_KERNEL(9, 4, 2, 2)
LORA_W2_DECIM_KERNEL(6, 4, 2, 4)
LORA_W2_DECIM_KERNEL(6, 8, 3, 4)
#undef LORA_W2_DECIM_KERNEL
static bool walker2_decim_covers(uint32_t sf, uint32_t decim) { return ((decim == 2u || decim == 4u) && sf >= 7u && sf <= 9u) || (sf == 6u && (decim == 4u || decim == 8u)); }

static uint32_t walker2_threads(uint32_t sf) { return 64u * (uint32_t)(sf == 7u ? kW2WavesSf7 : kW2WavesSf8); }

static uint32_t walker2_lds_bytes(uint32_t sf, bool grad = false, uint32_t decim = 8u)
{
    const uint32_t sps = decim << sf;
    const uint32_t nv = (3u * sps + 40u + 3u) & ~3u;
    if (decim != 8u || sf < 7u)
        return (uint32_t)((sizeof(W2Shared) + 15) & ~(size_t)15) + (2u * sps + nv + sps) * (uint32_t)sizeof(float) +
               (grad ? 0u : wave_tables_floats_d(sf, decim) * (uint32_t)sizeof(float)) + (2u * 256u + 8u) * (uint32_t)sizeof(double);
    if (!grad && sf == 8u && kW2Alias<8>)
        return (uint32_t)((sizeof(W2Shared) + 15) & ~(size_t)15) + (nv + sps) * (uint32_t)sizeof(float) + wave_tables_floats(sf) * (uint32_t)sizeof(float);
    return (uint32_t)((sizeof(W2Shared) + 15) & ~(size_t)15) + (2u * sps + nv + sps) * (uint32_t)sizeof(float) +
           (grad ? 0u : wave_tables_floats(sf) * (uint32_t)sizeof(float)) + (2u * 256u + 8u) * (uint32_t)sizeof(double);
}
```

### include/lora_hip.h

```cpp
#ifndef LORA_HIP_H
#define LORA_HIP_H

#include <stddef.h>
#include <stdint.h>

#ifdef __cplusplus
extern "C" {
#endif

#define LORA_HIP_ABI_VERSION 4

typedef enum lora_hip_status {
    LORA_HIP_OK = 0,
    LORA_HIP_ERR_BAD_SF = -1,
    LORA_HIP_ERR_BAD_CONFIG = -2,
    LORA_HIP_ERR_NO_DEVICE = -3,
    LORA_HIP_ERR_HIP = -4,
    LORA_HIP_ERR_NOMEM = -5,
    LORA_HIP_ERR_ARG = -6,
    LORA_HIP_ERR_OVERFLOW = -7,
    LORA_HIP_ERR_INTERNAL = -8
} lora_hip_status;

typedef enum lora_hip_iq_format {
    LORA_HIP_IQ_CF32 = 0,
    LORA_HIP_IQ_SC16 = 1,
    LORA_HIP_IQ_SC8 = 2,
    LORA_HIP_IQ_CU8 = 3
} lora_hip_iq_format;
size_t          lora_hip_iq_item_bytes(int fmt);

typedef enum lora_hip_demod {
    LORA_HIP_DEMOD_GRAD = 0,
    LORA_HIP_DEMOD_FFT = 1,
    LORA_HIP_DEMOD_FFT_COMPAT = 2
} lora_hip_demod;

#define LORA_HIP_FLAG_TRACE 0x1u
#define LORA_HIP_FLAG_FAST_SYNC 4u
#define LORA_HIP_FLAG_NO_DECOUPLED 8u
#define LORA_HIP_FLAG_PIN_HOST 2u

typedef struct lora_hip_config {
    uint32_t struct_size;
    float    samp_rate;
    uint32_t bandwidth;
    uint8_t  sf;
    uint8_t  implicit;
    uint8_t  cr;
    uint8_t  crc;
    uint8_t  reduced_rate;
    uint8_t  disable_drift_correction;
    uint8_t  reserved0[2];
    int32_t  device;
    int32_t  demod;
    uint32_t flags;
    uint32_t segment_symbols;
    uint32_t batch_items;
} lora_hip_config_t;

typedef struct lora_hip_frame_info {
    uint32_t stream;
    uint32_t length;
    int64_t  header_pos;
    int64_t  end_pos;
} lora_hip_frame_info_t;

typedef struct lora_hip_step {
    int32_t state;
    int32_t consumed;
    int64_t pos;
    int32_t bin;
    int32_t fine;
    float   value;
    uint32_t stream;
    uint32_t cycles;
    uint32_t reserved;
} lora_hip_step_t;

typedef struct lora_hip_timing {
    float    walker_ms;
    float    total_device_ms;
    uint32_t walker_launches;
    uint32_t jobs;
    uint32_t probes;
    uint32_t slow_path_relaunches;
    uint64_t items;
} lora_hip_timing_t;

typedef struct lora_hip_decoder lora_hip_decoder_t;

lora_hip_status lora_hip_create(const lora_hip_config_t *cfg, lora_hip_decoder_t **out);
void            lora_hip_destroy(lora_hip_decoder_t *h);
const char     *lora_hip_strerror(lora_hip_status s);
const char     *lora_hip_last_error(const lora_hip_decoder_t *h);
uint32_t        lora_hip_abi_version(void);

lora_hip_status lora_hip_get_geometry(const lora_hip_decoder_t *h, uint32_t *samples_per_symbol,
                                      uint32_t *bins, uint32_t *decimation);

lora_hip_status lora_hip_set_sf(lora_hip_decoder_t *h, uint8_t sf);
lora_hip_status lora_hip_set_samp_rate(lora_hip_decoder_t *h, float samp_rate);

lora_hip_status lora_hip_work(lora_hip_decoder_t *h, const float *iq, size_t n_items, size_t *consumed);
lora_hip_status lora_hip_work_raw(lora_hip_decoder_t *h, const void *iq, size_t n_items, int fmt, float scale, size_t *consumed);
lora_hip_status lora_hip_flush(lora_hip_decoder_t *h);

lora_hip_status lora_hip_set_stream_latency(lora_hip_decoder_t *h, float max_latency_ms);

typedef struct lora_hip_stream_info {
    uint64_t batch_items;
    uint64_t buffered_items;
    uint64_t passes;
    uint64_t passes_by_latency;
    int64_t  consumed_base;
    float    max_latency_ms;
    uint32_t pass_in_flight;
} lora_hip_stream_info_t;
lora_hip_status lora_hip_stream_info(const lora_hip_decoder_t *h, lora_hip_stream_info_t *out);

typedef struct lora_hip_mux lora_hip_mux_t;
lora_hip_status lora_hip_mux_create(const lora_hip_config_t *cfg, uint32_t n_channels, lora_hip_mux_t **out);
void            lora_hip_mux_destroy(lora_hip_mux_t *m);
lora_hip_status lora_hip_mux_work(lora_hip_mux_t *m, uint32_t channel, const float *iq, size_t n_items);
lora_hip_status lora_hip_mux_flush(lora_hip_mux_t *m);
lora_hip_status lora_hip_mux_set_latency(lora_hip_mux_t *m, float max_latency_ms);
lora_hip_status lora_hip_mux_set_max_ahead(lora_hip_mux_t *m, size_t max_ahead_items);
size_t          lora_hip_mux_frames_available(const lora_hip_mux_t *m);
lora_hip_status lora_hip_mux_poll_frame(lora_hip_mux_t *m, uint8_t *buf, size_t cap, size_t *len, lora_hip_frame_info_t *info);
lora_hip_status lora_hip_mux_passes(const lora_hip_mux_t *m, uint64_t *passes, uint64_t *passes_by_latency);
const char     *lora_hip_mux_last_error(const lora_hip_mux_t *m);

lora_hip_status lora_hip_decode_device(lora_hip_decoder_t *h, const void *d_iq, size_t total_items,
                                       const uint64_t *stream_off, const uint64_t *stream_len,
                                       uint32_t n_streams, void *hip_stream);

lora_hip_status lora_hip_iq_unpack_device(int device, const void *d_raw, size_t n_items, int fmt, float scale, void *d_out_cf32,
                                          void *hip_stream);

#define LORA_HIP_BEGIN_IQ_READY 1u
lora_hip_status lora_hip_decode_device_begin(lora_hip_decoder_t *h, const void *d_iq, size_t total_items,
                                             const uint64_t *stream_off, const uint64_t *stream_len,
                                             uint32_t n_streams, void *hip_stream, uint32_t flags);
lora_hip_status lora_hip_decode_device_end(lora_hip_decoder_t *h);
lora_hip_status lora_hip_decode_device_prepass(lora_hip_decoder_t *h, const void *d_iq, size_t total_items,
                                               const uint64_t *stream_off, const uint64_t *stream_len,
                                               uint32_t n_streams, void *hip_stream, uint32_t flags);

lora_hip_status lora_hip_gap_starts_device(lora_hip_decoder_t *h, const void *d_iq, size_t total_items,
                                           const uint64_t *stream_off, const uint64_t *stream_len, uint32_t n_streams,
                                           int64_t *pos, size_t cap, uint32_t *counts, void *hip_stream);

size_t          lora_hip_frames_available(const lora_hip_decoder_t *h);
lora_hip_status lora_hip_poll_frame(lora_hip_decoder_t *h, uint8_t *buf, size_t cap, size_t *len,
                                    lora_hip_frame_info_t *info);

lora_hip_status lora_hip_drain_frames(lora_hip_decoder_t *h, uint8_t *buf, size_t cap, lora_hip_frame_info_t *infos,
                                      size_t max_frames, size_t *n_frames);

lora_hip_status lora_hip_drain_slots(lora_hip_decoder_t *h, uint8_t *slots, size_t slot_bytes, size_t max_slots,
                                     size_t *n_frames);

lora_hip_status lora_hip_demod_symbols_device(lora_hip_decoder_t *h, const void *d_iq, size_t total_items,
                                              const int64_t *offsets, size_t n, int demod,
                                              uint32_t *bins_out, void *hip_stream);

lora_hip_status lora_hip_demod_symbols_ex_device(lora_hip_decoder_t *h, const void *d_iq, size_t total_items,
                                                 const int64_t *offsets, size_t n, int demod,
                                                 uint32_t *bins_out, int32_t *fine_out, void *hip_stream);

lora_hip_status lora_hip_last_timing(const lora_hip_decoder_t *h, lora_hip_timing_t *t);
const char     *lora_hip_walker_kernel_name(const lora_hip_decoder_t *h);
lora_hip_status lora_hip_last_payload_pass(const lora_hip_decoder_t *h, uint32_t *packets, uint32_t *moved, uint32_t *rerun, uint32_t *rounds,
                                           uint32_t *symbols, float *ms);

lora_hip_status lora_hip_last_plan(const lora_hip_decoder_t *h, uint32_t *burst_aware, uint32_t *segments);
lora_hip_status lora_hip_get_table(const lora_hip_decoder_t *h, int which, float *buf, size_t cap_floats, size_t *n_floats);
size_t          lora_hip_trace(const lora_hip_decoder_t *h, const lora_hip_step_t **steps);
void            lora_hip_trace_clear(lora_hip_decoder_t *h);

lora_hip_status lora_hip_estimate_cfo_device(lora_hip_decoder_t *h, const void *d_iq, size_t total_items,
                                             const int64_t *offsets, size_t n, int mode, float *cfo_hz_out,
                                             void *hip_stream);

lora_hip_status lora_hip_ref_ifreq_device(lora_hip_decoder_t *h, const void *d_iq, size_t n_items, float *arg_out, float *ifreq_out,
                                          void *hip_stream);

typedef struct lora_hip_window_stats {
    int32_t bin_down; float peak_down, total_down;
    int32_t bin_up;   float peak_up, total_up;
} lora_hip_window_stats_t;
lora_hip_status lora_hip_window_stats_device(lora_hip_decoder_t *h, const void *d_iq, size_t total_items, const int64_t *offsets,
                                             size_t n, lora_hip_window_stats_t *out, void *hip_stream);
typedef struct lora_hip_preamble {
    int64_t  header_pos;
    int64_t  run_pos;
    uint32_t stream;
    uint32_t run_len;
    int32_t  bin;
    int32_t  sfd_index;
    float    pmr;
    float    cfo_bins, cfo_hz;
    int32_t  delta;
} lora_hip_preamble_t;
lora_hip_status lora_hip_detect_preambles_device(lora_hip_decoder_t *h, const void *d_iq, size_t total_items,
                                                 const uint64_t *stream_off, const uint64_t *stream_len, uint32_t n_streams,
                                                 float threshold, lora_hip_preamble_t *out, size_t cap, size_t *n_found,
                                                 void *hip_stream);

lora_hip_status lora_hip_decode_at_headers_device(lora_hip_decoder_t *h, const void *d_iq, size_t total_items,
                                                  const uint64_t *stream_off, const uint64_t *stream_len, uint32_t n_streams,
                                                  const lora_hip_preamble_t *pre, size_t n, void *hip_stream);

typedef struct lora_hip_frame_check {
    uint8_t  has_header;
    uint8_t  header_checksum_ok;
    uint8_t  has_crc;
    uint8_t  crc_ok;
    uint8_t  header_checksum_rx, header_checksum_calc;
    uint16_t crc_rx, crc_calc;
    uint16_t reserved;
} lora_hip_frame_check_t;
lora_hip_status lora_hip_check_frame(const uint8_t *blob, size_t len, lora_hip_frame_check_t *out);

#ifdef __cplusplus
}
#endif
#endif
```

Measured before the change: 263,200.

## Finalize payload on control wavefront and precompute detect window ahead in walker2

Removes the separate kPlanFinalize workgroup round. The control wavefront now does the final payload decode (deshuffle, dewhiten, Hamming) inline using a wave-scoped LDS sync, right after the last payload symbol. Idle worker waves now also compute the next detect window speculatively and park the result, so the next DETECT round can skip re-evaluating that window when position and window count match. This saves a workgroup-wide barrier round per frame and some detect latency. In exchange it adds new counters to the job result and an API to read them, and it risks LDS hazards in the wave-only decode path.

Result: no change. 262,500 (-0.3%).

```diff
diff --git a/gr_lora_amd/capi.py b/gr_lora_amd/capi.py
--- a/gr_lora_amd/capi.py
+++ b/gr_lora_amd/capi.py
@@ -20,7 +20,7 @@
     "lora_hip_abi_version", "lora_hip_strerror", "lora_hip_last_error", "lora_hip_create", "lora_hip_destroy",
     "lora_hip_get_geometry", "lora_hip_set_sf", "lora_hip_set_samp_rate", "lora_hip_work", "lora_hip_flush",
     "lora_hip_decode_device", "lora_hip_frames_available", "lora_hip_poll_frame", "lora_hip_drain_frames", "lora_hip_drain_slots", "lora_hip_demod_symbols_device", "lora_hip_demod_symbols_ex_device",
-    "lora_hip_last_timing", "lora_hip_last_plan", "lora_hip_get_table", "lora_hip_last_payload_pass", "lora_hip_gap_starts_device", "lora_hip_decode_device_begin", "lora_hip_decode_device_end", "lora_hip_decode_device_prepass", "lora_hip_trace", "lora_hip_trace_clear", "lora_hip_check_frame", "lora_hip_estimate_cfo_device", "lora_hip_ref_ifreq_device",
+    "lora_hip_last_timing", "lora_hip_last_plan", "lora_hip_get_table", "lora_hip_last_payload_pass", "lora_hip_last_detect_ahead", "lora_hip_gap_starts_device", "lora_hip_decode_device_begin", "lora_hip_decode_device_end", "lora_hip_decode_device_prepass", "lora_hip_trace", "lora_hip_trace_clear", "lora_hip_check_frame", "lora_hip_estimate_cfo_device", "lora_hip_ref_ifreq_device",
     "lora_hip_set_stream_latency", "lora_hip_stream_info", "lora_hip_walker_kernel_name", "lora_hip_window_stats_device", "lora_hip_detect_preambles_device", "lora_hip_decode_at_headers_device",
     "lora_hip_mux_create", "lora_hip_mux_destroy", "lora_hip_mux_work", "lora_hip_mux_flush", "lora_hip_mux_set_latency", "lora_hip_mux_set_max_ahead", "lora_hip_mux_frames_available",
     "lora_hip_mux_poll_frame", "lora_hip_mux_passes", "lora_hip_mux_last_error",
@@ -172,6 +172,7 @@
     L.lora_hip_demod_symbols_ex_device.argtypes = [vp, vp, C.c_size_t, vp, C.c_size_t, C.c_int, vp, vp, vp]
     L.lora_hip_last_timing.argtypes = [vp, C.POINTER(Timing)]
     L.lora_hip_last_plan.argtypes = [vp, C.POINTER(C.c_uint32), C.POINTER(C.c_uint32)]
+    L.lora_hip_last_detect_ahead.argtypes = [vp] + [C.POINTER(C.c_uint32)] * 4
     L.lora_hip_last_payload_pass.argtypes = [vp, C.POINTER(C.c_uint32), C.POINTER(C.c_uint32), C.POINTER(C.c_uint32), C.POINTER(C.c_uint32), C.POINTER(C.c_uint32), C.POINTER(C.c_float)]
     L.lora_hip_decode_device_begin.argtypes = [vp, vp, C.c_size_t, vp, vp, C.c_uint32, vp, C.c_uint32]
     L.lora_hip_decode_device_end.argtypes = [vp]
@@ -509,6 +510,11 @@
         self._check(self.L.lora_hip_last_payload_pass(self.h, C.byref(a), C.byref(mv), C.byref(b), C.byref(r), C.byref(c), C.byref(m)))
         return dict(packets=int(a.value), moved=int(mv.value), rerun=int(b.value), rounds=int(r.value), symbols=int(c.value), ms=float(m.value))
 
+    def detect_ahead(self):
+        v = [C.c_uint32(0) for _ in range(4)]
+        self._check(self.L.lora_hip_last_detect_ahead(self.h, *[C.byref(x) for x in v]))
+        return dict(zip(("detect_parked", "detect_evaluated", "final_control", "final_workgroup"), (int(x.value) for x in v)))
+
     def trace(self):
         p = C.POINTER(Step)()
         n = self.L.lora_hip_trace(self.h, C.byref(p))
diff --git a/gr_lora_amd/csrc/lora_device.h b/gr_lora_amd/csrc/lora_device.h
--- a/gr_lora_amd/csrc/lora_device.h
+++ b/gr_lora_amd/csrc/lora_device.h
@@ -104,13 +104,14 @@
     uint32_t stop_reason;
     uint32_t n_steps;
     uint32_t pad;
-    uint32_t cyc[6];
-    uint32_t rounds[6];
+    uint32_t cyc[8];
+    uint32_t rounds[8];
     int64_t  tail_final_pos;
     uint32_t tail_valid, tail_first_rec, tail_n_attempts, tail_final_cr, tail_npush, tail_stop_reason, tail_pad, tail_rsv;
     float    tail_push_tail[4];
     uint32_t ctl[4];
     uint32_t dbg[6];
+    uint32_t ahead[4];
 };
 
 struct StepRec {
diff --git a/gr_lora_amd/csrc/lora_kernels.hip b/gr_lora_amd/csrc/lora_kernels.hip
--- a/gr_lora_amd/csrc/lora_kernels.hip
+++ b/gr_lora_amd/csrc/lora_kernels.hip
@@ -471,6 +471,33 @@
         sh.dec[k] = (uint8_t)((hi << 4) | lo);
     }
     __syncthreads();
+}
+
+__device__ __forceinline__ void wave_lds_sync()
+{
+    __builtin_amdgcn_wave_barrier();
+    asm volatile("s_waitcnt vmcnt(0) lgkmcnt(0)" ::: "memory");
+}
+__device__ void decode_payload_bytes_wave(Shared &sh, uint32_t n_cw, uint32_t cr, uint32_t n_bytes)
+{
+    const uint32_t lane = threadIdx.x & 63u;
+    wave_lds_sync();
+    for (uint32_t i = lane; i < n_cw; i += 64u) {
+        uint8_t w = deshuffle_byte(sh.cw[i]);
+        if (cr <= 2u) w ^= (i < LORA_WHITEN_CR56_LEN) ? c_whiten_cr56[i] : 0;
+        else w ^= (i < LORA_WHITEN_CR78_LEN) ? c_whiten_cr78[i] : 0;
+        sh.cw[i] = w;
+    }
+    wave_lds_sync();
+    for (uint32_t k = lane; k < n_bytes; k += 64u) {
+        const uint8_t c0 = (2u * k < n_cw) ? sh.cw[2u * k] : 0, c1 = (2u * k + 1u < n_cw) ? sh.cw[2u * k + 1u] : 0;
+        uint8_t lo, hi;
+        if (cr >= 3u) { lo = c_h84_decode[c0]; hi = c_h84_decode[c1]; }
+        else if (cr >= 1u) { lo = data_bits(c0); hi = data_bits(c1); }
+        else { lo = 0; hi = 0; }
+        sh.dec[k] = (uint8_t)((hi << 4) | lo);
+    }
+    wave_lds_sync();
 }
 
 template <int FLDS>
diff --git a/gr_lora_amd/csrc/lora_runtime.cpp b/gr_lora_amd/csrc/lora_runtime.cpp
--- a/gr_lora_amd/csrc/lora_runtime.cpp
+++ b/gr_lora_amd/csrc/lora_runtime.cpp
@@ -139,7 +139,7 @@
     hipEvent_t ev0 = nullptr, ev1 = nullptr, ev_done = nullptr;
     hipEvent_t ev_pre0 = nullptr, ev_pre1 = nullptr, ev_dep = nullptr;
     hipStream_t pre_stream = nullptr;
-    struct Pending { uint32_t nj = 0, recs_per_job = 0, eager = 0, trace_cap = 0; bool direct = true, open = false; hipStream_t st = nullptr;
+    struct Pending { uint32_t nj = 0, recs_per_job = 0, eager = 0, trace_cap = 0; bool direct = true, open = false, walker2 = false; hipStream_t st = nullptr;
                      std::chrono::steady_clock::time_point hp0, hp1; } pending;
     PassCtx pass;
     std::vector<StreamDesc> pass_streams;
@@ -185,6 +185,7 @@
     uint32_t dec_backoff = 0;
     uint32_t last_payload_packets = 0, last_payload_rerun = 0, last_payload_symbols = 0, last_payload_moved = 0, last_payload_rounds = 0;
     float last_payload_ms = 0.0f;
+    uint32_t last_ahead[4] = {0, 0, 0, 0};
     PinnedBuf<int64_t> p_pay_off;
     PinnedBuf<PayloadDesc> p_pay_desc;
     PinnedBuf<PayloadOut> p_pay_out;
@@ -435,6 +436,7 @@
     c.skip_payload = h->launch_skip ? 1u : 0u;
     HIP_TRY(h, hipEventRecord(h->ev0, st));
     if (nj >= h->last_kernel_jobs) { h->last_kernel = walker_kernel_name_for(h->P, nj, h->launch_skip); h->last_kernel_jobs = nj; }
+    h->pending.walker2 = std::strncmp(walker_kernel_name_for(h->P, nj, h->launch_skip), "walker2_", 8) == 0;
     if (launch_walker(h->P, c, st) != 0) return fail(h, LORA_HIP_ERR_HIP, "walker launch failed: %s", hipGetErrorString(hipGetLastError()));
     HIP_TRY(h, hipEventRecord(h->ev1, st));
     if (!direct) {
@@ -459,12 +461,18 @@
     HIP_TRY(h, hipEventSynchronize(h->ev_done));
     const auto hp2 = std::chrono::steady_clock::now();
     std::memcpy(out.res.data(), h->p_res.p, nj * sizeof(JobResult));
+    if (h->pending.walker2)
+        for (uint32_t j = 0; j < nj; j++) for (int i = 0; i < 4; i++) h->last_ahead[i] += out.res[j].ahead[i];
     static const bool dbg_stats = getenv("LORA_HIP_DEBUG") != nullptr;
     if (dbg_stats && h->P.use_fast) {
-        double cyc[6] = {0}, rnd[6] = {0};
-        for (uint32_t j = 0; j < nj; j++) for (int i = 0; i < 6; i++) { cyc[i] += 64.0 * out.res[j].cyc[i]; rnd[i] += out.res[j].rounds[i]; }
-        fprintf(stderr, "[lora_hip] per-job avg kcycles (rounds): DETECT %.0f (%.1f) SYNC %.0f (%.1f) SFD %.0f (%.1f) PAUSE %.0f (%.1f) HDR %.0f (%.1f) PAYLOAD %.0f (%.1f)\n",
-                cyc[0] / nj / 1e3, rnd[0] / nj, cyc[1] / nj / 1e3, rnd[1] / nj, cyc[2] / nj / 1e3, rnd[2] / nj, cyc[3] / nj / 1e3, rnd[3] / nj, cyc[4] / nj / 1e3, rnd[4] / nj, cyc[5] / nj / 1e3, rnd[5] / nj);
+        double cyc[8] = {0}, rnd[8] = {0};
+        uint32_t ahead[4] = {0, 0, 0, 0};
+        for (uint32_t j = 0; j < nj; j++) for (int i = 0; i < (h->pending.walker2 ? 8 : 6); i++) { cyc[i] += 64.0 * out.res[j].cyc[i]; rnd[i] += out.res[j].rounds[i]; }
+        if (h->pending.walker2) for (uint32_t j = 0; j < nj; j++) for (int i = 0; i < 4; i++) ahead[i] += out.res[j].ahead[i];
+        fprintf(stderr, "[lora_hip] per-job avg kcycles (rounds): DETECT %.0f (%.1f) SYNC %.0f (%.1f) SFD %.0f (%.1f) PAUSE %.0f (%.1f) HDR %.0f (%.1f) PAYLOAD %.0f (%.1f) DETECT-PARKED %.0f (%.1f) FINALIZE %.0f (%.1f); "
+                        "sums: DETECT rounds parked %u / evaluated %u, finalised by the control wavefront %u / the workgroup %u\n",
+                cyc[0] / nj / 1e3, rnd[0] / nj, cyc[1] / nj / 1e3, rnd[1] / nj, cyc[2] / nj / 1e3, rnd[2] / nj, cyc[3] / nj / 1e3, rnd[3] / nj, cyc[4] / nj / 1e3, rnd[4] / nj, cyc[5] / nj / 1e3, rnd[5] / nj,
+                cyc[6] / nj / 1e3, rnd[6] / nj, cyc[7] / nj / 1e3, rnd[7] / nj, ahead[0], ahead[1], ahead[2], ahead[3]);
         {
             double na = 0, nt = 0, ntv = 0; uint32_t sr[4] = {0, 0, 0, 0}, tsr[4] = {0, 0, 0, 0}, tpad = 0;
             for (uint32_t j = 0; j < nj; j++) {
@@ -479,7 +487,7 @@
         for (uint32_t j = 0; j < nj; j++) for (int i = 0; i < 4; i++) ctl[i] += 64.0 * out.res[j].ctl[i];
         fprintf(stderr, "[lora_hip] control per job, kcycles: copy-in %.0f loop %.0f plan %.0f copy-out %.0f (walker3: demodulation %.0f, replay %.0f of the decode rounds; with LORA_W3_REPLAY_STATS=2 copy-in and symbol loop in the 3rd / 4th figure)\n", ctl[0] / nj / 1e3, ctl[1] / nj / 1e3, ctl[2] / nj / 1e3, ctl[3] / nj / 1e3, ctl[0] / nj / 1e3, ctl[1] / nj / 1e3);
         std::vector<double> tot(nj);
-        for (uint32_t j = 0; j < nj; j++) { double t = 0; for (int i = 0; i < 6; i++) t += 64.0 * out.res[j].cyc[i]; tot[j] = t; }
+        for (uint32_t j = 0; j < nj; j++) { double t = 0; for (int i = 0; i < (h->pending.walker2 ? 7 : 6); i++) t += 64.0 * out.res[j].cyc[i]; tot[j] = t; }
         std::sort(tot.begin(), tot.end());
         double mean = 0; for (double t : tot) mean += t; mean /= nj;
         fprintf(stderr, "[lora_hip] job kcycles over %u jobs: min %.0f p50 %.0f p90 %.0f max %.0f mean %.0f\n", nj, tot[0] / 1e3, tot[nj / 2] / 1e3,
@@ -850,7 +858,7 @@
     int run_jobs_end(RunOut &out) { return ::run_jobs_end(h, out) == LORA_HIP_OK ? 0 : -1; }
     void publish(const AttemptRec &r, StreamDesc &sd) { ::publish(h, r, sd); }
     void append_trace(const RunOut &out, uint32_t job, uint32_t cap, int64_t base) { ::append_trace(h, out, job, cap, base); }
-    void count_jobs(uint32_t n) { h->timing.jobs += n; h->last_kernel_jobs = 0; if (h->dec_backoff) h->dec_backoff--; }
+    void count_jobs(uint32_t n) { h->timing.jobs += n; h->last_kernel_jobs = 0; if (h->dec_backoff) h->dec_backoff--; for (uint32_t &a : h->last_ahead) a = 0; }
     void count_probes(uint32_t n) { h->timing.probes += n; }
     void count_slow_path() { h->timing.slow_path_relaunches++; }
     void count_repair()
@@ -1927,6 +1935,16 @@
     return LORA_HIP_OK;
 }
 
+lora_hip_status lora_hip_last_detect_ahead(const lora_hip_decoder_t *h, uint32_t *detect_parked, uint32_t *detect_evaluated, uint32_t *final_control, uint32_t *final_workgroup)
+{
+    if (!h) return LORA_HIP_ERR_ARG;
+    if (detect_parked) *detect_parked = h->last_ahead[0];
+    if (detect_evaluated) *detect_evaluated = h->last_ahead[1];
+    if (final_control) *final_control = h->last_ahead[2];
+    if (final_workgroup) *final_workgroup = h->last_ahead[3];
+    return LORA_HIP_OK;
+}
+
 const char *lora_hip_walker_kernel_name(const lora_hip_decoder_t *h) { return h ? (h->last_kernel ? h->last_kernel : walker_kernel_name(h->P)) : ""; }
 
 lora_hip_status lora_hip_last_timing(const lora_hip_decoder_t *h, lora_hip_timing_t *t)
diff --git a/gr_lora_amd/csrc/lora_walker2.inc.hip b/gr_lora_amd/csrc/lora_walker2.inc.hip
--- a/gr_lora_amd/csrc/lora_walker2.inc.hip
+++ b/gr_lora_amd/csrc/lora_walker2.inc.hip
@@ -46,7 +46,8 @@
 struct alignas(16) W2Stats {
     long long prev_t;
     int32_t   prev_state;
-    uint32_t  cyc[6], rounds[6], ctl[4];
+    uint32_t  cyc[8], rounds[8], ctl[4];
+    uint32_t  ahead[4];
 };
 
 struct alignas(16) W2Shared {
@@ -66,6 +67,8 @@
     uint32_t words_pk[2];
     strict::Cands sc;
     uint32_t words_pk16[4];
+    int64_t  park_pos;
+    int32_t  park_kd, park_pad;
 };
 
 struct W2Tabs {
@@ -479,6 +482,16 @@
 }
 template <int SF, int LD> constexpr uint32_t w2_table_entries() { if constexpr (LD == 3 && SF >= 7) return WaveGeom<SF>::n_ent; else return WaveGeomD<SF, LD>::n_ent; }
 
+__device__ __forceinline__ void w2_finalize_wave(Shared &sh, uint32_t n_cw, uint32_t cr, uint32_t n_bytes, uint32_t plen, uint8_t *frame)
+{
+    decode_payload_bytes_wave(sh, n_cw, cr, n_bytes);
+    for (uint32_t i = threadIdx.x & 63u; i < plen; i += 64u) frame[3u + i] = (i < n_bytes) ? sh.dec[i] : 0;
+}
+__device__ __attribute__((noinline)) void w2_finalize_wave_call(Shared &sh, uint32_t n_cw, uint32_t cr, uint32_t n_bytes, uint32_t plen, uint8_t *frame)
+{
+    w2_finalize_wave(sh, n_cw, cr, n_bytes, plen, frame);
+}
+
 template <int SF, int WAVES, bool GRAD, bool SKIP = false, int LD = 3>
 __device__ __forceinline__ void walker2_body(const DevParams &P, const LaunchCfg &C)
 {
@@ -534,7 +547,6 @@
         pl.buf = 0; pl.resolve_prev = 0; pl.n_win = kW2Workers; pl.pos = S.pos; pl.prev_n = 0; pl.zmode = zreq ? 1 : 0;
         if (!S.done) (void)w2_pre_step(S, job, rec_cap, sps);
         if (S.done) { pl.mode = kPlanExit; return; }
-        if (S.fin_pending) { pl.mode = kPlanFinalize; return; }
         if (S.state != kDetect) W.det_streak = 0u;
         switch (S.state) {
         case kDetect:
@@ -557,7 +569,7 @@
     W2Tabs T{vl, ddl, W.red};
     uint32_t *bal_mine = nullptr, *bal_other = nullptr;
     uint32_t bal_rem = 0xffffffffu, bal_seen = 0u, bal_slot = 0u;
-    if (t0) W.prio = 0u;
+    if (t0) { W.prio = 0u; W.park_kd = 0; }
     if (t0 && C.balance) {
         const uint32_t hw = __builtin_amdgcn_s_getreg((31 << 11) | 4), xcc = __builtin_amdgcn_s_getreg((31 << 11) | 20);
         const uint32_t cu = ((xcc & 7u) << 8) | ((hw >> 8) & 0xffu);
@@ -592,7 +604,8 @@
         const long long t_start = clock64();
         if (t0) {
             W2Stats &Q = W.stats;
-            const int sidx = plan_mode == kPlanDetect ? 0 : plan_mode == kPlanSync ? 1 : plan_mode == kPlanSfd ? 2 : plan_mode == kPlanPause ? 3 : 5;
+            const int sidx = plan_mode == kPlanDetect ? ((W.park_kd == plan_n_win && W.park_pos == plan_pos) ? 6 : 0)
+                           : plan_mode == kPlanSync ? 1 : plan_mode == kPlanSfd ? 2 : plan_mode == kPlanPause ? 3 : 5;
             if (Q.prev_state >= 0) { Q.cyc[Q.prev_state] += (uint32_t)((t_start - Q.prev_t) >> 6); Q.rounds[Q.prev_state]++; }
             Q.prev_state = sidx; Q.prev_t = t_start;
         }
@@ -611,7 +624,8 @@
 
         if (plan_mode == kPlanDetect) {
             const int kd = plan_n_win;
-            if (!is_ctl) {
+            const bool parked = __builtin_amdgcn_readfirstlane((int)(W.park_kd == kd && W.park_pos == pos)) != 0;
+            if (!is_ctl && !parked) {
                 const int64_t dpos = pos + (int64_t)wave * kd * sps;
                 int nvalid = 0;
                 if (dpos + 2 * (int64_t)sps <= n_items) {
@@ -650,6 +664,8 @@
                 W.red[q] = pushed; W.red[64 + q] = e2; W.red[128 + q] = autocorr;
                 __builtin_amdgcn_wave_barrier();
                 if (t0) {
+                    W.park_kd = 0;
+                    W.stats.ahead[parked ? 0 : 1]++;
                     W2State L = S;
                     int64_t n_lim = (job.scan_limit - L.pos + (int64_t)sps - 1) / (int64_t)sps;
                     if (n_lim < 1) n_lim = 1;
@@ -820,25 +836,6 @@
             continue;
         }
 
-        if (plan_mode == kPlanFinalize) {
-            const uint32_t n_cw = S.n_cw, cr = S.cr, n_bytes = S.fin_n_bytes, plen = S.fin_plen;
-            decode_payload_bytes(sh, n_cw, cr, n_bytes);
-            AttemptRec &r = recs[S.n_att];
-            for (uint32_t i = threadIdx.x; i < plen; i += kW2) r.frame[3u + i] = (i < n_bytes) ? sh.dec[i] : 0;
-            __syncthreads();
-            if (t0) {
-                r.frame[0] = S.phdr[0]; r.frame[1] = S.phdr[1]; r.frame[2] = S.phdr[2];
-                r.frame_len = 3u + plen;
-                S.frame_ok = 1;
-                S.state = kDetect;
-                S.n_words = 0; S.n_cw = 0;
-                S.fin_pending = 0;
-                w2_end_step(S, job, C, recs, trace, S.fin_st, S.fin_consumed, S.fin_bin, S.fin_fine, 0.0f, t_start);
-                plan_from_state(next);
-            }
-            continue;
-        }
-
         int64_t dpos = pos;
         int32_t dn = plan_n_win;
         if (plan_resolve_prev && plan_prev_n > 0) {
@@ -871,6 +868,16 @@
                     } else
                     if constexpr (GRAD) wave_demod_symbol_grad<SF>(P, FT.v, X + dwpos, P.implicit != 0u, ws, wfine, wen);
                     else wave_demod_symbol<SF, kWaveFmode<SF>>(P, FT, X + dwpos, ws, wfine, P.implicit != 0u ? &wen : nullptr);
+                } else if (dn == 0) {
+                    const int nvalid = dwpos + 2 * (int64_t)sps <= n_items ? 1 : 0;
+                    float4 r = make_float4(0.f, 0.f, 0.f, 0.f);
+                    if (nvalid) r = w2_detect_window<GSF>(X + dwpos);
+                    if (lane == 0) {
+                        W.detn[wave] = nvalid;
+                        float *o = W.detf[wave * kW2DetectK];
+                        o[0] = r.x; o[1] = r.y; o[2] = r.z; o[3] = r.w;
+                        if (wave == 0) { W.park_pos = dpos; W.park_kd = 1; }
+                    }
                 }
                 if (lane == 0) { W.speci[plan_buf][widx][0] = dvalid ? (int32_t)ws : -1; W.speci[plan_buf][widx][1] = wfine; W.speci[plan_buf][widx][2] = __builtin_bit_cast(int32_t, wen); }
             }
@@ -906,7 +913,21 @@
                         if (ew < L.energy_threshold) { L.payload_symbols = 0; L.payload_length = L.n_cw / 2u; do_demod = false; bin_idx = 0u; step_bin = -1; fw = 0; }
                     }
                     if (w2_post_symbol<true, W16>(P, L, sh, bin_idx, is_first, wpk, do_demod)) {
-                        L.fin_pending = 1; L.fin_st = st_w; L.fin_consumed = (int32_t)sps + fw; L.fin_bin = step_bin; L.fin_fine = fw;
+                        if constexpr (SKIP) break;
+                        const long long tf0 = clock64();
+                        AttemptRec &r = recs[L.n_att];
+                        if constexpr (SF == 7 && LD == 3) w2_finalize_wave_call(sh, L.n_cw, L.cr, L.fin_n_bytes, L.fin_plen, r.frame);
+                        else w2_finalize_wave(sh, L.n_cw, L.cr, L.fin_n_bytes, L.fin_plen, r.frame);
+                        if (t0) {
+                            r.frame[0] = L.phdr[0]; r.frame[1] = L.phdr[1]; r.frame[2] = L.phdr[2];
+                            r.frame_len = 3u + L.fin_plen;
+                            W.stats.ahead[2]++; W.stats.rounds[7]++;
+                        }
+                        L.frame_ok = 1;
+                        L.state = kDetect;
+                        L.n_words = 0; L.n_cw = 0;
+                        w2_end_step(L, job, C, recs, trace, st_w, (int32_t)sps + fw, step_bin, fw, 0.0f, t_start, t0);
+                        if (t0) W.stats.cyc[7] += (uint32_t)((clock64() - tf0) >> 6);
                         break;
                     }
                     w2_end_step(L, job, C, recs, trace, st_w, (int32_t)sps + fw, step_bin, fw, 0.0f, t_start, t0);
@@ -930,7 +951,7 @@
                     }
                     if (L.done || fw != 0) break;
                 }
-                predicted = !zreq && !L.done && !L.fin_pending && (L.state == kDecodeHeader || L.state == kDecodePayload) && L.pos == dpos &&
+                predicted = !zreq && !L.done && (L.state == kDecodeHeader || L.state == kDecodePayload) && L.pos == dpos &&
                             w2_pre_step(L, job, rec_cap, sps);
             }
             const long long tr2 = clock64();
@@ -996,8 +1017,8 @@
         if (!go) {
             W2Stats &Q = W.stats;
             if (Q.prev_state >= 0) { Q.cyc[Q.prev_state] += (uint32_t)((clock64() - Q.prev_t) >> 6); Q.rounds[Q.prev_state]++; }
-            for (int i = 0; i < 6; i++) { jr.cyc[i] = Q.cyc[i]; jr.rounds[i] = Q.rounds[i]; }
-            for (int i = 0; i < 4; i++) jr.ctl[i] = Q.ctl[i];
+            for (int i = 0; i < 8; i++) { jr.cyc[i] = Q.cyc[i]; jr.rounds[i] = Q.rounds[i]; }
+            for (int i = 0; i < 4; i++) { jr.ctl[i] = Q.ctl[i]; jr.ahead[i] = Q.ahead[i]; }
             jr.dbg[0] = __builtin_amdgcn_s_getreg((31 << 11) | 4); jr.dbg[1] = __builtin_amdgcn_s_getreg((31 << 11) | 20);
             jr.dbg[2] = dbg_t0; jr.dbg[3] = (uint32_t)__builtin_amdgcn_s_memrealtime();
             jr.dbg[4] = dbg_c0; jr.dbg[5] = (uint32_t)(clock64() >> 6);
diff --git a/include/lora_hip.h b/include/lora_hip.h
--- a/include/lora_hip.h
+++ b/include/lora_hip.h
@@ -173,6 +173,9 @@
 const char     *lora_hip_walker_kernel_name(const lora_hip_decoder_t *h);
 lora_hip_status lora_hip_last_payload_pass(const lora_hip_decoder_t *h, uint32_t *packets, uint32_t *moved, uint32_t *rerun, uint32_t *rounds,
                                            uint32_t *symbols, float *ms);
+
+lora_hip_status lora_hip_last_detect_ahead(const lora_hip_decoder_t *h, uint32_t *detect_parked, uint32_t *detect_evaluated, uint32_t *final_control,
+                                           uint32_t *final_workgroup);
 
 lora_hip_status lora_hip_last_plan(const lora_hip_decoder_t *h, uint32_t *burst_aware, uint32_t *segments);
 lora_hip_status lora_hip_get_table(const lora_hip_decoder_t *h, int which, float *buf, size_t cap_floats, size_t *n_floats);
```
